# PolarisRisingWar/rgb-experiment

Hardware: AMD Instinct MI355X
Metric: aggregated edges/sec (full-graph GCN d=128, reference epoch = train fwd+bwd+Adam + 2 eval fwd) (higher is better)
Workload: dtype f32

## Files before the change

include/rgbx_hip.h:

```cpp
#ifndef RGBX_HIP_H
#define RGBX_HIP_H

#include <stddef.h>
#include <stdint.h>

#ifdef __cplusplus
extern "C" {
#endif

#define RGBX_VERSION 501

#define RGBX_OK 0
#define RGBX_E_ARG (-1)
#define RGBX_E_RANGE (-2)
#define RGBX_E_ALIGN (-3)
#define RGBX_E_WS (-4)
#define RGBX_E_SHAPE (-5)

typedef void* rgbx_stream_t;

enum {
  RGBX_LOOPS_KEEP = 0,
  RGBX_LOOPS_ADD_REMAINING = 1,
  RGBX_LOOPS_REMOVE_ADD = 2
// ... 77 lines not shown
  float* std;      int64_t ld_std;
  float* max;      int64_t ld_max;
  int32_t* argmax; int64_t ld_argmax;
  float* min;      int64_t ld_min;
  int32_t* argmin; int64_t ld_argmin;
} rgbx_multi_out_t;
int rgbx_spmm_csr_multi_supported(int64_t d);
int rgbx_spmm_csr_multi_partial_words(int64_t n_chunks, int64_t d, int which, int64_t* words);
int rgbx_spmm_csr_multi_f32(const int32_t* rowptr, const int32_t* col, const float* x, int64_t ldx,
                            const rgbx_multi_out_t* out, int64_t N, int64_t d, const rgbx_row_split_t* split,
                            rgbx_stream_t stream);

typedef struct rgbx_multi_grad {
  const float* a;        int64_t ld_a;
  const float* b;        int64_t ld_b;
  const float* x;        int64_t ld_x;
  const float* gmax;     int64_t ld_gmax;
  const int32_t* argmax; int64_t ld_argmax;
  const float* gmin;     int64_t ld_gmin;
  const int32_t* argmin; int64_t ld_argmin;
} rgbx_multi_grad_t;
int rgbx_multi_bwd_f32(const int32_t* rowptr_t, const int32_t* col_t, const int32_t* t2f, const rgbx_multi_grad_t* terms,
                       float* gx, int64_t ldgx, int64_t N, int64_t d, const rgbx_row_split_t* split, rgbx_stream_t stream);

typedef struct rgbx_spmm_epilogue {
  const struct rgbx_ce_epilogue* ce;
  int64_t n_classes;
  double* out_colsums;
  void* stats_ws;
  size_t stats_ws_bytes;
} rgbx_spmm_epilogue_t;

int rgbx_spmm_csr_epilogue_supported(int64_t d);
int rgbx_spmm_csr_epilogue_f32(const int32_t* rowptr, const int32_t* col, const float* w, const float* rs,
                               const float* x, int64_t ldx, const float* y, int64_t ldy, const float* bias,
                               float* out, int64_t ldo, int64_t N, int64_t d, float a, float b,
                               const rgbx_row_split_t* split, const rgbx_spmm_epilogue_t* epi,
                               rgbx_stream_t stream);

int rgbx_spmm_csr_short_rows_supported(int64_t d);
int rgbx_spmm_csr_short_rows_f32(const int32_t* rowptr, const int32_t* col, const float* w, const float* x, int64_t ldx,
                                 const float* bias, float* out, int64_t ldo, int64_t N, int64_t d, rgbx_stream_t stream);

typedef struct rgbx_ce_epilogue {
  const int64_t* y;
  const uint8_t* mask;
  const float* grad_scale;
  double* stats;
  double* scratch;
  int32_t mask_groups;
  const int32_t* rows;
  int64_t n_rows;
  int32_t skip_unselected;
} rgbx_ce_epilogue_t;

int rgbx_spmm_linear_supported(int64_t K, int64_t Nout, int has_root);
int rgbx_ce_rows_grad_scratch_doubles(int64_t N, int64_t* count);
int rgbx_spmm_linear_stats_workspace_bytes(int64_t N, int64_t Nout, size_t* bytes);
int rgbx_spmm_linear_f32(const int32_t* rowptr, const int32_t* col, const float* w, const float* rs,
                         const float* x, int64_t ldx, const float* wt, const float* x_root, int64_t ldr,
                         const float* wt_root, const float* bias, float* out, int64_t ldo, float* z_out,
                         int64_t ldz, const float* pre_scale, const float* pre_shift, const float* pre_rowsum,
                         double* out_colsums, void* stats_ws, size_t stats_ws_bytes,
                         const rgbx_ce_epilogue_t* ce, int64_t N, int64_t K, int64_t Nout,
                         const rgbx_row_split_t* split, rgbx_stream_t stream);

typedef struct rgbx_fused_layer {
  const int32_t* rowptr;
  const int32_t* col;
  const float* w;
  const float* rs;
  const float* x;
  int64_t ldx;
  int64_t x_blk_cols, x_blk_stride;
  const float* wt;
  const float* x_root;
  int64_t ldr;
  int64_t xr_blk_cols, xr_blk_stride;
  const float* wt_root;
  const float* bias;
  float* out;
  int64_t ldo;
  float* out_blk;
  int64_t ob_cols, ob_stride;
  float* z_out;
  int64_t ldz;
  const float* pre_scale;
  const float* pre_shift;
  const float* pre_rowsum;
  double* out_colsums;
  void* stats_ws;
  size_t stats_ws_bytes;
  const rgbx_ce_epilogue_t* ce;
  int64_t N, K, Nout;
  const rgbx_row_split_t* split;
  const float* w_pos;
  float* z_pos_out;
  const uint8_t* col_sel;
} rgbx_fused_layer_t;

int rgbx_fused_layer_f32(const rgbx_fused_layer_t* layer, rgbx_stream_t stream);

int rgbx_blocked_to_rows_f32(const float* src, int64_t blk_cols, int64_t blk_stride, float* dst, int64_t ldd,
                             int64_t n, int64_t d, const float* bias, rgbx_stream_t stream);

int rgbx_appnp_f32(const int32_t* rowptr, const int32_t* col, const float* w, const float* h,
                   int64_t ldh, float* out, float* tmp, int64_t ldo, int64_t N, int64_t d, int K,
                   float alpha, const rgbx_row_split_t* split, rgbx_stream_t stream);


int rgbx_dagnn_gate_fwd_f32(const float* h0, int64_t ld0, const float* hops, int64_t hop_stride, int64_t ldh,
                            const float* s, const float* b, float* out, int64_t ldo, int64_t N, int64_t d, int K,
                            rgbx_stream_t stream);

int rgbx_dagnn_gate_bwd_workspace_bytes(int64_t d, size_t* bytes);
int rgbx_dagnn_gate_bwd_f32(const float* h0, int64_t ld0, const float* hops, int64_t hop_stride, int64_t ldh,
                            const float* s, const float* b, const float* gout, int64_t ldg, float* d0,
                            int64_t ldd0, float* dk, int64_t d_stride, int64_t ldd, float* g_s, float* g_b,
                            void* ws, size_t ws_bytes, int64_t N, int64_t d, int K, rgbx_stream_t stream);


int rgbx_gru_step_supported(int64_t C);
int rgbx_gru_step_f32(const int32_t* rowptr, const int32_t* col, const float* x, int64_t ldx, const float* wt,
                      const float* wt_root, const float* bias, float* out, int64_t ldo, float* z_out, int64_t ldz,
                      float* pre_out, int64_t ldp, int64_t N, int64_t C, const rgbx_row_split_t* split,
                      rgbx_stream_t stream);

int rgbx_gru_gate_fwd_f32(const float* pre, int64_t ldp, const float* x, int64_t ldx, float* out, int64_t ldo,
                          int64_t N, int64_t C, rgbx_stream_t stream);

int rgbx_gru_gate_bwd_f32(const float* pre, int64_t ldp, const float* x, int64_t ldx, const float* gout, int64_t ldg,
                          float* dpre, int64_t lddp, float* dx, int64_t lddx, int64_t N, int64_t C,
                          rgbx_stream_t stream);


int rgbx_gat_scores_f32(const float* hfeat, int64_t ldh, const float* att_src,
                        const float* att_dst, float* a_src, float* a_dst, int64_t n, int H, int C,
                        rgbx_stream_t stream);

int rgbx_gat_scores_bwd_scratch_floats(int64_t n, int H, int C, int64_t* count);

int rgbx_gat_scores_bwd_f32(const float* hfeat, int64_t ldh, const float* g_a_src, const float* g_a_dst,
                            int64_t n_dst, const float* att_src, const float* att_dst, float* g_hfeat,
                            int64_t ldgh, float* g_att_src, float* g_att_dst, float* scratch,
                            int64_t scratch_floats, int64_t n, int H, int C, rgbx_stream_t stream);

int rgbx_gat_aggregate_fwd_f32(const int32_t* rowptr, const int32_t* col, const float* hfeat,
                               int64_t ldh, const float* a_src, const float* att_src,
                               float* a_dst, const float* att_dst, const float* out_scale, const float* bias,
                               float* out, int64_t ldo, float* m, float* rden, float* out_pos, float* a_pos,
                               int64_t N, int H, int C, float slope, const rgbx_row_split_t* split,
// ... 105 lines not shown
                                 const float* nodeq, const float* gout, int64_t ldg, float* g_k, int64_t ldgk,
                                 float* g_v, int64_t ldgv, int64_t N, int H, int C, float scale, const uint32_t* seed,
                                 float p_drop, const rgbx_row_split_t* split, rgbx_stream_t stream);



int rgbx_resgated_supported(int C);

int rgbx_resgated_fwd_f32(const int32_t* rowptr, const int32_t* col, const float* k, int64_t ldk, const float* q,
                          int64_t ldq, const float* v, int64_t ldv, float* out, int64_t ldo, int64_t N, int C,
                          const rgbx_row_split_t* split, rgbx_stream_t stream);

int rgbx_resgated_bwd_dst_f32(const int32_t* rowptr, const int32_t* col, const float* k, int64_t ldk, const float* q,
                              int64_t ldq, const float* v, int64_t ldv, const float* gout, int64_t ldg, float* g_k,
                              int64_t ldgk, int64_t N, int C, const rgbx_row_split_t* split, rgbx_stream_t stream);

int rgbx_resgated_bwd_src_f32(const int32_t* rowptr_t, const int32_t* col_t, const float* k, int64_t ldk, const float* q,
                              int64_t ldq, const float* v, int64_t ldv, const float* gout, int64_t ldg, float* g_q,
                              int64_t ldgq, float* g_v, int64_t ldgv, int64_t N, int C, const rgbx_row_split_t* split,
                              rgbx_stream_t stream);



int rgbx_softmax_aggr_supported(int C);

int rgbx_softmax_aggr_fwd_f32(const int32_t* rowptr, const int32_t* col, const float* m, int64_t ldm, const float* t,
                              int t_stride, float* out, int64_t ldo, float* lse, int64_t ldl, int64_t N, int C,
                              const rgbx_row_split_t* split, rgbx_stream_t stream);

int rgbx_softmax_aggr_gt_partial_floats(int64_t N, int C, const rgbx_row_split_t* split, int64_t* count);

int rgbx_softmax_aggr_bwd_f32(const int32_t* rowptr_t, const int32_t* col_t, const float* m, int64_t ldm, const float* t,
                              int t_stride, const float* out, int64_t ldo, const float* lse, int64_t ldl,
                              const float* gout, int64_t ldg, float* g_m, int64_t ldgm, float* g_t, float* gt_partial,
                              int64_t n_gt_partial, int64_t N, int C, const rgbx_row_split_t* split,
                              rgbx_stream_t stream);


int rgbx_gemm_tn_workspace_bytes(int64_t K, int64_t M, int64_t N, size_t* bytes);

int rgbx_gemm_tn_f32(const float* A, int64_t lda, const float* B, int64_t ldb, float* C, int64_t ldc,
                     float* a_colsum, int64_t K, int64_t M, int64_t N, float alpha, void* workspace,
                     size_t workspace_bytes, rgbx_stream_t stream);

int rgbx_gemm_tn_bn_bwd_f32(const float* G, int64_t ldg, const float* X, int64_t ldx, const float* mean,
                            const float* rstd, const float* ca, const float* cb, const float* ck, const float* B,
                            int64_t ldb, float* C, int64_t ldc, float* a_colsum, int64_t K, int64_t M, int64_t N,
                            float alpha, void* workspace, size_t workspace_bytes, rgbx_stream_t stream);

int rgbx_gemm_tn_rows_f32(const float* A, int64_t lda, const float* B, int64_t ldb, const int32_t* rows,
                          int64_t n_rows, float* C, int64_t ldc, float* a_colsum, int64_t K, int64_t M, int64_t N,
                          float alpha, void* workspace, size_t workspace_bytes, rgbx_stream_t stream);


int rgbx_bn_scratch_doubles(int64_t N, int64_t d, int64_t* count);

int rgbx_bn_stats_f32(const float* x, int64_t ldx, int64_t N, int64_t d, double* sums, double* scratch,
                      int64_t scratch_doubles, rgbx_stream_t stream);

int rgbx_bn_finalize_f32(const double* packed, const float* weight, const float* bias, float eps, float momentum,
                         float* running_mean, float* running_var, float* mean, float* rstd, float* scale,
                         float* shift, int64_t d, rgbx_stream_t stream);

int rgbx_fold_bn_linear_f32(const float* W, int64_t ldw, const float* Wr, int64_t ldwr, const float* bias,
                            const float* bias2, const float* gamma, const float* beta, const float* running_mean,
                            const float* running_var, float eps, float* wt, float* wrt, float* b_out, int64_t Nout,
                            int64_t K, rgbx_stream_t stream);

int rgbx_bn_bwd_finalize_f32(const double* glob, const double* local, const double* count, const float* weight,
                             const float* rstd, float* ca, float* cb, float* ck, float* g_weight, float* g_bias,
                             int64_t d, rgbx_stream_t stream);

int rgbx_affine_cols_f32(const float* x, int64_t ldx, const float* scale, const float* shift, float* y,
                         int64_t ldy, int64_t N, int64_t d, rgbx_stream_t stream);

int rgbx_bn_bwd_reduce_f32(const float* gy, int64_t ldg, const float* x, int64_t ldx, const float* mean,
                           const float* rstd, int64_t N, int64_t d, double* sums, double* scratch,
                           int64_t scratch_doubles, rgbx_stream_t stream);

int rgbx_bn_bwd_apply_f32(const float* gy, int64_t ldg, const float* x, int64_t ldx, const float* mean,
                          const float* rstd, const float* ca, const float* cb, const float* ck, float* gx,
                          int64_t ldgx, int64_t N, int64_t d, rgbx_stream_t stream);


int rgbx_masked_nll_scratch_doubles(int64_t N, int want_accuracy, int64_t* count);

int rgbx_masked_nll_fwd_f32(const float* logp, int64_t ld, const int64_t* y, const uint8_t* mask,
                            int64_t N, int64_t C, double* stats, double* scratch,
                            int64_t scratch_doubles, int want_accuracy, rgbx_stream_t stream);

int rgbx_masked_nll_bwd_f32(const int64_t* y, const uint8_t* mask, int64_t N, int64_t C,
                            const float* scale, float* grad, int64_t ldg, rgbx_stream_t stream);

int rgbx_masked_ce_fwd_f32(const float* logits, int64_t ld, const int64_t* y, const uint8_t* mask, int64_t N,
                           int64_t C, double* stats, double* scratch, int64_t scratch_doubles,
                           rgbx_stream_t stream);

int rgbx_masked_ce_fwd_blocked_f32(const float* logits, int64_t blk_cols, int64_t blk_stride, const float* bias,
                                   const int64_t* y, const uint8_t* mask, int64_t N, int64_t C, double* stats,
                                   double* scratch, int64_t scratch_doubles, rgbx_stream_t stream);

int rgbx_masked_ce_bwd_f32(const float* logits, int64_t ld, const int64_t* y, const uint8_t* mask, int64_t N,
                           int64_t C, const float* scale, float* grad, int64_t ldg, rgbx_stream_t stream);


int rgbx_coalesce_workspace_bytes(int64_t E, int64_t N, int mirror, size_t* bytes);
// ... 54 lines not shown
```

rgb_experiment_amd/_lib.py:

```python
import ctypes
import os

import torch

_HERE = os.path.dirname(os.path.abspath(__file__))
LIB_PATH = os.path.join(_HERE, "csrc", "librgbx_hip.so")

_P = ctypes.c_void_p
_I64 = ctypes.c_int64
_I = ctypes.c_int
_F = ctypes.c_float

class RowSplit(ctypes.Structure):
    _fields_ = [("threshold", ctypes.c_int32), ("n_chunks", ctypes.c_int32), ("n_long", ctypes.c_int32),
                ("chunk_begin", ctypes.c_void_p), ("chunk_end", ctypes.c_void_p), ("chunk_row", ctypes.c_void_p),
                ("long_row", ctypes.c_void_p),
                ("long_chunk_ptr", ctypes.c_void_p), ("partial", ctypes.c_void_p)]


class MultiOut(ctypes.Structure):
    _fields_ = [(f, t) for name in ("sum", "mean", "var", "std", "max", "argmax", "min", "argmin")
                for f, t in ((name, ctypes.c_void_p), ("ld_" + name, ctypes.c_int64))]


class MultiGrad(ctypes.Structure):
    _fields_ = [(f, t) for name in ("a", "b", "x", "gmax", "argmax", "gmin", "argmin")
                for f, t in ((name, ctypes.c_void_p), ("ld_" + name, ctypes.c_int64))]


class CeEpilogue(ctypes.Structure):
    _fields_ = [("y", ctypes.c_void_p), ("mask", ctypes.c_void_p), ("grad_scale", ctypes.c_void_p),
                ("stats", ctypes.c_void_p), ("scratch", ctypes.c_void_p), ("mask_groups", ctypes.c_int32),
                ("rows", ctypes.c_void_p), ("n_rows", ctypes.c_int64), ("skip_unselected", ctypes.c_int32)]


class SpmmEpilogue(ctypes.Structure):
    _fields_ = [("ce", ctypes.c_void_p), ("n_classes", ctypes.c_int64), ("out_colsums", ctypes.c_void_p),
                ("stats_ws", ctypes.c_void_p), ("stats_ws_bytes", ctypes.c_size_t)]


class FusedLayer(ctypes.Structure):
    _fields_ = [("rowptr", _P), ("col", _P), ("w", _P), ("rs", _P), ("x", _P), ("ldx", _I64),
                ("x_blk_cols", _I64), ("x_blk_stride", _I64), ("wt", _P), ("x_root", _P), ("ldr", _I64),
                ("xr_blk_cols", _I64), ("xr_blk_stride", _I64), ("wt_root", _P), ("bias", _P), ("out", _P),
                ("ldo", _I64), ("out_blk", _P), ("ob_cols", _I64), ("ob_stride", _I64), ("z_out", _P), ("ldz", _I64),
                ("pre_scale", _P), ("pre_shift", _P), ("pre_rowsum", _P), ("out_colsums", _P), ("stats_ws", _P),
                ("stats_ws_bytes", ctypes.c_size_t), ("ce", _P), ("N", _I64), ("K", _I64), ("Nout", _I64),
                ("split", _P), ("w_pos", _P), ("z_pos_out", _P), ("col_sel", _P)]


SIGNATURES = {
    "rgbx_csr_workspace_bytes": [_I64, _I64, ctypes.POINTER(ctypes.c_size_t)],
    "rgbx_csr_build": [_P, _P, _I64, _I64, _I, _P, _P, _P, _P, ctypes.c_size_t, _P],
    "rgbx_deg_inv_sqrt_f32": [_P, _I64, _P, _P],
    "rgbx_gcn_norm_f32": [_P, _P, _I64, _P, _P, _P],
    "rgbx_inv_degree_f32": [_P, _I64, _P, _P],
    "rgbx_loop_weights_f32": [_P, _P, _P, _I64, _I64, _I, _F, _P, _P, _P],
    "rgbx_edge_slot_weights_f32": [_P, _I64, _P, _I64, _P, _P, _P],
    "rgbx_weighted_deg_inv_sqrt_f32": [_P, _P, _I64, _P, _P],
    "rgbx_gcn_norm_weighted_f32": [_P, _P, _P, _I64, _P, _P, _P],
    "rgbx_edge_dot_supported": [_I64],
    "rgbx_edge_dot_f32": [_P, _P, _P, _I64, _P, _I64, _P, _I64, _I64, _P, _P],
    "rgbx_gcn_norm_bwd_f32": [_P, _P, _P, _P, _P, _P, _P, _P, _P, _P, _I64, _I64, _P, _P, _P],
    "rgbx_spmm_csr_f32": [_P, _P, _P, _P, _P, _I64, _P, _I64, _P, _P, _I64, _I64, _I64, _F, _F, _P, _P],
    "rgbx_spmm_csr_extremum_supported": [_I64],
    "rgbx_spmm_csr_extremum_f32": [_P, _P, _P, _I64, _P, _I64, _P, _I64, _I64, _I, _P, _P],
    "rgbx_extremum_bwd_f32": [_P, _P, _P, _P, _I64, _P, _P, _I64, _I64, _I64, _P, _P],
    "rgbx_spmm_csr_multi_supported": [_I64],
    "rgbx_spmm_csr_multi_partial_words": [_I64, _I64, _I, ctypes.POINTER(ctypes.c_int64)],
    "rgbx_spmm_csr_multi_f32": [_P, _P, _P, _I64, _P, _I64, _I64, _P, _P],
    "rgbx_multi_bwd_f32": [_P, _P, _P, _P, _P, _I64, _I64, _I64, _P, _P],
    "rgbx_spmm_csr_epilogue_supported": [_I64],
    "rgbx_spmm_csr_epilogue_f32": [_P, _P, _P, _P, _P, _I64, _P, _I64, _P, _P, _I64, _I64, _I64, _F, _F, _P, _P, _P],
    "rgbx_spmm_csr_short_rows_supported": [_I64],
    "rgbx_spmm_csr_short_rows_f32": [_P, _P, _P, _P, _I64, _P, _P, _I64, _I64, _I64, _P],
    "rgbx_spmm_linear_supported": [_I64, _I64, _I],
    "rgbx_ce_rows_grad_scratch_doubles": [_I64, ctypes.POINTER(ctypes.c_int64)],
    "rgbx_spmm_linear_stats_workspace_bytes": [_I64, _I64, ctypes.POINTER(ctypes.c_size_t)],
    "rgbx_spmm_linear_f32": [_P, _P, _P, _P, _P, _I64, _P, _P, _I64, _P, _P, _P, _I64, _P, _I64, _P, _P, _P, _P, _P,
                             ctypes.c_size_t, _P, _I64, _I64, _I64, _P, _P],
    "rgbx_fused_layer_f32": [_P, _P],
    "rgbx_blocked_to_rows_f32": [_P, _I64, _I64, _P, _I64, _I64, _I64, _P, _P],
    "rgbx_appnp_f32": [_P, _P, _P, _P, _I64, _P, _P, _I64, _I64, _I64, _I, _F, _P, _P],
    "rgbx_dagnn_gate_fwd_f32": [_P, _I64, _P, _I64, _I64, _P, _P, _P, _I64, _I64, _I64, _I, _P],
    "rgbx_dagnn_gate_bwd_workspace_bytes": [_I64, ctypes.POINTER(ctypes.c_size_t)],
    "rgbx_dagnn_gate_bwd_f32": [_P, _I64, _P, _I64, _I64, _P, _P, _P, _I64, _P, _I64, _P, _I64, _I64, _P, _P, _P,
                                ctypes.c_size_t, _I64, _I64, _I, _P],
    "rgbx_gru_step_supported": [_I64],
    "rgbx_gru_step_f32": [_P, _P, _P, _I64, _P, _P, _P, _P, _I64, _P, _I64, _P, _I64, _I64, _I64, _P, _P],
    "rgbx_gru_gate_fwd_f32": [_P, _I64, _P, _I64, _P, _I64, _I64, _I64, _P],
    "rgbx_gru_gate_bwd_f32": [_P, _I64, _P, _I64, _P, _I64, _P, _I64, _P, _I64, _I64, _I64, _P],
    "rgbx_gat_scores_f32": [_P, _I64, _P, _P, _P, _P, _I64, _I, _I, _P],
    "rgbx_gat_scores_bwd_scratch_floats": [_I64, _I, _I, ctypes.POINTER(ctypes.c_int64)],
    "rgbx_gat_scores_bwd_f32": [_P, _I64, _P, _P, _I64, _P, _P, _P, _I64, _P, _P, _P, _I64, _I64, _I, _I, _P],
    "rgbx_gat_aggregate_fwd_f32": [_P, _P, _P, _I64, _P, _P, _P, _P, _P, _P, _P, _I64, _P, _P, _P, _P, _I64, _I, _I, _F, _P,
                                   _P],
    "rgbx_gat_edge_softmax_f32": [_P, _P, _P, _P, _F, _P, _P, _P, _P, _P, _I64, _P, _P],
    "rgbx_gat_bwd_dst_f32": [_P, _P, _P, _I64, _P, _P, _P, _P, _P, _I64, _P, _I64, _P, _P, _I64, _I, _I,
                             _F, _P],
    "rgbx_gat_bwd_prep_f32": [_P, _P, _P, _P, _I64, _P, _P, _I64, _P, _P, _P, _F, _P, _I64, _I, _I, _P],
    "rgbx_gat_bwd_src_f32": [_P, _P, _P, _I64, _P, _P, _P, _I64, _P, _I64, _P, _P, _P, _P, _I64, _I, _I, _F, _P, _P],
    "rgbx_supergat_supported": [_I, _I],
    "rgbx_supergat_loss_records": [_I64, _P, ctypes.POINTER(ctypes.c_int64)],
    "rgbx_supergat_aggregate_fwd_f32": [_P, _P, _P, _I64, _P, _P, _P, _P, _I64, _P, _P, _I64, _I, _I, _F, _P, _F, _F, _P,
                                        _I64, _P, _P, _P],
    "rgbx_supergat_bwd_dst_f32": [_P, _P, _P, _I64, _P, _P, _P, _P, _P, _I64, _P, _P, _I64, _P, _P, _I64, _P, _I64, _I, _I,
                                  _F, _P, _F, _F, _P, _P, _P],
    "rgbx_supergat_bwd_src_f32": [_P, _P, _P, _P, _I64, _P, _P, _P, _I64, _P, _I64, _P, _I64, _I, _I, _F, _P, _F, _F, _P,
                                  _P, _P],
    "rgbx_supergat_sample_negatives": [_P, _I64, _I64, _P, _I64, _I, _P, _P, _P],
    "rgbx_supergat_neg_loss_fwd_f32": [_P, _I64, _P, _P, _I64, _I, _I, _P, _I64, _P, _P],
    "rgbx_supergat_neg_loss_bwd_f32": [_P, _I64, _P, _P, _I64, _I, _I, _P, _P, _I64, _P],
    "rgbx_supergat_draws_u8": [_P, _I64, _I, _F, _F, _P, _P, _P],
    "rgbx_gatv2_supported": [_I, _I],
    "rgbx_gatv2_fwd_f32": [_P, _P, _P, _I64, _P, _I64, _P, _P, _P, _I64, _P, _P, _I64, _I, _I, _F, _P, _F, _P, _P],
    "rgbx_gatv2_att_partial_floats": [_I64, _I, _I, _P, ctypes.POINTER(ctypes.c_int64)],
    "rgbx_gatv2_bwd_dst_f32": [_P, _P, _P, _I64, _P, _I64, _P, _P, _P, _P, _I64, _P, _P, _I64, _P, _P, _I64, _P, _P, _I64,
                               _I64, _I, _I, _F, _P, _F, _P, _P],
    "rgbx_gatv2_bwd_src_f32": [_P, _P, _P, _P, _I64, _P, _I64, _P, _P, _P, _I64, _P, _I64, _I64, _I, _I, _F, _P, _F, _P,
                               _P],
    "rgbx_gatv2_draws_u8": [_P, _I64, _I, _F, _P, _P],
    "rgbx_transformer_supported": [_I, _I],
    "rgbx_transformer_fwd_f32": [_P, _P, _P, _I64, _P, _I64, _P, _I64, _P, _I64, _P, _P, _I64, _I, _I, _F, _P, _F, _P,
                                 _P],
    "rgbx_transformer_bwd_dst_f32": [_P, _P, _P, _I64, _P, _I64, _P, _I64, _P, _P, _P, _I64, _P, _I64, _P, _P, _I64,
                                     _I64, _I, _I, _F, _P, _F, _P, _P],
    "rgbx_transformer_bwd_src_f32": [_P, _P, _P, _P, _I64, _P, _I64, _P, _I64, _P, _P, _I64, _P, _I64, _P, _I64, _I64,
                                     _I, _I, _F, _P, _F, _P, _P],
    "rgbx_resgated_supported": [_I],
    "rgbx_resgated_fwd_f32": [_P, _P, _P, _I64, _P, _I64, _P, _I64, _P, _I64, _I64, _I, _P, _P],
    "rgbx_resgated_bwd_dst_f32": [_P, _P, _P, _I64, _P, _I64, _P, _I64, _P, _I64, _P, _I64, _I64, _I, _P, _P],
    "rgbx_resgated_bwd_src_f32": [_P, _P, _P, _I64, _P, _I64, _P, _I64, _P, _I64, _P, _I64, _P, _I64, _I64, _I, _P,
                                  _P],
    "rgbx_softmax_aggr_supported": [_I],
    "rgbx_softmax_aggr_fwd_f32": [_P, _P, _P, _I64, _P, _I, _P, _I64, _P, _I64, _I64, _I, _P, _P],
    "rgbx_softmax_aggr_gt_partial_floats": [_I64, _I, _P, ctypes.POINTER(ctypes.c_int64)],
    "rgbx_softmax_aggr_bwd_f32": [_P, _P, _P, _I64, _P, _I, _P, _I64, _P, _I64, _P, _I64, _P, _I64, _P, _P, _I64, _I64,
                                  _I, _P, _P],
    "rgbx_gemm_tn_workspace_bytes": [_I64, _I64, _I64, ctypes.POINTER(ctypes.c_size_t)],
    "rgbx_gemm_tn_f32": [_P, _I64, _P, _I64, _P, _I64, _P, _I64, _I64, _I64, _F, _P, ctypes.c_size_t, _P],
    "rgbx_gemm_tn_bn_bwd_f32": [_P, _I64, _P, _I64, _P, _P, _P, _P, _P, _P, _I64, _P, _I64, _P, _I64, _I64, _I64, _F, _P,
                                ctypes.c_size_t, _P],
    "rgbx_gemm_tn_rows_f32": [_P, _I64, _P, _I64, _P, _I64, _P, _I64, _P, _I64, _I64, _I64, _F, _P, ctypes.c_size_t, _P],
    "rgbx_bn_scratch_doubles": [_I64, _I64, ctypes.POINTER(ctypes.c_int64)],
    "rgbx_bn_stats_f32": [_P, _I64, _I64, _I64, _P, _P, _I64, _P],
    "rgbx_bn_finalize_f32": [_P, _P, _P, _F, _F, _P, _P, _P, _P, _P, _P, _I64, _P],
    "rgbx_fold_bn_linear_f32": [_P, _I64, _P, _I64, _P, _P, _P, _P, _P, _P, _F, _P, _P, _P, _I64, _I64, _P],
    "rgbx_bn_bwd_finalize_f32": [_P, _P, _P, _P, _P, _P, _P, _P, _P, _P, _I64, _P],
    "rgbx_affine_cols_f32": [_P, _I64, _P, _P, _P, _I64, _I64, _I64, _P],
    "rgbx_bn_bwd_reduce_f32": [_P, _I64, _P, _I64, _P, _P, _I64, _I64, _P, _P, _I64, _P],
    "rgbx_bn_bwd_apply_f32": [_P, _I64, _P, _I64, _P, _P, _P, _P, _P, _P, _I64, _I64, _I64, _P],
    "rgbx_masked_nll_scratch_doubles": [_I64, _I, ctypes.POINTER(ctypes.c_int64)],
    "rgbx_masked_nll_fwd_f32": [_P, _I64, _P, _P, _I64, _I64, _P, _P, _I64, _I, _P],
    "rgbx_masked_ce_fwd_f32": [_P, _I64, _P, _P, _I64, _I64, _P, _P, _I64, _P],
    "rgbx_masked_ce_fwd_blocked_f32": [_P, _I64, _I64, _P, _P, _P, _I64, _I64, _P, _P, _I64, _P],
    "rgbx_masked_ce_bwd_f32": [_P, _I64, _P, _P, _I64, _I64, _P, _P, _I64, _P],
    "rgbx_masked_nll_bwd_f32": [_P, _P, _I64, _I64, _P, _P, _I64, _P],
    "rgbx_coalesce_workspace_bytes": [_I64, _I64, _I, ctypes.POINTER(ctypes.c_size_t)],
    "rgbx_coalesce_keys_i64": [_P, _P, _I64, _I64, _I, _P, _P, _P, ctypes.c_size_t, _P],
    "rgbx_split_edge_keys_i64": [_P, _P, _I64, _I64, _P, _P, _P],
    "rgbx_gather_rows_f32": [_P, _I64, _P, _I64, _I64, _P, _I64, _P],
    "rgbx_scatter_add_rows_f32": [_P, _I64, _P, _I64, _I64, _P, _I64, _P],
    "rgbx_paced_copy_f32": [_P, _P, _I64, _I, _I, _P],
    "rgbx_py_random_shuffle_i64": [_I64, _I64, _P],
    "rgbx_faconv_supported": [_I64],
    "rgbx_faconv_scores_f32": [_P, _I64, _P, _P, _P, _I64, _I64, _P],
    "rgbx_faconv_fwd_f32": [_P, _P, _P, _P, _I64, _P, _P, _I64, _F, _P, _I64, _I64, _I64, _P, _F, _P, _P],
    "rgbx_faconv_bwd_dst_f32": [_P, _P, _P, _P, _I64, _P, _P, _I64, _P, _I64, _I64, _P, _F, _P, _P],
    "rgbx_faconv_bwd_src_f32": [_P, _P, _P, _P, _P, _I64, _P, _P, _I64, _P, _P, _P, _P, _I64, _I64, _I64, _P, _F, _P,
                                _P],
    "rgbx_faconv_edge_coef_f32": [_P, _P, _P, _P, _P, _I, _I64, _P, _F, _P, _P, _P],
    "rgbx_faconv_edge_dot_f32": [_P, _P, _P, _P, _I64, _P, _I64, _P, _I64, _I64, _I64, _P],
    "rgbx_faconv_draws_u8": [_P, _I64, _F, _P, _P],
}
EXPORTS = ["rgbx_version", "rgbx_last_error_string"] + list(SIGNATURES)

_lib = None


def bind(path, strict=True):
    lib = ctypes.CDLL(path)
    lib.rgbx_version.restype = _I
    lib.rgbx_version.argtypes = []
    lib.rgbx_last_error_string.restype = ctypes.c_char_p
    lib.rgbx_last_error_string.argtypes = []
    for name, argtypes in SIGNATURES.items():
        if not strict and not hasattr(lib, name):
            continue
        fn = getattr(lib, name)
        fn.restype = _I
        fn.argtypes = argtypes
    return lib


def load():
    global _lib
# ... 46 lines not shown
```

rgb_experiment_amd/csrc/gemm.hip:

```cpp
#include "rgbx_common.h"

namespace rgbx {
namespace {

constexpr int BM = 128, BN = 128, KT = 32;
enum { A_PLAIN = 0, A_BN = 1, A_ROWS = 2 };

struct TnExtra {
  const float* X;
  int64_t ldx;
  const float *mean, *rstd, *ca, *cb, *ck;
  const int32_t* rows;
  int64_t n_rows;
};
using f32x16 = __attribute__((ext_vector_type(16))) float;

template <int W>
__device__ __forceinline__ void stage_tile(float* __restrict__ lds, const float* __restrict__ src,
                                           int64_t ld, int64_t k0, int64_t k_end, int c0, int ncols) {
  const int tid = threadIdx.x;
#pragma unroll 4
  for (int p = 0; p < KT * W / 256; ++p) {
    const int idx = p * 256 + tid;
    const int r = idx / W, c = idx % W;
    const int64_t k = k0 + r;
    lds[r * W + c] = (k < k_end && c0 + c < ncols) ? src[k * ld + c0 + c] : 0.f;
  }
}

template <int W>
__device__ __forceinline__ void fetch_tile(float4 (&regs)[KT * (W / 4) / 256], const float* __restrict__ src, int64_t ld,
                                           int64_t k0, int64_t k_end, int c0, int ncols) {
#pragma unroll
  for (int p = 0; p < KT * (W / 4) / 256; ++p) {
    const int idx = p * 256 + threadIdx.x;
    const int r = idx / (W / 4), c = (idx % (W / 4)) * 4;
    const int64_t k = k0 + r;
    regs[p] = make_float4(0.f, 0.f, 0.f, 0.f);
    if (k < k_end && c0 + c < ncols) regs[p] = *reinterpret_cast<const float4*>(src + k * ld + c0 + c);
  }
}

template <int W>
__device__ __forceinline__ void put_tile(float* __restrict__ lds, const float4 (&regs)[KT * (W / 4) / 256]) {
#pragma unroll
  for (int p = 0; p < KT * (W / 4) / 256; ++p) {
    const int idx = p * 256 + threadIdx.x;
    const int r = idx / (W / 4), c = (idx % (W / 4)) * 4;
    *reinterpret_cast<float4*>(lds + r * W + c) = regs[p];
  }
}

template <int W>
__device__ __forceinline__ void put_tile_bn(float* __restrict__ lds, const float4 (&rg)[KT * (W / 4) / 256],
                                            const float4 (&rx)[KT * (W / 4) / 256], const float* __restrict__ lc,
                                            int64_t k0, int64_t k_end, int c0, int ncols) {
#pragma unroll
  for (int p = 0; p < KT * (W / 4) / 256; ++p) {
    const int idx = p * 256 + threadIdx.x;
// ... 88 lines not shown
      for (int i = 0; i < MI; ++i) {
        acc[i][0] = __builtin_amdgcn_mfma_f32_32x32x2f32(a[i], b0, acc[i][0], 0, 0, 0);
        acc[i][1] = __builtin_amdgcn_mfma_f32_32x32x2f32(a[i], b1, acc[i][1], 0, 0, 0);
      }
    }
  };
  if constexpr (MODE == A_BN) {
    float* lc = lds + KT * (MT + 128);
    for (int i = threadIdx.x; i < 5 * MT; i += 256) {
      const float* src = i < MT ? ex.mean : i < 2 * MT ? ex.rstd : i < 3 * MT ? ex.ca : i < 4 * MT ? ex.cb : ex.ck;
      const int c = m0 + i % MT;
      lc[i] = c < M ? src[c] : 0.f;
    }
    float4 ra[KT * (MT / 4) / 256], rx[KT * (MT / 4) / 256], rb[KT * 32 / 256];
    fetch_tile<MT>(ra, A, lda, k_begin, k_end, m0, M);
    fetch_tile<MT>(rx, ex.X, ex.ldx, k_begin, k_end, m0, M);
    fetch_tile<128>(rb, B, ldb, k_begin, k_end, n0, N);
    for (int64_t k0 = k_begin; k0 < k_end; k0 += KT) {
      __syncthreads();
      put_tile_bn<MT>(la, ra, rx, lc, k0, k_end, m0, M);
      put_tile<128>(lb, rb);
      __syncthreads();
      if (k0 + KT < k_end) {
        fetch_tile<MT>(ra, A, lda, k0 + KT, k_end, m0, M);
        fetch_tile<MT>(rx, ex.X, ex.ldx, k0 + KT, k_end, m0, M);
        fetch_tile<128>(rb, B, ldb, k0 + KT, k_end, n0, N);
      }
      consume();
    }
  } else if constexpr (MODE == A_ROWS) {
    const int64_t j_begin = lower_bound_rows(ex.rows, ex.n_rows, k_begin);
    const int64_t j_end = lower_bound_rows(ex.rows, ex.n_rows, k_end);
    float4 ra[KT * (MT / 4) / 256], rb[KT * 32 / 256];
    int32_t ia[KT * (MT / 4) / 256], ib[KT * 32 / 256];
    fetch_row_ids<MT>(ia, ex.rows, j_begin, j_end);
    fetch_row_ids<128>(ib, ex.rows, j_begin, j_end);
    fetch_tile_rows<MT>(ra, A, lda, ia, m0, M);
    fetch_tile_rows<128>(rb, B, ldb, ib, n0, N);
    fetch_row_ids<MT>(ia, ex.rows, j_begin + KT, j_end);
    fetch_row_ids<128>(ib, ex.rows, j_begin + KT, j_end);
    for (int64_t j0 = j_begin; j0 < j_end; j0 += KT) {
      __syncthreads();
      put_tile<MT>(la, ra);
      put_tile<128>(lb, rb);
      __syncthreads();
      if (j0 + KT < j_end) {
        fetch_tile_rows<MT>(ra, A, lda, ia, m0, M);
        fetch_tile_rows<128>(rb, B, ldb, ib, n0, N);
        fetch_row_ids<MT>(ia, ex.rows, j0 + 2 * KT, j_end);
        fetch_row_ids<128>(ib, ex.rows, j0 + 2 * KT, j_end);
      }
      consume();
    }
  } else if constexpr (VEC4) {
    float4 ra[KT * (MT / 4) / 256], rb[KT * 32 / 256];
    fetch_tile<MT>(ra, A, lda, k_begin, k_end, m0, M);
    fetch_tile<128>(rb, B, ldb, k_begin, k_end, n0, N);
    for (int64_t k0 = k_begin; k0 < k_end; k0 += KT) {
      __syncthreads();
      put_tile<MT>(la, ra);
      put_tile<128>(lb, rb);
      __syncthreads();
      if (k0 + KT < k_end) {
        fetch_tile<MT>(ra, A, lda, k0 + KT, k_end, m0, M);
        fetch_tile<128>(rb, B, ldb, k0 + KT, k_end, n0, N);
      }
      consume();
    }
  } else {
    for (int64_t k0 = k_begin; k0 < k_end; k0 += KT) {
      __syncthreads();
      stage_tile<MT>(la, A, lda, k0, k_end, m0, M);
      stage_tile<128>(lb, B, ldb, k0, k_end, n0, N);
      __syncthreads();
      consume();
    }
  }

  if (sums && m0 + (int)threadIdx.x < M) colpart[(int64_t)split * M + m0 + threadIdx.x] = csum;
  float* out = part + (int64_t)split * M * N;
#pragma unroll
  for (int i = 0; i < MI; ++i)
#pragma unroll
    for (int j = 0; j < 2; ++j)
#pragma unroll
      for (int r = 0; r < 16; ++r) {
        const int m = m0 + wm + i * 32 + (r & 3) + 8 * (r >> 2) + 4 * kr;
        const int n = n0 + wn + j * 32 + cc;
        if (m < M && n < N) out[(int64_t)m * N + n] = acc[i][j][r];
      }
}

__global__ void __launch_bounds__(256)
gemm_tn_reduce_kernel(const float* __restrict__ part, int S, int64_t MN, float* __restrict__ C, int N,
                      int64_t ldc, float alpha) {
  __shared__ float sh[8][32];
  const int j = threadIdx.x & 31, q = threadIdx.x >> 5;
  for (int64_t base = (int64_t)blockIdx.x * 32; base < MN; base += (int64_t)gridDim.x * 32) {
    const int64_t i = base + j;
    float s = 0.f;
    if (i < MN)
      for (int p = q; p < S; p += 8) s += part[(int64_t)p * MN + i];
    __syncthreads();
    sh[q][j] = s;
    __syncthreads();
    if (q == 0 && i < MN) {
      float t = 0.f;
#pragma unroll
      for (int k = 0; k < 8; ++k) t += sh[k][j];
      C[(i / N) * ldc + (i % N)] = alpha * t;
    }
  }
}

int tile_rows(int M) { return M <= 64 ? 64 : BM; }

int choose_splits(int64_t K, int M, int N) {
  const int64_t tiles = cdiv(M, tile_rows(M)) * cdiv(N, BN);
  int64_t s = cdiv(tile_rows(M) == 64 ? 1024 : 768, tiles);
  const int64_t max_s = cdiv(K, 16 * KT);
  if (s > max_s) s = max_s;
  if (s < 1) s = 1;
  return (int)s;
}

}
}

using namespace rgbx;

extern "C" int rgbx_gemm_tn_workspace_bytes(int64_t K, int64_t M, int64_t N, size_t* bytes) {
  if (!bytes || K < 0 || M < 0 || N < 0) return fail(RGBX_E_ARG, "gemm_tn_workspace_bytes: bad argument");
  if (M >= INT32_MAX || N >= INT32_MAX) return fail(RGBX_E_RANGE, "gemm_tn: M or N exceeds int32");
  *bytes = (size_t)choose_splits(K, (int)M, (int)N) * ((size_t)M * (size_t)N + (size_t)M) * sizeof(float);
  return RGBX_OK;
}

namespace rgbx {
namespace {

int run_gemm_tn(const char* name, int mode, const float* A, int64_t lda, const float* B, int64_t ldb, float* C,
                int64_t ldc, float* a_colsum, int64_t K, int64_t M, int64_t N, float alpha, void* workspace,
                size_t workspace_bytes, rgbx_stream_t stream, const TnExtra& ex) {
  if (K < 0 || M < 0 || N < 0) return fail(RGBX_E_ARG, "%s: negative size", name);
  if (M == 0 || N == 0) return RGBX_OK;
  if (!C || (K > 0 && (!A || !B))) return fail(RGBX_E_ARG, "%s: null pointer", name);
  if (M >= INT32_MAX || N >= INT32_MAX) return fail(RGBX_E_RANGE, "%s: M or N exceeds int32", name);
  if (lda < M || ldb < N || ldc < N) return fail(RGBX_E_ARG, "%s: leading dimension too small", name);
  bool v4 = aligned16(A) && aligned16(B) && lda % 4 == 0 && ldb % 4 == 0;
  if (mode == A_BN) {
    if (K > 0 && (!ex.X || !ex.mean || !ex.rstd || !ex.ca || !ex.cb || !ex.ck))
      return fail(RGBX_E_ARG, "%s: null pointer", name);
    if (ex.ldx < M) return fail(RGBX_E_ARG, "%s: leading dimension too small", name);
    v4 = v4 && aligned16(ex.X) && ex.ldx % 4 == 0;
  }
  if (mode == A_ROWS) {
    if (ex.n_rows < 0 || ex.n_rows > K || (ex.n_rows > 0 && !ex.rows)) return fail(RGBX_E_ARG, "%s: bad row list", name);
    if (K >= INT32_MAX) return fail(RGBX_E_RANGE, "%s: K exceeds int32", name);
  }
  if (mode != A_PLAIN && !v4)
    return fail(RGBX_E_ALIGN, "%s: operands must be 16-byte aligned with leading dimensions that are multiples of 4", name);
  size_t need = 0;
  if (int rc = rgbx_gemm_tn_workspace_bytes(K, M, N, &need)) return rc;
  if (!workspace || workspace_bytes < need)
    return fail(RGBX_E_WS, "%s: workspace %zu < %zu bytes", name, workspace_bytes, need);
  hipStream_t s = (hipStream_t)stream;
  const int S = choose_splits(K, (int)M, (int)N);
  const int64_t slab = cdiv(cdiv(K > 0 ? K : 1, S), KT) * KT;
  float* part = static_cast<float*>(workspace);
  float* colpart = a_colsum ? part + (size_t)S * M * N : nullptr;
  const int mt = tile_rows((int)M);
  dim3 grid(S, (unsigned)cdiv(M, mt), (unsigned)cdiv(N, BN));
#define RGBX_GEMM_TN(V4, MT, MODE) \
  gemm_tn_partial_kernel<V4, MT, MODE><<<grid, 256, 0, s>>>(A, lda, B, ldb, part, colpart, K, (int)M, (int)N, slab, ex)
  if (mode == A_BN) { if (mt == 64) RGBX_GEMM_TN(true, 64, A_BN); else RGBX_GEMM_TN(true, 128, A_BN); }
  else if (mode == A_ROWS) { if (mt == 64) RGBX_GEMM_TN(true, 64, A_ROWS); else RGBX_GEMM_TN(true, 128, A_ROWS); }
  else if (v4) { if (mt == 64) RGBX_GEMM_TN(true, 64, A_PLAIN); else RGBX_GEMM_TN(true, 128, A_PLAIN); }
  else { if (mt == 64) RGBX_GEMM_TN(false, 64, A_PLAIN); else RGBX_GEMM_TN(false, 128, A_PLAIN); }
#undef RGBX_GEMM_TN
  RGBX_CHECK_LAUNCH("gemm_tn_partial_kernel");
  const int64_t MN = M * N;
  int64_t rb = cdiv(MN, 32);
  if (rb > kMaxGrid) rb = kMaxGrid;
  gemm_tn_reduce_kernel<<<(int)rb, 256, 0, s>>>(part, S, MN, C, (int)N, ldc, alpha);
  RGBX_CHECK_LAUNCH("gemm_tn_reduce_kernel");
  if (a_colsum) {
    gemm_tn_reduce_kernel<<<(int)cdiv(M, 32), 256, 0, s>>>(colpart, S, M, a_colsum, (int)M, M, 1.0f);
    RGBX_CHECK_LAUNCH("gemm_tn_reduce_kernel");
  }
  return RGBX_OK;
}

}
}

extern "C" int rgbx_gemm_tn_f32(const float* A, int64_t lda, const float* B, int64_t ldb, float* C,
                                int64_t ldc, float* a_colsum, int64_t K, int64_t M, int64_t N, float alpha,
                                void* workspace, size_t workspace_bytes, rgbx_stream_t stream) {
  return run_gemm_tn("gemm_tn", A_PLAIN, A, lda, B, ldb, C, ldc, a_colsum, K, M, N, alpha, workspace, workspace_bytes,
                     stream, TnExtra{});
}

extern "C" int rgbx_gemm_tn_bn_bwd_f32(const float* G, int64_t ldg, const float* X, int64_t ldx, const float* mean,
                                       const float* rstd, const float* ca, const float* cb, const float* ck,
                                       const float* B, int64_t ldb, float* C, int64_t ldc, float* a_colsum, int64_t K,
                                       int64_t M, int64_t N, float alpha, void* workspace, size_t workspace_bytes,
                                       rgbx_stream_t stream) {
  TnExtra ex{};
  ex.X = X, ex.ldx = ldx, ex.mean = mean, ex.rstd = rstd, ex.ca = ca, ex.cb = cb, ex.ck = ck;
  return run_gemm_tn("gemm_tn_bn_bwd", A_BN, G, ldg, B, ldb, C, ldc, a_colsum, K, M, N, alpha, workspace,
                     workspace_bytes, stream, ex);
}

extern "C" int rgbx_gemm_tn_rows_f32(const float* A, int64_t lda, const float* B, int64_t ldb, const int32_t* rows,
                                     int64_t n_rows, float* C, int64_t ldc, float* a_colsum, int64_t K, int64_t M,
                                     int64_t N, float alpha, void* workspace, size_t workspace_bytes,
                                     rgbx_stream_t stream) {
  TnExtra ex{};
  ex.rows = rows, ex.n_rows = n_rows;
  return run_gemm_tn("gemm_tn_rows", A_ROWS, A, lda, B, ldb, C, ldc, a_colsum, K, M, N, alpha, workspace,
                     workspace_bytes, stream, ex);
}
```

rgb_experiment_amd/csrc/graph_prep.hip:

```cpp
#include "rgbx_common.h"

#include <rocprim/rocprim.hpp>

namespace rgbx {

char* err_buf() {
  static thread_local char buf[256] = "";
  return buf;
}

namespace {

__global__ void __launch_bounds__(256)
fill_keys_kernel(const int64_t* __restrict__ agg_row, const int64_t* __restrict__ other_row,
                 int64_t E, int64_t M, int N, int loops_mode, int* __restrict__ keys,
                 int* __restrict__ ids) {
  for (int64_t e = (int64_t)blockIdx.x * blockDim.x + threadIdx.x; e < M;
       e += (int64_t)gridDim.x * blockDim.x) {
    int key;
    if (e < E) {
      const int64_t t = agg_row[e];
      key = (loops_mode != RGBX_LOOPS_KEEP && other_row[e] == t) ? N : (int)t;
    } else {
      key = (int)(e - E);
// ... 33 lines not shown
  }
}

__global__ void __launch_bounds__(256)
inv_degree_kernel(const int* __restrict__ rowptr, int N, float* __restrict__ inv) {
  for (int i = blockIdx.x * blockDim.x + threadIdx.x; i < N; i += gridDim.x * blockDim.x) {
    const int cnt = rowptr[i + 1] - rowptr[i];
    inv[i] = 1.0f / (float)(cnt > 1 ? cnt : 1);
  }
}

__global__ void __launch_bounds__(256)
gcn_norm_kernel(const int* __restrict__ rowptr, const int* __restrict__ col, int N,
                const float* __restrict__ dis, float* __restrict__ w) {
  const int lane = threadIdx.x & 63;
  const int wpb = blockDim.x >> 6;
  for (int row = blockIdx.x * wpb + (threadIdx.x >> 6); row < N; row += gridDim.x * wpb) {
    const int s = rowptr[row], e = rowptr[row + 1];
    const float di = dis[row];
    for (int p = s + lane; p < e; p += 64) w[p] = dis[col[p]] * di;
  }
}


__global__ void __launch_bounds__(256) fill_i32_kernel(int* __restrict__ v, int64_t n, int value) {
  for (int64_t i = (int64_t)blockIdx.x * blockDim.x + threadIdx.x; i < n; i += (int64_t)gridDim.x * blockDim.x)
    v[i] = value;
}

__global__ void __launch_bounds__(256)
loop_source_kernel(const int64_t* __restrict__ src, const int64_t* __restrict__ dst, int64_t E,
                   int* __restrict__ loop_src) {
  for (int64_t e = (int64_t)blockIdx.x * blockDim.x + threadIdx.x; e < E; e += (int64_t)gridDim.x * blockDim.x) {
    const int64_t t = dst[e];
    if (src[e] == t) atomicMax(loop_src + t, (int)e);
  }
}

__global__ void __launch_bounds__(256)
loop_weight_kernel(const int* __restrict__ loop_src, const float* __restrict__ ew, int N, float fill,
                   float* __restrict__ loop_w) {
  for (int i = blockIdx.x * blockDim.x + threadIdx.x; i < N; i += gridDim.x * blockDim.x) {
    const int e = loop_src[i];
    loop_w[i] = e >= 0 ? ew[e] : fill;
  }
}

__global__ void __launch_bounds__(256)
slot_weight_kernel(const int* __restrict__ perm, int64_t nnz, const float* __restrict__ ew, int64_t E,
                   const float* __restrict__ loop_w, float* __restrict__ ew_slot) {
  for (int64_t p = (int64_t)blockIdx.x * blockDim.x + threadIdx.x; p < nnz; p += (int64_t)gridDim.x * blockDim.x) {
    const int id = perm[p];
    ew_slot[p] = id < E ? ew[id] : loop_w[id - E];
  }
}

__device__ __forceinline__ float wave_sum_fixed(float v) {
#pragma unroll
  for (int off = 32; off >= 1; off >>= 1) v += __shfl_xor(v, off);
  return v;
}

__global__ void __launch_bounds__(256)
weighted_deg_inv_sqrt_kernel(const int* __restrict__ rowptr, const float* __restrict__ ew_slot, int N,
                             float* __restrict__ dis) {
  const int lane = threadIdx.x & 63;
  const int wpb = blockDim.x >> 6;
  for (int row = blockIdx.x * wpb + (threadIdx.x >> 6); row < N; row += gridDim.x * wpb) {
    const int s = rowptr[row], e = rowptr[row + 1];
    float acc = 0.f;
    for (int p = s + lane; p < e; p += 64) acc += ew_slot[p];
    const float deg = wave_sum_fixed(acc);
    if (lane == 0) dis[row] = deg == 0.f ? 0.f : 1.0f / sqrtf(deg);
  }
}

__global__ void __launch_bounds__(256)
gcn_norm_weighted_kernel(const int* __restrict__ rowptr, const int* __restrict__ col,
                         const float* __restrict__ ew_slot, int N, const float* __restrict__ dis,
                         float* __restrict__ w) {
  const int lane = threadIdx.x & 63;
  const int wpb = blockDim.x >> 6;
  for (int row = blockIdx.x * wpb + (threadIdx.x >> 6); row < N; row += gridDim.x * wpb) {
    const int s = rowptr[row], e = rowptr[row + 1];
    const float di = dis[row];
    for (int p = s + lane; p < e; p += 64) w[p] = dis[col[p]] * ew_slot[p] * di;
  }
}

__global__ void __launch_bounds__(256)
gcn_norm_bwd_deg_kernel(const int* __restrict__ rowptr, const int* __restrict__ col,
                        const int* __restrict__ rowptr_t, const int* __restrict__ col_t,
                        const int* __restrict__ t2f, const float* __restrict__ g,
                        const float* __restrict__ ew_slot, const float* __restrict__ dis, int N,
                        float* __restrict__ ddeg) {
  const int lane = threadIdx.x & 63;
  const int wpb = blockDim.x >> 6;
  for (int row = blockIdx.x * wpb + (threadIdx.x >> 6); row < N; row += gridDim.x * wpb) {
    float acc = 0.f;
    for (int p = rowptr[row] + lane; p < rowptr[row + 1]; p += 64) acc = fmaf(g[p] * ew_slot[p], dis[col[p]], acc);
    float acc_t = 0.f;
    for (int q = rowptr_t[row] + lane; q < rowptr_t[row + 1]; q += 64) {
      const int p = t2f[q];
      acc_t = fmaf(g[p] * ew_slot[p], dis[col_t[q]], acc_t);
    }
    const float ddis = wave_sum_fixed(acc) + wave_sum_fixed(acc_t);
// ... 141 lines not shown
  RGBX_CHECK_LAUNCH("loop_weight_kernel");
  return RGBX_OK;
}

extern "C" int rgbx_edge_slot_weights_f32(const int32_t* perm, int64_t nnz, const float* ew, int64_t E,
                                          const float* loop_w, float* ew_slot, rgbx_stream_t stream) {
  if (nnz < 0 || E < 0 || (nnz > 0 && (!perm || !ew_slot)) || (E > 0 && !ew))
    return fail(RGBX_E_ARG, "edge_slot_weights: null pointer or negative size");
  if (nnz > E && !loop_w) return fail(RGBX_E_ARG, "edge_slot_weights: nnz > E needs loop weights");
  if (nnz == 0) return RGBX_OK;
  slot_weight_kernel<<<grid_for(nnz), 256, 0, (hipStream_t)stream>>>(perm, nnz, ew, E, loop_w, ew_slot);
  RGBX_CHECK_LAUNCH("slot_weight_kernel");
  return RGBX_OK;
}

extern "C" int rgbx_weighted_deg_inv_sqrt_f32(const int32_t* rowptr, const float* ew_slot, int64_t N, float* dis,
                                              rgbx_stream_t stream) {
  if (N < 0 || !rowptr || !ew_slot || (N > 0 && !dis)) return fail(RGBX_E_ARG, "weighted_deg_inv_sqrt: bad argument");
  if (N >= INT32_MAX) return fail(RGBX_E_RANGE, "weighted_deg_inv_sqrt: N exceeds int32");
  if (N == 0) return RGBX_OK;
  weighted_deg_inv_sqrt_kernel<<<grid_for(N, 4), 256, 0, (hipStream_t)stream>>>(rowptr, ew_slot, (int)N, dis);
  RGBX_CHECK_LAUNCH("weighted_deg_inv_sqrt_kernel");
  return RGBX_OK;
}

extern "C" int rgbx_gcn_norm_weighted_f32(const int32_t* rowptr, const int32_t* col, const float* ew_slot,
                                          int64_t N, const float* dis, float* w, rgbx_stream_t stream) {
  if (N < 0 || !rowptr || !col || !ew_slot || !dis || !w) return fail(RGBX_E_ARG, "gcn_norm_weighted: bad argument");
  if (N >= INT32_MAX) return fail(RGBX_E_RANGE, "gcn_norm_weighted: N exceeds int32");
  if (N == 0) return RGBX_OK;
  gcn_norm_weighted_kernel<<<grid_for(N, 4), 256, 0, (hipStream_t)stream>>>(rowptr, col, ew_slot, (int)N, dis, w);
  RGBX_CHECK_LAUNCH("gcn_norm_weighted_kernel");
  return RGBX_OK;
}

extern "C" int rgbx_gcn_norm_bwd_f32(const int32_t* rowptr, const int32_t* col, const int32_t* perm,
                                     const int32_t* rowptr_t, const int32_t* col_t, const int32_t* t2f,
                                     const int32_t* loop_src, const float* g, const float* ew_slot,
                                     const float* dis, int64_t N, int64_t E, float* ddeg, float* dew,
                                     rgbx_stream_t stream) {
  if (N < 0 || E < 0) return fail(RGBX_E_ARG, "gcn_norm_bwd: negative size");
  if (!rowptr || !col || !perm || !rowptr_t || !col_t || !t2f || !g || !ew_slot || !dis || !ddeg || (E > 0 && !dew))
    return fail(RGBX_E_ARG, "gcn_norm_bwd: null pointer");
  if (N >= INT32_MAX || E >= INT32_MAX) return fail(RGBX_E_RANGE, "gcn_norm_bwd: N or E exceeds int32");
  hipStream_t s = (hipStream_t)stream;
  if (E > 0) RGBX_HIP(hipMemsetAsync(dew, 0, sizeof(float) * (size_t)E, s));
  if (N == 0) return RGBX_OK;
  gcn_norm_bwd_deg_kernel<<<grid_for(N, 4), 256, 0, s>>>(rowptr, col, rowptr_t, col_t, t2f, g, ew_slot, dis, (int)N, ddeg);
  RGBX_CHECK_LAUNCH("gcn_norm_bwd_deg_kernel");
  gcn_norm_bwd_edge_kernel<<<grid_for(N, 4), 256, 0, s>>>(rowptr, col, perm, loop_src, g, dis, ddeg, (int)N, E, dew);
  RGBX_CHECK_LAUNCH("gcn_norm_bwd_edge_kernel");
  return RGBX_OK;
}
```

rgb_experiment_amd/csrc/spmm.hip:

```cpp
#include "rgbx_common.h"
#include "spmm_internal.h"

namespace rgbx {
namespace {

struct SpmmArgs {
  const int* rowptr;
  const int* col;
  const float* w;
  const float* rs;
  const float* x;
  const float* y;
  const float* bias;
  float* out;
  int64_t ldx, ldy, ldo;
  int N, d;
  float a, b;
  int skip_longer;
};

template <int G, int VEC, bool HAS_W>
__device__ __forceinline__ void accumulate_slots(const SpmmArgs& A, int start, int end, const float* xc,
                                                 bool active, int lane, int g, float (&acc)[VEC]) {
  constexpr int NG = kWave / G;
  constexpr int U = 4;
  for (int base = start; base < end; base += kWave) {
    const int n = min(kWave, end - base);
    int mycol = 0;
    float myw = 0.f;
    if (lane < n) {
      mycol = A.col[base + lane];
      if constexpr (HAS_W) myw = A.w[base + lane];
    }
    for (int k = 0; k < n; k += NG * U) {
      float v[U][VEC];
      float ww[U];
#pragma unroll
      for (int u = 0; u < U; ++u) {
        const int idx = k + u * NG + g;
        const int src = __shfl(mycol, idx & 63);
        if constexpr (HAS_W) ww[u] = __shfl(myw, idx & 63);
        const bool ok = active && idx < n;
#pragma unroll
        for (int i = 0; i < VEC; ++i) v[u][i] = 0.f;
        if (ok) load_vec<VEC>(v[u], xc + (int64_t)src * A.ldx);
        if constexpr (HAS_W) { if (!ok) ww[u] = 0.f; }
      }
#pragma unroll
      for (int u = 0; u < U; ++u) {
#pragma unroll
        for (int i = 0; i < VEC; ++i) {
          if constexpr (HAS_W) acc[i] = fmaf(ww[u], v[u][i], acc[i]);
          else acc[i] += v[u][i];
        }
      }
    }
  }
#pragma unroll
  for (int off = 32; off >= G; off >>= 1) {
#pragma unroll
    for (int i = 0; i < VEC; ++i) acc[i] += __shfl_xor(acc[i], off);
  }
}

template <int VEC>
__device__ __forceinline__ void spmm_epilogue(const SpmmArgs& A, int row, int c, const float (&acc)[VEC]) {
  const float scale = A.rs ? A.a * A.rs[row] : A.a;
  float r[VEC];
#pragma unroll
  for (int i = 0; i < VEC; ++i) r[i] = scale * acc[i];
  if (A.y) {
    float yv[VEC];
    load_vec<VEC>(yv, A.y + (int64_t)row * A.ldy + c);
#pragma unroll
    for (int i = 0; i < VEC; ++i) r[i] = fmaf(A.b, yv[i], r[i]);
  }
  if (A.bias) {
    float bv[VEC];
    load_vec<VEC>(bv, A.bias + c);
#pragma unroll
    for (int i = 0; i < VEC; ++i) r[i] += bv[i];
  }
  if constexpr (VEC == 4) {
    using f4v = __attribute__((ext_vector_type(4))) float;
    f4v t = {r[0], r[1], r[2], r[3]};
    __builtin_nontemporal_store(t, reinterpret_cast<f4v*>(A.out + (int64_t)row * A.ldo + c));
  } else {
    store_vec<VEC>(A.out + (int64_t)row * A.ldo + c, r);
  }
}

template <int G, int VEC, bool HAS_W>
__global__ void __launch_bounds__(256) spmm_csr_kernel(const SpmmArgs A) {
  const int lane = threadIdx.x & 63;
  const int g = lane / G;
  const int t = lane % G;
  const int wpb = blockDim.x >> 6;
  const int wave0 = blockIdx.x * wpb + (threadIdx.x >> 6);
  const int wstride = gridDim.x * wpb;

  for (int row = wave0; row < A.N; row += wstride) {
    const int start = __builtin_amdgcn_readfirstlane(A.rowptr[row]);
    const int end = __builtin_amdgcn_readfirstlane(A.rowptr[row + 1]);
    if (A.skip_longer > 0 && end - start > A.skip_longer) continue;
    for (int cbase = 0; cbase < A.d; cbase += G * VEC) {
      const int c = cbase + t * VEC;
      const bool active = c < A.d;
      float acc[VEC];
#pragma unroll
      for (int i = 0; i < VEC; ++i) acc[i] = 0.f;
      accumulate_slots<G, VEC, HAS_W>(A, start, end, A.x + c, active, lane, g, acc);
      if (g == 0 && active) spmm_epilogue<VEC>(A, row, c, acc);
    }
  }
}

template <int G, int VEC, bool HAS_W>
__global__ void __launch_bounds__(256)
spmm_chunk_kernel(const SpmmArgs A, int n_chunks, const int* __restrict__ chunk_begin,
                  const int* __restrict__ chunk_end, float* __restrict__ partial) {
  const int lane = threadIdx.x & 63;
  const int g = lane / G;
  const int t = lane % G;
  const int wpb = blockDim.x >> 6;
  for (int ch = blockIdx.x * wpb + (threadIdx.x >> 6); ch < n_chunks; ch += gridDim.x * wpb) {
    const int start = __builtin_amdgcn_readfirstlane(chunk_begin[ch]);
    const int end = __builtin_amdgcn_readfirstlane(chunk_end[ch]);
    for (int cbase = 0; cbase < A.d; cbase += G * VEC) {
      const int c = cbase + t * VEC;
      const bool active = c < A.d;
      float acc[VEC];
#pragma unroll
      for (int i = 0; i < VEC; ++i) acc[i] = 0.f;
      accumulate_slots<G, VEC, HAS_W>(A, start, end, A.x + c, active, lane, g, acc);
      if (g == 0 && active) store_vec<VEC>(partial + (int64_t)ch * A.d + c, acc);
    }
  }
}

template <int VEC>
__global__ void __launch_bounds__(256)
spmm_combine_kernel(const SpmmArgs A, int n_long, const int* __restrict__ long_row,
                    const int* __restrict__ long_chunk_ptr, const float* __restrict__ partial) {
  const int lane = threadIdx.x & 63;
  const int wpb = blockDim.x >> 6;
  for (int r = blockIdx.x * wpb + (threadIdx.x >> 6); r < n_long; r += gridDim.x * wpb) {
    const int row = long_row[r];
    const int c0 = long_chunk_ptr[r], c1 = long_chunk_ptr[r + 1];
    for (int c = lane * VEC; c < A.d; c += kWave * VEC) {
      float acc[VEC];
#pragma unroll
      for (int i = 0; i < VEC; ++i) acc[i] = 0.f;
      for (int ch = c0; ch < c1; ++ch) {
        float p[VEC];
        load_vec<VEC>(p, partial + (int64_t)ch * A.d + c);
#pragma unroll
        for (int i = 0; i < VEC; ++i) acc[i] += p[i];
      }
      spmm_epilogue<VEC>(A, row, c, acc);
    }
  }
}

template <int VEC>
__global__ void __launch_bounds__(256)
spmm_combine_compact_kernel(const float* __restrict__ rs, int d, int n_long, const int* __restrict__ long_row,
                            const int* __restrict__ long_chunk_ptr, const float* __restrict__ partial,
                            float* __restrict__ zlong) {
  const int lane = threadIdx.x & 63;
  const int wpb = blockDim.x >> 6;
  for (int r = blockIdx.x * wpb + (threadIdx.x >> 6); r < n_long; r += gridDim.x * wpb) {
    const float scale = rs ? rs[long_row[r]] : 1.0f;
    const int c0 = long_chunk_ptr[r], c1 = long_chunk_ptr[r + 1];
    for (int c = lane * VEC; c < d; c += kWave * VEC) {
      float acc[VEC];
#pragma unroll
      for (int i = 0; i < VEC; ++i) acc[i] = 0.f;
      for (int ch = c0; ch < c1; ++ch) {
        float p[VEC];
        load_vec<VEC>(p, partial + (int64_t)ch * d + c);
#pragma unroll
        for (int i = 0; i < VEC; ++i) acc[i] += p[i];
      }
#pragma unroll
      for (int i = 0; i < VEC; ++i) acc[i] *= scale;
      store_vec<VEC>(zlong + (int64_t)r * d + c, acc);
    }
  }
}

template <int G>
int launch_long_compact(const SpmmArgs& A, const rgbx_row_split_t* sp, float* zlong, hipStream_t s) {
  int64_t cb = cdiv(sp->n_chunks, 4);
  if (cb > kMaxGrid) cb = kMaxGrid;
  if (A.w)
    spmm_chunk_kernel<G, 4, true><<<(int)cb, 256, 0, s>>>(A, sp->n_chunks, sp->chunk_begin, sp->chunk_end, sp->partial);
  else
    spmm_chunk_kernel<G, 4, false><<<(int)cb, 256, 0, s>>>(A, sp->n_chunks, sp->chunk_begin, sp->chunk_end, sp->partial);
  RGBX_CHECK_LAUNCH("spmm_chunk_kernel");
  int64_t lb = cdiv(sp->n_long, 4);
  if (lb > kMaxGrid) lb = kMaxGrid;
  spmm_combine_compact_kernel<4><<<(int)lb, 256, 0, s>>>(A.rs, A.d, sp->n_long, sp->long_row, sp->long_chunk_ptr,
                                                         sp->partial, zlong);
  RGBX_CHECK_LAUNCH("spmm_combine_compact_kernel");
  return RGBX_OK;
}

template <int G, int VEC>
int launch(const SpmmArgs& A, const rgbx_row_split_t* sp, hipStream_t s) {
  constexpr int kWavesPerBlock = 4;
  const int64_t blocks = cdiv(A.N, kWavesPerBlock);
  if (A.w)
    spmm_csr_kernel<G, VEC, true><<<(int)blocks, 256, 0, s>>>(A);
  else
    spmm_csr_kernel<G, VEC, false><<<(int)blocks, 256, 0, s>>>(A);
  RGBX_CHECK_LAUNCH("spmm_csr_kernel");
  if (sp) {
    int64_t cb = cdiv(sp->n_chunks, kWavesPerBlock);
    if (cb > kMaxGrid) cb = kMaxGrid;
    if (A.w)
      spmm_chunk_kernel<G, VEC, true><<<(int)cb, 256, 0, s>>>(A, sp->n_chunks, sp->chunk_begin, sp->chunk_end,
                                                             sp->partial);
    else
      spmm_chunk_kernel<G, VEC, false><<<(int)cb, 256, 0, s>>>(A, sp->n_chunks, sp->chunk_begin, sp->chunk_end,
                                                              sp->partial);
    RGBX_CHECK_LAUNCH("spmm_chunk_kernel");
    int64_t lb = cdiv(sp->n_long, kWavesPerBlock);
    if (lb > kMaxGrid) lb = kMaxGrid;
    spmm_combine_kernel<VEC><<<(int)lb, 256, 0, s>>>(A, sp->n_long, sp->long_row, sp->long_chunk_ptr, sp->partial);
    RGBX_CHECK_LAUNCH("spmm_combine_kernel");
  }
  return RGBX_OK;
}

struct EpiArgs {
  float* stats_part;
  const int64_t* ce_y;
  const uint8_t* ce_mask;
  const float* ce_scale;
  double* ce_part;
  int ce_groups;
  int C;
  const int* long_row;
  const float* zlong;
  int threshold, n_long;
};

template <int G, bool HAS_W, bool CE>
// ... 185 lines not shown
}

template <int G>
int launch_epilogue(const SpmmArgs& A, const EpiArgs& E, hipStream_t s) {
  const int tiles = (int)cdiv(A.N, kTileRows);
  if (E.ce_part) {
    if (A.w) spmm_tile_epilogue_kernel<G, true, true><<<tiles, 256, 0, s>>>(A, E);
    else spmm_tile_epilogue_kernel<G, false, true><<<tiles, 256, 0, s>>>(A, E);
  } else {
    if (A.w) spmm_tile_epilogue_kernel<G, true, false><<<tiles, 256, 0, s>>>(A, E);
    else spmm_tile_epilogue_kernel<G, false, false><<<tiles, 256, 0, s>>>(A, E);
  }
  RGBX_CHECK_LAUNCH("spmm_tile_epilogue_kernel");
  return RGBX_OK;
}

template <int VEC>
int dispatch_groups(const SpmmArgs& A, const rgbx_row_split_t* sp, hipStream_t s) {
  const int lanes = (A.d + VEC - 1) / VEC;
  if (lanes <= 1) return launch<1, VEC>(A, sp, s);
  if (lanes <= 2) return launch<2, VEC>(A, sp, s);
  if (lanes <= 4) return launch<4, VEC>(A, sp, s);
  if (lanes <= 8) return launch<8, VEC>(A, sp, s);
  if (lanes <= 16) return launch<16, VEC>(A, sp, s);
  if (lanes <= 32) return launch<32, VEC>(A, sp, s);
  return launch<64, VEC>(A, sp, s);
}

int spmm_dispatch(SpmmArgs A, const rgbx_row_split_t* split, hipStream_t s) {
  const rgbx_row_split_t* sp = nullptr;
  if (split && split->threshold > 0 && split->n_chunks > 0) {
    if (split->n_long <= 0 || !split->chunk_begin || !split->chunk_end || !split->long_row ||
        !split->long_chunk_ptr || !split->partial)
      return fail(RGBX_E_ARG, "spmm: incomplete row-split plan");
    sp = split;
    A.skip_longer = split->threshold;
  }
  auto vec_ok = [&](int v) {
    const uintptr_t mask = (uintptr_t)v * 4 - 1;
    auto okp = [&](const void* p, int64_t ld) {
      return !p || (((reinterpret_cast<uintptr_t>(p) & mask) == 0) && (ld % v == 0));
    };
    return A.d % v == 0 && okp(A.x, A.ldx) && okp(A.y, A.ldy) && okp(A.out, A.ldo) && okp(A.bias, v) &&
           (!sp || okp(sp->partial, v));
  };
  if (vec_ok(4)) return dispatch_groups<4>(A, sp, s);
  if (vec_ok(2)) return dispatch_groups<2>(A, sp, s);
  return dispatch_groups<1>(A, sp, s);
}

}

int spmm_long_rows_compact(const int* rowptr, const int* col, const float* w, const float* rs, const float* x,
                           int64_t ldx, int d, const rgbx_row_split_t* split, float* zlong, hipStream_t s) {
  if (!split || split->n_long <= 0 || split->n_chunks <= 0 || !split->chunk_begin || !split->chunk_end ||
      !split->long_row || !split->long_chunk_ptr || !split->partial || !zlong)
    return fail(RGBX_E_ARG, "spmm_long_rows: incomplete row-split plan");
  if (d % 4 || !aligned16(x) || ldx % 4 || !aligned16(split->partial) || !aligned16(zlong))
    return fail(RGBX_E_ALIGN, "spmm_long_rows: needs d %% 4 == 0 and 16-byte aligned x / partial / zlong");
  SpmmArgs A{rowptr, col, w, rs, x, nullptr, nullptr, zlong, ldx, 0, d, 0, d, 1.0f, 0.0f, 0};
  const int lanes = d / 4;
  if (lanes <= 1) return launch_long_compact<1>(A, split, zlong, s);
  if (lanes <= 2) return launch_long_compact<2>(A, split, zlong, s);
  if (lanes <= 4) return launch_long_compact<4>(A, split, zlong, s);
  if (lanes <= 8) return launch_long_compact<8>(A, split, zlong, s);
  if (lanes <= 16) return launch_long_compact<16>(A, split, zlong, s);
  if (lanes <= 32) return launch_long_compact<32>(A, split, zlong, s);
  return launch_long_compact<64>(A, split, zlong, s);
}

}

using namespace rgbx;

extern "C" int rgbx_spmm_csr_f32(const int32_t* rowptr, const int32_t* col, const float* w,
                                 const float* rs, const float* x, int64_t ldx, const float* y,
                                 int64_t ldy, const float* bias, float* out, int64_t ldo, int64_t N,
                                 int64_t d, float a, float b, const rgbx_row_split_t* split,
                                 rgbx_stream_t stream) {
  if (N < 0 || d < 0) return fail(RGBX_E_ARG, "spmm: negative size");
  if (N == 0 || d == 0) return RGBX_OK;
  if (!rowptr || !col || !x || !out) return fail(RGBX_E_ARG, "spmm: null pointer");
  if (N >= INT32_MAX || d >= INT32_MAX) return fail(RGBX_E_RANGE, "spmm: N or d exceeds int32");
  if (ldx < d || ldo < d || (y && ldy < d)) return fail(RGBX_E_ARG, "spmm: leading dimension < d");
  if (out == x) return fail(RGBX_E_ARG, "spmm: out must not alias x");
  SpmmArgs A{rowptr, col, w, rs, x, y, bias, out, ldx, ldy, ldo, (int)N, (int)d, a, b, 0};
  return spmm_dispatch(A, split, (hipStream_t)stream);
}

extern "C" int rgbx_appnp_f32(const int32_t* rowptr, const int32_t* col, const float* w,
                              const float* h, int64_t ldh, float* out, float* tmp, int64_t ldo,
                              int64_t N, int64_t d, int K, float alpha, const rgbx_row_split_t* split,
                              rgbx_stream_t stream) {
  if (N < 0 || d < 0 || K < 0) return fail(RGBX_E_ARG, "appnp: negative size");
  if (N == 0 || d == 0) return RGBX_OK;
  if (!rowptr || !col || !h || !out || (K > 1 && !tmp)) return fail(RGBX_E_ARG, "appnp: null pointer");
  if (N >= INT32_MAX || d >= INT32_MAX) return fail(RGBX_E_RANGE, "appnp: N or d exceeds int32");
  if (ldh < d || ldo < d) return fail(RGBX_E_ARG, "appnp: leading dimension < d");
  if (out == h || tmp == h || (K > 1 && out == tmp)) return fail(RGBX_E_ARG, "appnp: buffers alias");
  hipStream_t s = (hipStream_t)stream;
  if (K == 0) {
    RGBX_HIP(hipMemcpy2DAsync(out, ldo * sizeof(float), h, ldh * sizeof(float), d * sizeof(float),
                              N, hipMemcpyDeviceToDevice, s));
    return RGBX_OK;
  }
  const float* src = h;
  int64_t lds = ldh;
  for (int k = 0; k < K; ++k) {
    float* dst = ((K - 1 - k) % 2 == 0) ? out : tmp;
    SpmmArgs A{rowptr, col, w, nullptr, src, h, nullptr, dst, lds, ldh, ldo, (int)N, (int)d, 1.0f - alpha, alpha, 0};
    if (int rc = spmm_dispatch(A, split, s)) return rc;
    src = dst;
    lds = ldo;
// ... 80 lines not shown
```

rgb_experiment_amd/csrc/spmm_internal.h:

```cpp
#pragma once
#include "rgbx_common.h"

namespace rgbx {

int spmm_long_rows_compact(const int* rowptr, const int* col, const float* w, const float* rs, const float* x,
                           int64_t ldx, int d, const rgbx_row_split_t* split, float* zlong, hipStream_t s);

constexpr int kTileRows = 32;
constexpr int kCeGather = 64;
constexpr int kStatsGather = 1024;
int reduce_ce_tiles(double* scratch, int tiles, double* stats, int W, hipStream_t s);
int reduce_tile_stats(const float* part, int tiles, int width2, double* part2, double* sums, int64_t n_rows, hipStream_t s);

}
```

rgb_experiment_amd/csrc/spmm_linear.hip:

```cpp
#include "rgbx_common.h"
#include "spmm_internal.h"

namespace rgbx {
namespace {

using f32x16 = __attribute__((ext_vector_type(16))) float;

using f4v = __attribute__((ext_vector_type(4))) float;
__device__ __forceinline__ void nt_store4(float* p, const float (&v)[4]) {
  f4v t = {v[0], v[1], v[2], v[3]};
  __builtin_nontemporal_store(t, reinterpret_cast<f4v*>(p));
}
__device__ __forceinline__ void nt_store1(float* p, float v) { __builtin_nontemporal_store(v, p); }

struct FusedArgs {
  const int* rowptr;
  const int* col;
  const float* w;
  const float* rs;
  const float* x;
  const float* wt;
  const float* xr;
  const float* wtr;
  const float* bias;
  float* out;
  float* z_out;
  int64_t ldx, ldo, ldz, ldr;
  const int* long_row;
  const float* zlong;
  int threshold, n_long;
  int N, K, Nout;
  const float* pre_scale;
  const float* pre_shift;
  const float* pre_rowsum;
  float* stats_part;
  const int64_t* ce_y;
  const uint8_t* ce_mask;
  const float* ce_scale;
  double* ce_part;
  int ce_groups;
  int64_t x_bc, x_bs, xr_bc, xr_bs;
  float* out_blk;
  int64_t ob_c, ob_s;
  const float* w2;
  float* zpos_out;
  const float* zlong_pos;
  const int* ce_rows;
  int ce_n_rows;
  int ce_skip;
  float* ce_term;
  uint8_t* ce_hit;
  const uint8_t* col_sel;
};

__device__ __forceinline__ const float* blocked_at(const float* base, int64_t bc, int64_t bs, int64_t ld, int row,
                                                   int c) {
  return bc ? base + (int64_t)(c / (int)bc) * bs + (int64_t)row * bc + (c % (int)bc) : base + (int64_t)row * ld + c;
}

constexpr int TM = kTileRows;
constexpr int NT_ROOT = 2;

constexpr int KB = 16;

__device__ __forceinline__ void load_b_batch(float (&b)[KB], const float* __restrict__ wt, int Nout, int n0,
                                             int s0, int kr, int cc) {
#pragma unroll
  for (int i = 0; i < KB; ++i) b[i] = wt[(int64_t)(2 * (s0 + i) + kr) * Nout + n0 + cc];
}

__device__ __forceinline__ void mfma_batch(f32x16& acc, const float (&b)[KB], const float* __restrict__ zt, int ldz,
                                           int s0, int kr, int cc) {
#pragma unroll
  for (int i = 0; i < KB; ++i) {
    const float a = zt[cc * ldz + 2 * (s0 + i) + kr];
    acc = __builtin_amdgcn_mfma_f32_32x32x2f32(a, b[i], acc, 0, 0, 0);
  }
}

template <int KC>
__device__ __forceinline__ void tile_times_wt(f32x16& acc, const float* __restrict__ zt, int ldz,
                                              const float* __restrict__ wt, int K, int Nout, int n0, int kr,
                                              int cc, const float (*first)[KB] = nullptr) {
  if constexpr (KC > 0) {
    static_assert(KC % (2 * KB) == 0, "KC must be a multiple of 2 * KB");
    int s0 = 0;
    if (first) {
      mfma_batch(acc, *first, zt, ldz, 0, kr, cc);
      s0 = KB;
    }
#pragma unroll 1
    for (; s0 < KC / 2; s0 += KB) {
      float b[KB];
      load_b_batch(b, wt, Nout, n0, s0, kr, cc);
      mfma_batch(acc, b, zt, ldz, s0, kr, cc);
    }
  } else {
    for (int ks = 0; ks < K; ks += 4) {
      const float b0 = wt[(int64_t)(ks + kr) * Nout + n0 + cc];
      const float b1 = wt[(int64_t)(ks + 2 + kr) * Nout + n0 + cc];
      const float a0 = zt[cc * ldz + ks + kr], a1 = zt[cc * ldz + ks + 2 + kr];
      acc = __builtin_amdgcn_mfma_f32_32x32x2f32(a0, b0, acc, 0, 0, 0);
      acc = __builtin_amdgcn_mfma_f32_32x32x2f32(a1, b1, acc, 0, 0, 0);
    }
  }
// ... 83 lines not shown
    for (int k = 0; k < 32; ++k) t += sh[k][j];
    sums[c] = t;
  }
}


__device__ __forceinline__ int ce_select(const FusedArgs& A, int row, int* t) {
  int bits = A.ce_mask ? (int)A.ce_mask[row] : 1;
  bits = A.ce_groups == 2 ? (bits & 3) : (bits ? 1 : 0);
  *t = -1;
  if (bits) {
    const int64_t ti = A.ce_y[row];
    if (ti >= 0 && ti < A.Nout) *t = (int)ti;
  }
  return *t >= 0 ? bits : 0;
}

template <bool CE>
__device__ __forceinline__ int tile_row(const FusedArgs& A, int row_base, int r) {
  if constexpr (CE) {
    if (A.ce_rows) {
      const int i = row_base + r;
      const int row = i < A.ce_n_rows ? A.ce_rows[i] : A.N;
      return (unsigned)row < (unsigned)A.N ? row : A.N;
    }
  }
  return row_base + r;
}

__device__ __forceinline__ void zero_rows(float* __restrict__ base, int64_t ld, int q, int lo, int hi, int lane) {
  const int per = kWave / q, sub = lane / q;
  const float zero[4] = {0.f, 0.f, 0.f, 0.f};
  if (sub < per)
    for (int r = lo + sub; r < hi; r += per) nt_store4(base + (int64_t)r * ld + (lane - sub * q) * 4, zero);
}

__device__ __forceinline__ void ce_fill_gaps(const FusedArgs& A, int i, int row, int lane) {
  if (i >= A.ce_n_rows || row >= A.N) return;
  int lo = 0;
  if (i > 0) {
    const int prev = A.ce_rows[i - 1];
    lo = (unsigned)prev < (unsigned)A.N ? prev + 1 : A.N;
  }
  if (lo < row) {
    zero_rows(A.out, A.ldo, A.Nout >> 2, lo, row, lane);
    if (A.z_out) zero_rows(A.z_out, A.ldz, A.K >> 2, lo, row, lane);
  }
  if (i == A.ce_n_rows - 1 && row + 1 < A.N) {
    zero_rows(A.out, A.ldo, A.Nout >> 2, row + 1, A.N, lane);
    if (A.z_out) zero_rows(A.z_out, A.ldz, A.K >> 2, row + 1, A.N, lane);
  }
}

__device__ __forceinline__ void ce_epilogue(const FusedArgs& A, const f32x16& acc, float* __restrict__ ot, int row_base,
                                            int wave, int lane, int tile = -1) {
  if (tile < 0) tile = blockIdx.x;
  const int kr = lane >> 5, cc = lane & 31;
  const int ldq = A.Nout + 4;
  const int n0 = wave * 32;
  __syncthreads();
  if (n0 < A.Nout) {
    const float bb = A.bias ? A.bias[n0 + cc] : 0.f;
#pragma unroll
    for (int r = 0; r < 16; ++r) ot[((r & 3) + 8 * (r >> 2) + 4 * kr) * ldq + n0 + cc] = acc[r] + bb;
  }
  __syncthreads();
  double nll = 0.0, nll2 = 0.0;
  int cnt = 0, hit = 0, cnt2 = 0, hit2 = 0;
  const int W = 3 * A.ce_groups;
  const float sc = A.ce_scale ? A.ce_scale[0] : 0.f;
  const bool c0 = lane < A.Nout, c1 = lane + 64 < A.Nout;
  for (int rr = 0; rr < TM / 4; ++rr) {
    const int rl = wave * (TM / 4) + rr;
    const int row = tile_row<true>(A, row_base, rl);
    if (row >= A.N) break;
    int t;
    const int bits = ce_select(A, row, &t);
    if (t < 0 && !A.ce_scale) continue;
    const float v0 = c0 ? ot[rl * ldq + lane] : -INFINITY;
    const float v1 = c1 ? ot[rl * ldq + lane + 64] : -INFINITY;
    float best = v0;
    int arg = c0 ? lane : INT32_MAX;
    if (v1 > best) { best = v1; arg = lane + 64; }
#pragma unroll
    for (int off = 32; off > 0; off >>= 1) {
      const float ob = __shfl_xor(best, off);
      const int oa = __shfl_xor(arg, off);
      if (ob > best || (ob == best && oa < arg)) { best = ob; arg = oa; }
    }
    float se = (c0 ? expf(v0 - best) : 0.f) + (c1 ? expf(v1 - best) : 0.f);
#pragma unroll
    for (int off = 32; off > 0; off >>= 1) se += __shfl_xor(se, off);
    const float lse = best + logf(se);
    if (t >= 0 && A.ce_term) {
      if (lane == 0) {
        A.ce_term[row] = lse - ot[rl * ldq + t];
        A.ce_hit[row] = arg == t ? 1 : 0;
      }
    } else if (t >= 0) {
      const double term = (double)(lse - ot[rl * ldq + t]);
      const int h = arg == t ? 1 : 0;
      if (bits & 1) {
        nll += term;
        cnt += 1;
        hit += h;
      }
      if (bits & 2) {
        nll2 += term;
        cnt2 += 1;
        hit2 += h;
      }
    }
    if (A.ce_scale) {
      float* orow = A.out + (int64_t)row * A.ldo;
      if (c0) nt_store1(&orow[lane], t >= 0 ? sc * (expf(v0 - lse) - (lane == t ? 1.f : 0.f)) : 0.f);
      if (c1) nt_store1(&orow[lane + 64], t >= 0 ? sc * (expf(v1 - lse) - (lane + 64 == t ? 1.f : 0.f)) : 0.f);
    }
  }
  if (A.ce_term) return;
  __shared__ double cew[4][6];
  if (lane == 0) {
    cew[wave][0] = nll;
    cew[wave][1] = (double)cnt;
    cew[wave][2] = (double)hit;
    cew[wave][3] = nll2;
    cew[wave][4] = (double)cnt2;
    cew[wave][5] = (double)hit2;
  }
  __syncthreads();
  if ((int)threadIdx.x < W) {
    const int k = threadIdx.x;
    A.ce_part[(int64_t)tile * W + k] = (cew[0][k] + cew[1][k]) + (cew[2][k] + cew[3][k]);
  }
}


__device__ __forceinline__ double block_tree_sum(double v, double* sh) {
  sh[threadIdx.x] = v;
  __syncthreads();
  for (int off = 128; off > 0; off >>= 1) {
    if ((int)threadIdx.x < off) sh[threadIdx.x] += sh[threadIdx.x + off];
    __syncthreads();
  }
  const double r = sh[0];
  __syncthreads();
  return r;
}

__global__ void __launch_bounds__(256)
ce_tiles_gather_kernel(const double* __restrict__ part, int n_tiles, double* __restrict__ part2, int W) {
  __shared__ double sh[256];
  const int per = (n_tiles + gridDim.x - 1) / gridDim.x;
  const int b0 = blockIdx.x * per, b1 = min(n_tiles, b0 + per);
  for (int k = 0; k < W; ++k) {
    double v = 0.0;
    for (int b = b0 + threadIdx.x; b < b1; b += 256) v += part[(int64_t)b * W + k];
    v = block_tree_sum(v, sh);
    if (threadIdx.x == 0) part2[blockIdx.x * W + k] = v;
  }
}

__global__ void __launch_bounds__(256)
ce_tiles_finish_kernel(const double* __restrict__ part2, int n, double* __restrict__ stats, int W) {
  __shared__ double sh[256];
  for (int k = 0; k < W; ++k) {
    const double v = block_tree_sum((int)threadIdx.x < n ? part2[threadIdx.x * W + k] : 0.0, sh);
    if (threadIdx.x == 0) stats[k] = v;
  }
}

__global__ void __launch_bounds__(256) ce_row_records_kernel(const FusedArgs A, int tiles) {
  const int tid = blockIdx.x * 256 + threadIdx.x;
  const int b = tid >> 2, w = tid & 3;
  double v[3] = {0.0, 0.0, 0.0};
  if (b < tiles) {
    double nll = 0.0;
    int cnt = 0, hit = 0;
    for (int rr = 0; rr < TM / 4; ++rr) {
      const int row = b * TM + w * (TM / 4) + rr;
      if (row >= A.N) break;
      int t;
      if (ce_select(A, row, &t)) {
        nll += (double)A.ce_term[row];
        cnt += 1;
        hit += A.ce_hit[row];
      }
    }
    v[0] = nll, v[1] = (double)cnt, v[2] = (double)hit;
  }
#pragma unroll
  for (int k = 0; k < 3; ++k) {
    const double pair = v[k] + __shfl_xor(v[k], 1);
    const double rec = pair + __shfl_xor(pair, 2);
    if (w == 0 && b < tiles) A.ce_part[(int64_t)b * 3 + k] = rec;
  }
}

template <int G, bool HAS_W, int KC, int NT, bool CE = false, bool DENSE = false, bool BLK = false, bool POS = false,
          bool SEL = false>
__global__ void __launch_bounds__(256, POS ? 7 : (NT == 2 ? 5 : 8)) spmm_linear_kernel(const FusedArgs A) {
  constexpr int NG = kWave / G;
  constexpr int U = 4;
  extern __shared__ float zt[];
  const int K = KC ? KC : A.K;
  const int ldz = K + 4;
  const int lane = threadIdx.x & 63, wave = threadIdx.x >> 6;
  const int g = lane / G, t = lane % G;
  const int c = t * 4;
  const bool active = c < K;
  const int row_base = blockIdx.x * TM;

  __shared__ int next_row;
  if constexpr (DENSE) {
    const int k4 = K >> 2;
    for (int idx = threadIdx.x; idx < TM * k4; idx += 256) {
      const int r = idx / k4, c4 = (idx - r * k4) * 4;
      const int row = row_base + r;
      float v[4] = {0.f, 0.f, 0.f, 0.f};
      if (row < A.N) {
        load_vec<4>(v, blocked_at(A.x, BLK ? A.x_bc : 0, A.x_bs, A.ldx, row, c4));
        if (A.pre_scale) {
          float ps[4], pt[4];
          load_vec<4>(ps, A.pre_scale + c4);
          load_vec<4>(pt, A.pre_shift + c4);
          const float rsum = A.pre_rowsum[row];
#pragma unroll
          for (int i = 0; i < 4; ++i) v[i] = fmaf(v[i], ps[i], pt[i] * rsum);
        }
        if (A.z_out) store_vec<4>(A.z_out + (int64_t)row * A.ldz + c4, v);
      }
      store_vec<4>(&zt[r * ldz + c4], v);
    }
  }
  if (!DENSE && threadIdx.x == 0) next_row = 0;
  if constexpr (!DENSE) __syncthreads();
  while (!DENSE) {
    int lr = 0;
    if (lane == 0) lr = atomicAdd(&next_row, 1);
    lr = __builtin_amdgcn_readfirstlane(lr);
    if (lr >= TM) break;
    const int row = tile_row<CE>(A, row_base, lr);
    if constexpr (CE && !POS && !DENSE) {
      if (A.ce_term) ce_fill_gaps(A, row_base + lr, row, lane);
    }
    float acc[4] = {0.f, 0.f, 0.f, 0.f};
    float accp[4] = {0.f, 0.f, 0.f, 0.f};
    bool skip = false;
    if constexpr (CE && !POS) {
      if (A.ce_skip && row < A.N) {
        int t;
        skip = ce_select(A, row, &t) == 0;
      }
    }
    if (row < A.N && !skip) {
      const int start = __builtin_amdgcn_readfirstlane(A.rowptr[row]);
      const int end = __builtin_amdgcn_readfirstlane(A.rowptr[row + 1]);
      if (A.threshold > 0 && end - start > A.threshold) {
        int lo = 0, hi = A.n_long - 1;
        while (lo < hi) {
          const int mid = (lo + hi) >> 1;
          if (A.long_row[mid] < row) lo = mid + 1;
          else hi = mid;
        }
        if (g == 0 && active) {
          load_vec<4>(acc, A.zlong + (int64_t)lo * K + c);
          if constexpr (POS) load_vec<4>(accp, A.zlong_pos + (int64_t)lo * K + c);
        }
      } else {
        const float* xc = A.x + c;
        for (int base = start; base < end; base += kWave) {
          const int n = min(kWave, end - base);
          int mycol = 0;
          float myw = 0.f, mywp = 0.f;
          if (lane < n) {
            mycol = A.col[base + lane];
            if constexpr (HAS_W) myw = A.w[base + lane];
            if constexpr (POS) mywp = A.w2[base + lane];
            if constexpr (SEL) { if (!A.col_sel[mycol]) mycol = -1; }
          }
          for (int k = 0; k < n; k += NG * U) {
            float v[U][4];
            float ww[U];
            float wp[POS ? U : 1];
#pragma unroll
            for (int u = 0; u < U; ++u) {
              const int idx = k + u * NG + g;
              const int src = __shfl(mycol, idx & 63);
              if constexpr (HAS_W) ww[u] = __shfl(myw, idx & 63);
              if constexpr (POS) wp[u] = __shfl(mywp, idx & 63);
              const bool ok = active && idx < n && (!SEL || src >= 0);
#pragma unroll
              for (int i = 0; i < 4; ++i) v[u][i] = 0.f;
              if (ok) load_vec<4>(v[u], xc + (int64_t)src * A.ldx);
              if constexpr (HAS_W) { if (!ok) ww[u] = 0.f; }
              if constexpr (POS) { if (!ok) wp[u] = 0.f; }
            }
#pragma unroll
            for (int u = 0; u < U; ++u) {
#pragma unroll
              for (int i = 0; i < 4; ++i) {
                if constexpr (HAS_W) acc[i] = fmaf(ww[u], v[u][i], acc[i]);
                else acc[i] += v[u][i];
                if constexpr (POS) accp[i] = fmaf(wp[u], v[u][i], accp[i]);
              }
            }
          }
        }
#pragma unroll
        for (int off = 32; off >= G; off >>= 1) {
#pragma unroll
          for (int i = 0; i < 4; ++i) acc[i] += __shfl_xor(acc[i], off);
          if constexpr (POS) {
#pragma unroll
            for (int i = 0; i < 4; ++i) accp[i] += __shfl_xor(accp[i], off);
          }
        }
        if (A.rs) {
          const float s = A.rs[row];
#pragma unroll
          for (int i = 0; i < 4; ++i) acc[i] *= s;
        }
      }
    }
    if (g == 0 && active) {
      if (A.pre_scale && row < A.N && !skip) {
        float ps[4], pt[4];
        load_vec<4>(ps, A.pre_scale + c);
        load_vec<4>(pt, A.pre_shift + c);
        const float rsum = A.pre_rowsum[row];
#pragma unroll
        for (int i = 0; i < 4; ++i) acc[i] = fmaf(acc[i], ps[i], pt[i] * rsum);
      }
      store_vec<4>(&zt[lr * ldz + c], acc);
      if (A.z_out && row < A.N) nt_store4(A.z_out + (int64_t)row * A.ldz + c, acc);
      if constexpr (POS) {
        if (row < A.N) store_vec<4>(A.zpos_out + (int64_t)row * A.ldz + c, accp);
      }
    }
  }
  const int kr = lane >> 5, cc = lane & 31;
  float bpre[KB];
  const bool pre = KC > 0 && NT > 0 && wave < 4 && wave * 32 < A.Nout;
  if constexpr (KC > 0) {
    if (pre) load_b_batch(bpre, A.wt, A.Nout, wave * 32, 0, kr, cc);
  }
  constexpr bool kRootRegs = KC > 0 && KC <= 128 && NT > 0;
  constexpr int kRootVecs = kRootRegs ? (TM * (KC / 4)) / 256 : 1;
  float rootv[kRootVecs][4];
  if constexpr (kRootRegs) {
    if (A.xr) {
#pragma unroll
      for (int j = 0; j < kRootVecs; ++j) {
        const int idx = threadIdx.x + j * 256;
        const int r = idx / (KC / 4), c4 = (idx - r * (KC / 4)) * 4;
        const int row = tile_row<CE>(A, row_base, r);
#pragma unroll
        for (int i = 0; i < 4; ++i) rootv[j][i] = 0.f;
        if (row < A.N) {
          load_vec<4>(rootv[j], blocked_at(A.xr, BLK ? A.xr_bc : 0, A.xr_bs, A.ldr, row, c4));
          if (A.pre_scale) {
            float ps[4], pt[4];
            load_vec<4>(ps, A.pre_scale + c4);
            load_vec<4>(pt, A.pre_shift + c4);
#pragma unroll
            for (int i = 0; i < 4; ++i) rootv[j][i] = fmaf(rootv[j][i], ps[i], pt[i]);
          }
        }
      }
    }
  }
  __syncthreads();

  if (NT == 0) {
    if (wave >= 4) return;
    for (int n0 = wave * 32; n0 < A.Nout; n0 += 4 * 32) {
      f32x16 acc;
#pragma unroll
      for (int r = 0; r < 16; ++r) acc[r] = 0.f;
      tile_times_wt<KC>(acc, zt, ldz, A.wt, K, A.Nout, n0, kr, cc);
      store_tile<BLK>(acc, A.bias, A.out, A.ldo, row_base, A.N, n0, kr, cc, A.stats_part, A.Nout, A.out_blk, A.ob_c, A.ob_s);
    }
    return;
  }
  constexpr int NTT = NT > 0 ? NT : 1;
  f32x16 acc[NTT];
#pragma unroll
  for (int tt = 0; tt < NTT; ++tt) {
#pragma unroll
    for (int r = 0; r < 16; ++r) acc[tt][r] = 0.f;
    const int n0 = wave * 32 + tt * 128;
    if (wave < 4 && n0 < A.Nout)
      tile_times_wt<KC>(acc[tt], zt, ldz, A.wt, K, A.Nout, n0, kr, cc, pre && tt == 0 ? &bpre : nullptr);
  }
  if (!A.xr) {
    if constexpr (CE) {
      ce_epilogue(A, acc[0], zt, row_base, wave, lane);
      return;
    }
    if (wave >= 4) return;
#pragma unroll
    for (int tt = 0; tt < NTT; ++tt) {
      const int n0 = wave * 32 + tt * 128;
      if (n0 < A.Nout) store_tile<BLK>(acc[tt], A.bias, A.out, A.ldo, row_base, A.N, n0, kr, cc, A.stats_part, A.Nout, A.out_blk,
                                  A.ob_c, A.ob_s);
    }
    return;
  }
  __syncthreads();
  if constexpr (kRootRegs) {
#pragma unroll
    for (int j = 0; j < kRootVecs; ++j) {
      const int idx = threadIdx.x + j * 256;
      const int r = idx / (KC / 4), c4 = (idx - r * (KC / 4)) * 4;
      store_vec<4>(&zt[r * ldz + c4], rootv[j]);
    }
  } else {
    const int k4 = K >> 2;
    for (int idx = threadIdx.x; idx < TM * k4; idx += 256) {
      const int r = idx / k4, c4 = (idx - r * k4) * 4;
      const int row = tile_row<CE>(A, row_base, r);
      float v[4] = {0.f, 0.f, 0.f, 0.f};
      if (row < A.N) {
        load_vec<4>(v, blocked_at(A.xr, BLK ? A.xr_bc : 0, A.xr_bs, A.ldr, row, c4));
        if (A.pre_scale) {
          float ps[4], pt[4];
          load_vec<4>(ps, A.pre_scale + c4);
          load_vec<4>(pt, A.pre_shift + c4);
#pragma unroll
          for (int i = 0; i < 4; ++i) v[i] = fmaf(v[i], ps[i], pt[i]);
        }
      }
      store_vec<4>(&zt[r * ldz + c4], v);
    }
  }
  __syncthreads();
  if constexpr (CE) {
    if (wave * 32 < A.Nout) tile_times_wt<KC>(acc[0], zt, ldz, A.wtr, K, A.Nout, wave * 32, kr, cc);
    ce_epilogue(A, acc[0], zt, row_base, wave, lane);
    return;
  }
  if (wave >= 4) return;
#pragma unroll
  for (int tt = 0; tt < NTT; ++tt) {
    const int n0 = wave * 32 + tt * 128;
    if (n0 < A.Nout) {
      tile_times_wt<KC>(acc[tt], zt, ldz, A.wtr, K, A.Nout, n0, kr, cc);
      store_tile<BLK>(acc[tt], A.bias, A.out, A.ldo, row_base, A.N, n0, kr, cc, A.stats_part, A.Nout, A.out_blk,
                                  A.ob_c, A.ob_s);
    }
  }
}

__device__ __forceinline__ void park4(float* __restrict__ row, int c4, const float (&v)[4]) {
  float* p = row + (c4 & ~7) + ((c4 & 4) >> 1);
  const bool swap = (c4 & 32) != 0;
  const float2 even = make_float2(v[0], v[2]), odd = make_float2(v[1], v[3]);
  *reinterpret_cast<float2*>(swap ? p + 4 : p) = swap ? odd : even;
  *reinterpret_cast<float2*>(swap ? p : p + 4) = swap ? even : odd;
}

template <int KC>
__device__ __forceinline__ void stream_tile_mfma(f32x16& acc, const float* __restrict__ zt, const float (&breg)[KC / 2],
                                                 int kr, int cc) {
  constexpr int ldz = KC + 4;
#pragma unroll
  for (int j = 0; j < KC / 8; ++j) {
    const float4 a = *reinterpret_cast<const float4*>(&zt[cc * ldz + 8 * j + 4 * kr]);
    acc = __builtin_amdgcn_mfma_f32_32x32x2f32(a.x, breg[4 * j], acc, 0, 0, 0);
    acc = __builtin_amdgcn_mfma_f32_32x32x2f32(a.y, breg[4 * j + 1], acc, 0, 0, 0);
    acc = __builtin_amdgcn_mfma_f32_32x32x2f32(a.z, breg[4 * j + 2], acc, 0, 0, 0);
    acc = __builtin_amdgcn_mfma_f32_32x32x2f32(a.w, breg[4 * j + 3], acc, 0, 0, 0);
  }
}

template <int KC, int NT, bool CE, bool ROOT>
__global__ void __launch_bounds__(256, ROOT || NT > 1 ? 2 : (CE || KC > 64 ? 3 : 4)) dense_stream_kernel(const FusedArgs A, int tiles) {
  extern __shared__ float zt[];
  constexpr int ldz = KC + 4, k4 = KC / 4, S = KC / 2;
  constexpr bool PIPE = !CE && NT == 1;
  constexpr int VPT = (TM * k4) / 256;
  static_assert((TM * k4) % 256 == 0, "tile loads are spread evenly over the workgroup");
  const int lane = threadIdx.x & 63, wave = threadIdx.x >> 6;
  const int kr = lane >> 5, cc = lane & 31;
  float breg[NT][S];
  float rreg[ROOT ? NT : 1][ROOT ? S : 1];
#pragma unroll
  for (int tt = 0; tt < NT; ++tt) {
    const int n0 = wave * 32 + tt * 128;
    if (n0 < A.Nout) {
#pragma unroll
      for (int i = 0; i < S; ++i) {
// ... 147 lines not shown
    }
    __syncthreads();
  }
}

template <int KC>
bool launch_dense_stream(const FusedArgs& A, hipStream_t s) {
  const int tiles = (int)cdiv(A.N, TM);
  const bool root = A.xr != nullptr;
  const int nt = A.Nout <= 128 ? 1 : 2;
  if (A.Nout > 256 || (root && nt == 2)) return false;
  if (A.ce_part) return false;
  const int per_cu = (root || nt > 1) ? 2 : (KC > 64 ? 3 : 4);
  const int slots = 256 * per_cu;
  const int grid = tiles <= slots ? tiles : (int)cdiv(tiles, cdiv(tiles, slots));
  const size_t lds2 = 2 * (size_t)TM * (KC + 4) * sizeof(float);
  if (nt == 1) {
    if (root) {
      static const hipError_t allow = hipFuncSetAttribute(
          reinterpret_cast<const void*>(&dense_stream_kernel<KC, 1, false, true>),
          hipFuncAttributeMaxDynamicSharedMemorySize, (int)(2 * lds2));
      if (allow != hipSuccess) return false;
      dense_stream_kernel<KC, 1, false, true><<<grid, 256, 2 * lds2, s>>>(A, tiles);
    }
    else dense_stream_kernel<KC, 1, false, false><<<grid, 256, lds2, s>>>(A, tiles);
  } else {
    dense_stream_kernel<KC, 2, false, false><<<grid, 256, lds2, s>>>(A, tiles);
  }
  return true;
}

template <int G, int KC, bool DENSE = false>
int launch(const FusedArgs& A, hipStream_t s) {
  const int64_t blocks = A.ce_rows ? cdiv(A.ce_n_rows, TM) : cdiv(A.N, TM);
  if (blocks == 0) return RGBX_OK;
  const size_t lds = (size_t)TM * ((A.ce_part && A.Nout > A.K ? A.Nout : A.K) + 4) * sizeof(float);
  const int nt = A.Nout <= 128 ? 1 : (A.Nout <= 128 * NT_ROOT ? NT_ROOT : 0);
  const bool blk = DENSE || A.out_blk || A.xr_bc;
#define RGBX_FUSED(HW, NTV)                                                                      \
  do {                                                                                           \
    if (blk) spmm_linear_kernel<G, HW, KC, NTV, false, DENSE, true><<<(int)blocks, 256, lds, s>>>(A); \
    else spmm_linear_kernel<G, HW, KC, NTV, false, DENSE, DENSE><<<(int)blocks, 256, lds, s>>>(A);   \
  } while (0)
  if constexpr (!DENSE && KC > 0) {
    if (A.w2) {
      if (A.ce_part) spmm_linear_kernel<G, true, KC, 1, true, false, false, true><<<(int)blocks, 256, lds, s>>>(A);
      else spmm_linear_kernel<G, true, KC, 1, false, false, false, true><<<(int)blocks, 256, lds, s>>>(A);
      RGBX_CHECK_LAUNCH("spmm_linear_kernel (second aggregate)");
      return RGBX_OK;
    }
  }
  if constexpr (!DENSE && KC > 0) {
    if (A.col_sel && !blk && nt == 1) {
      if (A.w) spmm_linear_kernel<G, true, KC, 1, false, false, false, false, true><<<(int)blocks, 256, lds, s>>>(A);
      else spmm_linear_kernel<G, false, KC, 1, false, false, false, false, true><<<(int)blocks, 256, lds, s>>>(A);
      RGBX_CHECK_LAUNCH("spmm_linear_kernel (column selection)");
      return RGBX_OK;
    }
  }
  if (A.ce_part) {
    if (A.w && !DENSE) spmm_linear_kernel<G, !DENSE, KC, 1, true, DENSE, DENSE><<<(int)blocks, 256, lds, s>>>(A);
    else if (blk) spmm_linear_kernel<G, false, KC, 1, true, DENSE, true><<<(int)blocks, 256, lds, s>>>(A);
    else spmm_linear_kernel<G, false, KC, 1, true, DENSE, DENSE><<<(int)blocks, 256, lds, s>>>(A);
    RGBX_CHECK_LAUNCH("spmm_linear_kernel (cross-entropy epilogue)");
    return RGBX_OK;
  }
  if (A.w && !DENSE) {
    if (nt == 0) RGBX_FUSED(!DENSE, 0);
    else if (nt == 1) RGBX_FUSED(!DENSE, 1);
    else RGBX_FUSED(!DENSE, 2);
  } else {
    if (nt == 0) RGBX_FUSED(false, 0);
    else if (nt == 1) RGBX_FUSED(false, 1);
    else RGBX_FUSED(false, 2);
  }
#undef RGBX_FUSED
  RGBX_CHECK_LAUNCH("spmm_linear_kernel");
  return RGBX_OK;
}

}

int reduce_ce_tiles(double* scratch, int tiles, double* stats, int W, hipStream_t s) {
  double* part2 = scratch + (size_t)tiles * W;
  ce_tiles_gather_kernel<<<kCeGather, 256, 0, s>>>(scratch, tiles, part2, W);
  RGBX_CHECK_LAUNCH("ce_tiles_gather_kernel");
  ce_tiles_finish_kernel<<<1, 256, 0, s>>>(part2, kCeGather, stats, W);
  RGBX_CHECK_LAUNCH("ce_tiles_finish_kernel");
  return RGBX_OK;
}

int reduce_tile_stats(const float* part, int tiles, int width2, double* part2, double* sums, int64_t n_rows, hipStream_t s) {
  const int G = tiles < kStatsGather ? tiles : kStatsGather;
  tile_stats_gather_kernel<<<G, 256, 0, s>>>(part, tiles, width2, part2, (int)n_rows);
  RGBX_CHECK_LAUNCH("tile_stats_gather_kernel");
  tile_stats_finish_kernel<<<(int)cdiv(width2, 8), 256, 0, s>>>(part2, G, width2, sums);
  RGBX_CHECK_LAUNCH("tile_stats_finish_kernel");
  return RGBX_OK;
}

}

using namespace rgbx;

extern "C" int rgbx_spmm_linear_supported(int64_t K, int64_t Nout, int has_root) {
  return K >= 4 && K % 4 == 0 && K <= 256 && Nout >= 32 && Nout % 32 == 0 && (!has_root || Nout <= 128 * NT_ROOT);
}

extern "C" int rgbx_spmm_linear_f32(const int32_t* rowptr, const int32_t* col, const float* w, const float* rs,
                                    const float* x, int64_t ldx, const float* wt, const float* x_root, int64_t ldr,
                                    const float* wt_root, const float* bias, float* out, int64_t ldo, float* z_out,
                                    int64_t ldz, const float* pre_scale, const float* pre_shift,
                                    const float* pre_rowsum, double* out_colsums, void* stats_ws,
                                    size_t stats_ws_bytes, const rgbx_ce_epilogue_t* ce, int64_t N, int64_t K,
                                    int64_t Nout, const rgbx_row_split_t* split, rgbx_stream_t stream) {
  if (!rowptr) return fail(RGBX_E_ARG, "spmm_linear: null pointer");
  rgbx_fused_layer_t L{};
  L.rowptr = rowptr; L.col = col; L.w = w; L.rs = rs; L.x = x; L.ldx = ldx; L.wt = wt;
  L.x_root = x_root; L.ldr = ldr; L.wt_root = wt_root; L.bias = bias; L.out = out; L.ldo = ldo;
  L.z_out = z_out; L.ldz = ldz; L.pre_scale = pre_scale; L.pre_shift = pre_shift; L.pre_rowsum = pre_rowsum;
  L.out_colsums = out_colsums; L.stats_ws = stats_ws; L.stats_ws_bytes = stats_ws_bytes; L.ce = ce;
  L.N = N; L.K = K; L.Nout = Nout; L.split = split;
  return rgbx_fused_layer_f32(&L, stream);
}

extern "C" int rgbx_fused_layer_f32(const rgbx_fused_layer_t* Lp, rgbx_stream_t stream) {
  if (!Lp) return fail(RGBX_E_ARG, "fused_layer: null pointer");
  const rgbx_fused_layer_t& L = *Lp;
  const int64_t N = L.N, K = L.K, Nout = L.Nout;
  const rgbx_ce_epilogue_t* ce = L.ce;
  const bool dense = L.rowptr == nullptr;
  if (N < 0 || K <= 0 || Nout <= 0) return fail(RGBX_E_ARG, "spmm_linear: bad size");
  if (N == 0) return RGBX_OK;
  const bool stats_only = ce && !ce->grad_scale;
  if ((!dense && !L.col) || !L.x || !L.wt || (!L.out && !L.out_blk && !stats_only))
    return fail(RGBX_E_ARG, "spmm_linear: null pointer");
  if (ce) {
    if (!ce->y || !ce->stats || !ce->scratch) return fail(RGBX_E_ARG, "spmm_linear: incomplete cross-entropy epilogue");
    if (Nout > 128) return fail(RGBX_E_SHAPE, "spmm_linear: the cross-entropy epilogue needs Nout <= 128 (got %lld)", (long long)Nout);
    if (L.out_colsums) return fail(RGBX_E_ARG, "spmm_linear: out_colsums and the cross-entropy epilogue exclude each other");
    if (L.out_blk) return fail(RGBX_E_ARG, "spmm_linear: a blocked output and the cross-entropy epilogue exclude each other");
    if (ce->grad_scale && !L.out) return fail(RGBX_E_ARG, "spmm_linear: the loss gradient needs `out`");
    if (ce->mask_groups < 0 || ce->mask_groups > 2)
      return fail(RGBX_E_ARG, "spmm_linear: mask_groups must be 0, 1 or 2 (got %d)", (int)ce->mask_groups);
    if (ce->mask_groups == 2 && ce->grad_scale && (ce->rows || ce->n_rows))
      return fail(RGBX_E_ARG, "spmm_linear: a row list with the loss gradient excludes two statistics sets (mask_groups == 2)");
    if (ce->mask_groups == 2 && (ce->grad_scale || !ce->mask))
      return fail(RGBX_E_ARG, "spmm_linear: two statistics sets (mask_groups == 2) need a mask and no loss gradient");
    if (ce->rows || ce->n_rows) {
      if (!ce->rows || ce->n_rows < 0 || ce->n_rows > N)
        return fail(RGBX_E_ARG, "spmm_linear: row list of %lld rows for N = %lld", (long long)ce->n_rows, (long long)N);
      if (dense || L.w_pos)
        return fail(RGBX_E_ARG, "spmm_linear: a row list needs an aggregating launch (rowptr set) without w_pos");
      if (!ce->grad_scale && L.z_out)
        return fail(RGBX_E_ARG, "spmm_linear: a row list with z_out needs the loss gradient (grad_scale): the "
                                "statistics-only form leaves unlisted rows unwritten");
      if (ce->grad_scale && (!aligned16(L.out) || L.ldo % 4))
        return fail(RGBX_E_ALIGN, "spmm_linear: a row list with the loss gradient needs `out` 16-byte aligned with "
                                  "ldo %% 4 == 0");
    }
  }
  if (L.col_sel && (dense || ce || L.w_pos || L.out_blk || (L.x_root && L.xr_blk_cols > 0)))
    return fail(RGBX_E_ARG, "fused_layer: col_sel needs an aggregating launch without ce, w_pos or blocked layouts");
  if ((L.w_pos != nullptr) != (L.z_pos_out != nullptr))
    return fail(RGBX_E_ARG, "fused_layer: w_pos and z_pos_out go together");
  if (L.w_pos) {
    if (dense || !L.w || L.rs || L.pre_scale || L.out_blk || L.z_out == nullptr)
      return fail(RGBX_E_ARG, "fused_layer: w_pos needs an aggregating launch with w and z_out, without rs / pre_* / out_blk");
    if ((K != 64 && K != 128 && K != 256) || Nout > 128)
      return fail(RGBX_E_SHAPE, "fused_layer: w_pos needs K in {64, 128, 256} and Nout <= 128 (got K=%lld, Nout=%lld)",
                  (long long)K, (long long)Nout);
    if (!aligned16(L.z_pos_out)) return fail(RGBX_E_ALIGN, "fused_layer: z_pos_out must be 16-byte aligned");
  }
  if (N >= INT32_MAX) return fail(RGBX_E_RANGE, "spmm_linear: N exceeds int32");
  if ((L.x_root != nullptr) != (L.wt_root != nullptr))
    return fail(RGBX_E_ARG, "spmm_linear: x_root and wt_root go together");
  if ((L.pre_scale != nullptr) != (L.pre_shift != nullptr) || (L.pre_scale != nullptr) != (L.pre_rowsum != nullptr))
    return fail(RGBX_E_ARG, "spmm_linear: pre_scale, pre_shift and pre_rowsum go together");
  if (L.pre_scale && (!aligned16(L.pre_scale) || !aligned16(L.pre_shift)))
    return fail(RGBX_E_ALIGN, "spmm_linear: pre_scale / pre_shift must be 16-byte aligned");
  if (!rgbx_spmm_linear_supported(K, Nout, L.x_root != nullptr))
    return fail(RGBX_E_SHAPE,
                "spmm_linear: needs K %% 4 == 0, K <= 256, Nout %% 32 == 0, Nout <= 256 with a root term (got K=%lld, "
                "Nout=%lld)", (long long)K, (long long)Nout);
  const bool x_blk = dense && L.x_blk_cols > 0, xr_blk = L.x_root && L.xr_blk_cols > 0;
  if (!dense && L.x_blk_cols) return fail(RGBX_E_ARG, "fused_layer: a blocked x needs DENSE mode (rowptr == NULL)");
  if (!dense && xr_blk && ((ce && L.w) || L.w_pos))
    return fail(RGBX_E_ARG, "fused_layer: blocked root rows (xr_blk_cols) cannot be combined with per-slot weights plus "
                            "the cross-entropy epilogue, or with w_pos, on an aggregating launch");
  if ((x_blk && (L.x_blk_cols % 4 || L.x_blk_stride % 4 || K % L.x_blk_cols)) ||
      (xr_blk && (L.xr_blk_cols % 4 || L.xr_blk_stride % 4 || K % L.xr_blk_cols)) ||
      (L.out_blk && (L.ob_cols <= 0 || Nout % L.ob_cols)))
    return fail(RGBX_E_ARG, "fused_layer: block widths must divide the matrix width (inputs: multiples of 4)");
  if ((!x_blk && L.ldx < K) || (L.out && L.ldo < Nout) || (L.z_out && L.ldz < K) || (L.x_root && !xr_blk && L.ldr < K))
    return fail(RGBX_E_ARG, "spmm_linear: leading dimension too small");
  if (!aligned16(L.x) || (!x_blk && L.ldx % 4) || (L.z_out && (!aligned16(L.z_out) || L.ldz % 4)) ||
      (L.x_root && (!aligned16(L.x_root) || (!xr_blk && L.ldr % 4))))
    return fail(RGBX_E_ALIGN, "spmm_linear: x / x_root / z_out must be 16-byte aligned with ld %% 4 == 0");
  float* stats_part = nullptr;
  double* stats_part2 = nullptr;
  if (L.out_colsums) {
    size_t need = 0;
    rgbx_spmm_linear_stats_workspace_bytes(N, Nout, &need);
    if (!L.stats_ws || L.stats_ws_bytes < need)
      return fail(RGBX_E_WS, "spmm_linear: statistics workspace %zu < %zu bytes", L.stats_ws_bytes, need);
    if (reinterpret_cast<uintptr_t>(L.stats_ws) % 8) return fail(RGBX_E_ALIGN, "spmm_linear: stats_ws must be 8-byte aligned");
    stats_part2 = static_cast<double*>(L.stats_ws);
    stats_part = reinterpret_cast<float*>(stats_part2 + (size_t)kStatsGather * 2 * Nout);
  }
  hipStream_t s = (hipStream_t)stream;
  const int* long_row = nullptr;
  const float* zlong = nullptr;
  const float* zlong_pos = nullptr;
  int threshold = 0, n_long = 0;
  const rgbx_row_split_t* split = dense ? nullptr : L.split;
  if (split && split->threshold > 0 && split->n_chunks > 0) {
    float* zl = split->partial ? split->partial + (size_t)split->n_chunks * K : nullptr;
    if (int rc = spmm_long_rows_compact(L.rowptr, L.col, L.w, L.rs, L.x, L.ldx, (int)K, split, zl, s)) return rc;
    if (L.w_pos) {
      float* zlp = zl ? zl + (size_t)split->n_long * K : nullptr;
      if (int rc = spmm_long_rows_compact(L.rowptr, L.col, L.w_pos, L.rs, L.x, L.ldx, (int)K, split, zlp, s)) return rc;
      zlong_pos = zlp;
    }
    long_row = split->long_row;
    zlong = zl;
    threshold = split->threshold;
    n_long = split->n_long;
  }
  FusedArgs A{L.rowptr, L.col, L.w, L.rs, L.x, L.wt, L.x_root, L.wt_root, L.bias, L.out, L.z_out,
              L.ldx, L.ldo, L.ldz, L.ldr, long_row, zlong, threshold, n_long, (int)N, (int)K, (int)Nout,
              L.pre_scale, L.pre_shift, L.pre_rowsum, stats_part,
              ce ? ce->y : nullptr, ce ? ce->mask : nullptr, ce ? ce->grad_scale : nullptr, ce ? ce->scratch : nullptr,
              ce && ce->mask_groups == 2 ? 2 : 1,
              x_blk ? L.x_blk_cols : 0, L.x_blk_stride, xr_blk ? L.xr_blk_cols : 0, L.xr_blk_stride,
              L.out_blk, L.ob_cols, L.ob_stride, L.w_pos, L.z_pos_out, zlong_pos};
  A.col_sel = L.col_sel;
  if (ce) {
    A.ce_rows = ce->rows;
    A.ce_n_rows = (int)ce->n_rows;
    A.ce_skip = ce->skip_unselected ? 1 : 0;
    if (ce->rows && ce->grad_scale) {
      if (ce->n_rows == 0) {
        A.ce_rows = nullptr;
        A.ce_skip = 1;
      } else {
        double* behind = ce->scratch + (size_t)(cdiv(N, TM) + kCeGather) * 3;
        A.ce_term = reinterpret_cast<float*>(behind);
        A.ce_hit = reinterpret_cast<uint8_t*>(behind + cdiv(N, 2));
        A.ce_skip = 0;
      }
    }
  }
  const int64_t tiles = A.ce_rows && !A.ce_term ? cdiv(A.ce_n_rows, TM) : cdiv(N, TM);
  const int lanes = (int)(K / 4);
  int rc;
  if (dense) {
    if (K == 128 && launch_dense_stream<128>(A, s)) { RGBX_CHECK_LAUNCH("dense_stream_kernel"); rc = RGBX_OK; }
    else if (K == 64 && launch_dense_stream<64>(A, s)) { RGBX_CHECK_LAUNCH("dense_stream_kernel"); rc = RGBX_OK; }
    else if (K == 128) rc = launch<32, 128, true>(A, s);
    else if (K == 64) rc = launch<16, 64, true>(A, s);
    else if (K == 256) rc = launch<64, 256, true>(A, s);
    else rc = launch<32, 0, true>(A, s);
  }
  else if (K == 128) rc = launch<32, 128>(A, s);
  else if (K == 64) rc = launch<16, 64>(A, s);
  else if (K == 256) rc = launch<64, 256>(A, s);
  else if (lanes <= 1) rc = launch<1, 0>(A, s);
  else if (lanes <= 2) rc = launch<2, 0>(A, s);
  else if (lanes <= 4) rc = launch<4, 0>(A, s);
  else if (lanes <= 8) rc = launch<8, 0>(A, s);
  else if (lanes <= 16) rc = launch<16, 0>(A, s);
  else if (lanes <= 32) rc = launch<32, 0>(A, s);
  else rc = launch<64, 0>(A, s);
  if (rc) return rc;
  if (A.ce_term) {
    ce_row_records_kernel<<<(int)cdiv(tiles * 4, 256), 256, 0, s>>>(A, (int)tiles);
    RGBX_CHECK_LAUNCH("ce_row_records_kernel");
  }
  if (ce) {
    if (int rc2 = reduce_ce_tiles(ce->scratch, (int)tiles, ce->stats, ce->mask_groups == 2 ? 6 : 3, s)) return rc2;
  }
  if (!L.out_colsums) return RGBX_OK;
  return reduce_tile_stats(stats_part, (int)cdiv(N, TM), (int)(2 * Nout), stats_part2, L.out_colsums, N, s);
}

extern "C" int rgbx_ce_rows_grad_scratch_doubles(int64_t N, int64_t* count) {
  if (!count || N < 0) return fail(RGBX_E_ARG, "ce_rows_grad_scratch_doubles: bad argument");
  *count = (cdiv(N, TM) + kCeGather) * 3 + cdiv(N, 2) + cdiv(N, 8);
  return RGBX_OK;
}

extern "C" int rgbx_spmm_linear_stats_workspace_bytes(int64_t N, int64_t Nout, size_t* bytes) {
  if (!bytes || N < 0 || Nout <= 0) return fail(RGBX_E_ARG, "spmm_linear_stats_workspace_bytes: bad argument");
  *bytes = (size_t)kStatsGather * 2 * (size_t)Nout * sizeof(double) + (size_t)cdiv(N, TM) * 2 * (size_t)Nout * sizeof(float);
  return RGBX_OK;
}
```

rgb_experiment_amd/ops.py:

```python
import ctypes

import torch

from . import _lib

_EVENT_SINK = None


def set_event_sink(sink):
    global _EVENT_SINK
    _EVENT_SINK = sink


class Kind(str):
    variant = None


class _Timed:
    def __init__(self, kind, variant=None):
        if variant is not None and _EVENT_SINK is not None:
            kind = Kind(kind)
            kind.variant = variant
        self.kind = kind

# ... 650 lines not shown
    _WEIGHTS_EPOCH[0] += 1


def weights_epoch():
    return _WEIGHTS_EPOCH[0]


from torch.optim.optimizer import register_optimizer_step_post_hook as _register_step_post_hook

_register_step_post_hook(note_weights_changed)


class _MadeOn:
    __slots__ = ("value", "stream", "event")

    def __init__(self, value):
        self.value, self.stream, self.event = value, None, None
        if value.is_cuda and not torch.cuda.is_current_stream_capturing():
            self.stream = torch.cuda.current_stream(value.device)
            self.event = torch.cuda.Event()
            self.event.record(self.stream)

    def get(self):
        if self.event is not None:
            cur = torch.cuda.current_stream(self.value.device)
            if cur != self.stream and not torch.cuda.is_current_stream_capturing():
                cur.wait_event(self.event)
                self.value.record_stream(cur)
        return self.value


def weight_t(weight):
    w = weight.detach()
    if not isinstance(weight, torch.nn.Parameter) or (w.is_cuda and torch.cuda.is_current_stream_capturing()):
        return w.t().contiguous()
    tag = (weight._version, _WEIGHTS_EPOCH[0], w.data_ptr(), tuple(w.shape))
    cached = getattr(weight, "_rgbx_wt", None)
    if cached is None or cached[0] != tag:
        cached = (tag, _MadeOn(w.t().contiguous()))
        weight._rgbx_wt = cached
    return cached[1].get()


def _blocked(t, what):
    if (t.dtype != torch.float32 or t.dim() != 3 or (t.size(2) > 1 and t.stride(2) != 1)
            or (t.size(1) > 1 and t.stride(1) != t.size(2))):
        raise RuntimeError(f"{what}: expected a float32 [blocks, rows, cols] tensor with contiguous blocks, got "
                           f"{t.dtype} {tuple(t.shape)} strides {t.stride()}")
    return t.data_ptr(), t.size(2), t.stride(0)


def fused_layer(x, wt, csr=None, w=None, rs=None, bias=None, x_root=None, wt_root=None, pre=None, want_out=True,
                out_blocked=None, want_z=False, want_colsums=False, ce=None, kind="linear", out=None, z=None, w_pos=None,
                select_rows=False, col_sel=None):
    _lib.require_device(x, wt, bias, x_root, wt_root, out_blocked, col_sel)
    lib = _lib.load()
    L = _lib.FusedLayer()
    dense = csr is None
    if x.dim() == 3:
        if not dense:
            raise RuntimeError("fused_layer: a blocked x needs DENSE mode (no csr)")
        L.x, L.x_blk_cols, L.x_blk_stride = _blocked(x, "x")
        n_rows, K = x.size(1), x.size(0) * x.size(2)
    else:
        x = x if x.stride(-1) == 1 else x.contiguous()
        L.x, L.ldx = x.data_ptr(), x.stride(0) if x.size(0) > 1 else x.size(1)
        n_rows, K = x.size(0), x.size(1)
    N = n_rows if dense else csr.N
    wt = wt.contiguous()
    n_out = wt.size(1)
    if wt.size(0) != K:
        raise RuntimeError(f"fused_layer: wt is {tuple(wt.shape)}, the input width is {K}")
    keep = [x, wt]
    L.wt = wt.data_ptr()
    if not dense:
        L.rowptr, L.col, L.w, L.rs = _lib.ptr(csr.rowptr), _lib.ptr(csr.col), _lib.ptr(w), _lib.ptr(rs)
        if col_sel is not None:
            if col_sel.dtype != torch.uint8 or col_sel.numel() < x.size(0):
                raise RuntimeError(f"fused_layer: col_sel must be uint8 with an entry per input row, got {col_sel.dtype} "
                                   f"{tuple(col_sel.shape)} for {x.size(0)} rows")
            col_sel = col_sel.contiguous()
            keep.append(col_sel)
            L.col_sel = col_sel.data_ptr()
        split, _scratch = csr.split_arg(K, x.device, hub_rows=2 if w_pos is not None else 1)
        keep.append(_scratch)
        if split is not None:
            keep.append(split)
            L.split = ctypes.addressof(split)
    if wt_root is not None:
        wtr = wt_root.contiguous()
        keep.append(wtr)
        L.wt_root = wtr.data_ptr()
        if x_root.dim() == 3:
            L.x_root, L.xr_blk_cols, L.xr_blk_stride = _blocked(x_root, "x_root")
        else:
            xr = x_root if x_root.stride(-1) == 1 else x_root.contiguous()
            keep.append(xr)
            L.x_root, L.ldr = xr.data_ptr(), xr.stride(0) if xr.size(0) > 1 else xr.size(1)
    if bias is not None:
        b = bias.contiguous()
        keep.append(b)
        L.bias = b.data_ptr()
    if pre is not None:
        ps, pt, pr = (t.contiguous() for t in pre)
        keep += [ps, pt, pr]
        L.pre_scale, L.pre_shift, L.pre_rowsum = ps.data_ptr(), pt.data_ptr(), pr.data_ptr()
    ce_stats = None
    groups = 1
    if ce is not None:
        y, mask, grad_scale = ce
        if isinstance(mask, (tuple, list)):
            if grad_scale is not None:
                raise RuntimeError("fused_layer: two masks are for statistics only (no loss gradient)")
            mask, groups = group_masks(*mask), 2
        _lib.require_device(y, mask, grad_scale)
        if y.dtype != torch.int64:
            raise RuntimeError(f"labels must be int64, got {y.dtype}")
        if mask is not None and mask.dtype not in (torch.bool, torch.uint8):
            raise RuntimeError(f"mask must be bool, got {mask.dtype}")
        y = y.contiguous()
        mask = None if mask is None else mask.contiguous()
        ce_stats = torch.empty(3 * groups, dtype=torch.float64, device=x.device)
        scratch_doubles = 3 * groups * ((N + 31) // 32 + 64)
        rows = None
        if select_rows and not dense and w_pos is None and mask is not None:
            if grad_scale is not None:
                if CE_GRAD_ROW_LIST and (out is None or (out.data_ptr() % 16 == 0 and (N == 1 or out.stride(0) % 4 == 0))):
                    rows = selected_rows(y, mask, n_out)
                    if rows is not None and rows.numel() == 0:
                        rows = None
            elif not want_z and z is None:
                rows = selected_rows(y, mask, n_out)
        if rows is not None and grad_scale is not None:
            count = ctypes.c_int64(0)
            _lib.check(lib.rgbx_ce_rows_grad_scratch_doubles(N, ctypes.byref(count)), "rgbx_ce_rows_grad_scratch_doubles")
            scratch_doubles = count.value
        ce_scratch = torch.empty(scratch_doubles, dtype=torch.float64, device=x.device)
        ce_arg = _lib.CeEpilogue(_lib.ptr(y), _lib.ptr(mask), _lib.ptr(grad_scale), _lib.ptr(ce_stats),
                                 _lib.ptr(ce_scratch), groups)
        if rows is not None:
            ce_arg.rows, ce_arg.n_rows = rows.data_ptr(), rows.numel()
            keep.append(rows)
        elif select_rows and not dense and w_pos is None and grad_scale is not None:
            ce_arg.skip_unselected = 1
        keep += [y, mask, ce_scratch, ce_arg]
        L.ce = ctypes.addressof(ce_arg)
        want_out = grad_scale is not None
    if out is not None:
        if tuple(out.shape) != (N, n_out) or out.stride(1) != 1 or out.dtype != torch.float32:
            raise RuntimeError(f"fused_layer: out is {tuple(out.shape)}, expected a float32 [{N}, {n_out}] with contiguous rows")
    elif want_out:
        out = torch.empty((N, n_out), dtype=torch.float32, device=x.device)
    if out is not None:
        L.out, L.ldo = out.data_ptr(), out.stride(0) if N > 1 else n_out
    else:
        L.ldo = n_out
    if out_blocked is not None:
        L.out_blk, L.ob_cols, L.ob_stride = _blocked(out_blocked, "out_blocked")
        if out_blocked.size(1) != N or out_blocked.size(0) * out_blocked.size(2) != n_out:
            raise RuntimeError(f"fused_layer: out_blocked is {tuple(out_blocked.shape)} for a [{N}, {n_out}] output")
    if z is not None:
        if tuple(z.shape) != (N, K) or z.stride(1) != 1 or z.dtype != torch.float32:
            raise RuntimeError(f"fused_layer: z is {tuple(z.shape)}, expected a float32 [{N}, {K}] with contiguous rows")
    elif want_z or w_pos is not None:
        z = torch.empty((N, K), dtype=torch.float32, device=x.device)
    L.ldz = K
    if z is not None:
        L.z_out, L.ldz = z.data_ptr(), z.stride(0) if N > 1 else K
    z_pos = None
    if w_pos is not None:
        _lib.require_device(w_pos)
        z_pos = torch.empty_strided((N, K), (L.ldz, 1), dtype=torch.float32, device=x.device)
        keep.append(w_pos)
        L.w_pos, L.z_pos_out = w_pos.data_ptr(), z_pos.data_ptr()
    colsums = None
    if want_colsums:
        nbytes = ctypes.c_size_t(0)
        _lib.check(lib.rgbx_spmm_linear_stats_workspace_bytes(N, n_out, ctypes.byref(nbytes)),
                   "rgbx_spmm_linear_stats_workspace_bytes")
        ws = torch.empty(max(nbytes.value, 8), dtype=torch.uint8, device=x.device)
        colsums = torch.empty((2, n_out), dtype=torch.float64, device=x.device)
        keep.append(ws)
        L.out_colsums, L.stats_ws, L.stats_ws_bytes = colsums.data_ptr(), ws.data_ptr(), nbytes.value
    L.N, L.K, L.Nout = N, K, n_out
    variant = None
    if _EVENT_SINK is not None:
        variant = "+".join([name for name, on in (
            ("dense", dense), ("pre", pre is not None), ("root", wt_root is not None), ("z", z is not None),
            ("zpos", w_pos is not None), ("stats", want_colsums), ("ce_stats", ce is not None and ce[2] is None),
            ("ce_grad", ce is not None and ce[2] is not None), ("noout", out is None and out_blocked is None and ce is None),
            ("blk", out_blocked is not None)) if on]) or "plain"
    with _Timed(kind, variant):
        _lib.check(lib.rgbx_fused_layer_f32(ctypes.byref(L), _lib.stream_ptr()), "rgbx_fused_layer_f32")
    del keep
    if groups == 2:
        ce_stats = ce_stats.view(2, 3)
    return out, (z if w_pos is None else (z, z_pos)), (ce_stats if ce is not None else colsums)


def blocked_to_rows(src, out=None, bias=None):
    _lib.require_device(src, bias)
    ptr, bc, bs = _blocked(src, "src")
    n, d = src.size(1), src.size(0) * src.size(2)
    if out is None:
        out = torch.empty((n, d), dtype=torch.float32, device=src.device)
    b = None if bias is None else bias.detach().contiguous()
    _lib.check(_lib.load().rgbx_blocked_to_rows_f32(ptr, bc, bs, out.data_ptr(), out.stride(0), n, d, _lib.ptr(b),
                                                    _lib.stream_ptr()), "rgbx_blocked_to_rows_f32")
    return out


def spmm_linear_raw(csr, w, rs, x, wt, bias=None, want_z=False, x_root=None, wt_root=None, kind="linear", pre=None,
                    want_colsums=False, ce=None, select_rows=False):
    out, z, extra = fused_layer(x, wt, csr=csr, w=w, rs=rs, bias=bias, x_root=x_root if wt_root is not None else None,
                                wt_root=wt_root, pre=pre, want_z=want_z, want_colsums=want_colsums, ce=ce, kind=kind,
                                select_rows=select_rows)
    if ce is not None or want_colsums:
        return out, z, extra
    return out, z


class _AggregateLinear(torch.autograd.Function):

    @staticmethod
    def forward(ctx, z, weight, bias, root_weight, x_root, want_colsums):
        out, _, cs = fused_layer(z, weight_t(weight), bias=None if bias is None else bias.detach(),
                                 x_root=x_root if root_weight is not None else None,
                                 wt_root=None if root_weight is None else weight_t(root_weight),
                                 want_colsums=want_colsums, kind="cached_aggregate_linear_fwd")
        ctx.save_for_backward(z, x_root if root_weight is not None else None)
        ctx.has_bias = bias is not None
        if want_colsums:
            ctx.mark_non_differentiable(cs)
            return out, cs
        return out

    @staticmethod
    def backward(ctx, gy, _g_cs=None):
        z, x_root = ctx.saved_tensors
        gy = gy.contiguous()
        gw = gb = gwr = None
        want_b = ctx.has_bias and ctx.needs_input_grad[2]
        if ctx.needs_input_grad[1]:
            if want_b:
                gw, gb = gemm_tn(gy, z, colsum=True)
            else:
                gw = gemm_tn(gy, z)
        elif want_b:
            gb = gy.sum(0)
        if x_root is not None and ctx.needs_input_grad[3]:
            gwr = gemm_tn(gy, x_root)
        return None, gw, gb, gwr, None, None


def aggregate_linear_ok(in_channels, out_channels, root=False):
    return bool(_lib.load().rgbx_spmm_linear_supported(in_channels, out_channels, int(root)))


def aggregate_linear(z, weight, bias=None, root_weight=None, x_root=None, want_colsums=False):
    return _tag_colsums(_AggregateLinear.apply(z, weight, bias, root_weight, x_root, want_colsums), want_colsums)


def fold_bn_linear(weight, bias=None, bias2=None, root_weight=None, bn=None):
    _lib.require_device(weight, bias, bias2, root_weight)
    W = weight.detach()
    W = W if W.stride(-1) == 1 else W.contiguous()
    n_out, K = W.shape
    Wr = None
    if root_weight is not None:
        Wr = root_weight.detach()
        Wr = Wr if Wr.stride(-1) == 1 else Wr.contiguous()
    wt = torch.empty((K, n_out), dtype=torch.float32, device=W.device)
    wrt = torch.empty_like(wt) if Wr is not None else None
    has_b = bias is not None or bias2 is not None or bn is not None
    b_out = torch.empty(n_out, dtype=torch.float32, device=W.device) if has_b else None
    c = lambda t: None if t is None else t.detach().contiguous()
    b1, b2 = c(bias), c(bias2)
    g = be = rm = rv = None
    eps = 0.0
    if bn is not None:
        g, be, rm, rv, eps = c(bn.weight), c(bn.bias), c(bn.running_mean), c(bn.running_var), bn.eps
    _lib.check(_lib.load().rgbx_fold_bn_linear_f32(
        _lib.ptr(W), W.stride(0), _lib.ptr(Wr), 0 if Wr is None else Wr.stride(0), _lib.ptr(b1), _lib.ptr(b2),
        _lib.ptr(g), _lib.ptr(be), _lib.ptr(rm), _lib.ptr(rv), float(eps), _lib.ptr(wt), _lib.ptr(wrt), _lib.ptr(b_out),
        n_out, K, _lib.stream_ptr()), "rgbx_fold_bn_linear_f32")
    return wt, b_out, wrt


FUSE_DENSE_BACKWARD = True
CE_GRAD_ROW_LIST = True

BN_HANDOVER = "_rgbx_bn_handover"


class BNHandover:
    __slots__ = ("bn", "mean", "rstd", "n", "reduce")

    def __init__(self, bn):
        self.bn, self.mean, self.rstd, self.n, self.reduce = bn, None, None, None, None

    def fill(self, mean, rstd, n, reduce):
        self.mean, self.rstd, self.n, self.reduce = mean, rstd, n, reduce


def _take_handover(x, bn):
    rec = getattr(x, BN_HANDOVER, None)
    if rec is None or rec.bn is not bn or rec.mean is not None or not x.requires_grad or not FUSE_DENSE_BACKWARD:
        return None
    return rec


class _PropagateLinear(torch.autograd.Function):

    @staticmethod
    def forward(ctx, x, graph, kind, weight, bias, need_z=True, root_weight=None, x_root=None, want_colsums=False,
                bn_weight=None, bn_bias=None, handover=None):
        x = x.contiguous()
        xr = x if x_root is None else x_root.contiguous()
        w = graph.w if kind == "gcn" else None
        rs = graph.inv_deg if kind == "mean" else None
        if kind not in ("gcn", "mean", "sum"):
            raise ValueError(kind)
        res = spmm_linear_raw(graph.fwd, w, rs, x, weight_t(weight), None if bias is None else bias.detach(),
                              need_z, xr if root_weight is not None else None,
                              None if root_weight is None else weight_t(root_weight),
                              kind=f"{getattr(graph, 'event_prefix', '')}{kind}_linear_fwd", want_colsums=want_colsums)
        out, z = res[0], res[1]
        ctx.save_for_backward(z, weight, root_weight, xr if root_weight is not None else None,
                              bn_weight if handover is not None else None, out if handover is not None else None)
        ctx.graph, ctx.kind, ctx.has_bias, ctx.handover = graph, kind, bias is not None, handover
        if want_colsums:
            ctx.mark_non_differentiable(res[2])
            return out, res[2]
        return out

    @staticmethod
    def backward(ctx, gy, _g_colsums=None):
        z, weight, root_weight, x, bn_weight, y = ctx.saved_tensors
        g, kind = ctx.graph, ctx.kind
        gy = gy.contiguous()
        gx = gw = gb = gwr = g_bnw = g_bnb = None
        want_b = ctx.has_bias and ctx.needs_input_grad[4]
        rec, bn_a = ctx.handover, None
        if rec is not None and rec.mean is not None:
            from .nn import batchnorm as B
            ca, cb, ck, g_bnw, g_bnb = B.train_backward_coefficients(gy, y, bn_weight, rec.mean, rec.rstd, rec.n,
                                                                     rec.reduce)
            if (ctx.needs_input_grad[0] or (root_weight is not None and ctx.needs_input_grad[6])
                    or not ctx.needs_input_grad[3]):
                gy = B.bwd_apply(gy, y, rec.mean, rec.rstd, ca, cb, ck)
            else:
                bn_a = (y, rec.mean, rec.rstd, ca, cb, ck)
        if bn_a is not None:
            gw, gb = gemm_tn_bn_bwd(gy, *bn_a, z, colsum=want_b)
        elif ctx.needs_input_grad[3]:
            if want_b:
                gw, gb = gemm_tn(gy, z, colsum=True)
            else:
                gw = gemm_tn(gy, z)
        elif want_b:
            gb = gy.sum(0)
        if root_weight is not None and ctx.needs_input_grad[6]:
            gwr = gemm_tn(gy, x)
        if ctx.needs_input_grad[0]:
            gx = _propagate_linear_input_grad(g, kind, gy, weight, root_weight)
        return gx, None, None, gw, gb, None, gwr, None, None, g_bnw, g_bnb, None


def _propagate_linear_input_grad(g, kind, gy, weight, root_weight, ce_sel=None):
    csr = g.bwd
    wt = {"gcn": lambda: g.w_t, "mean": lambda: g.w_mean_t, "sum": lambda: None}[kind]()
    prefix = getattr(g, "event_prefix", "")
    n_out, n_in = weight.shape
    if n_out <= n_in and _lib.load().rgbx_spmm_linear_supported(n_out, n_in, int(root_weight is not None)):
        gx, _, _ = fused_layer(gy, weight.detach().contiguous(), csr=csr, w=wt,
                               x_root=gy if root_weight is not None else None,
                               wt_root=None if root_weight is None else root_weight.detach().contiguous(),
                               col_sel=None if ce_sel is None else selected_cols(*ce_sel), kind=f"{prefix}{kind}_linear_bwd")
        return gx
    gz = gy @ weight
    gr = gy @ root_weight if root_weight is not None else None
    if gr is None:
        return spmm_raw(csr, wt, None, gz, kind=f"{prefix}{kind}_bwd")
    return spmm_raw(csr, wt, None, gz, y=gr, a=1.0, b=1.0, out=gr, kind=f"{prefix}{kind}_bwd")


class _BNPropagateLinear(torch.autograd.Function):

    @staticmethod
    def forward(ctx, x, bn_weight, bn_bias, graph, kind, weight, bias, root_weight, eps, reduce, running, need_z,
                colsums=None, want_colsums=False, handover=None):
        from .nn import batchnorm as B
        x = x.contiguous()
        mean, rstd, scale, shift, n = B.train_statistics(x, bn_weight, bn_bias, eps, reduce, running, colsums)
        if handover is not None:
            handover.fill(mean, rstd, n, reduce)
        ctx.handed_over = handover is not None
        w, rs = (graph.w, None) if kind == "gcn" else (None, graph.inv_deg)
        res = spmm_linear_raw(graph.fwd, w, rs, x, weight_t(weight), None if bias is None else bias.detach(), need_z,
                              x if root_weight is not None else None,
                              None if root_weight is None else weight_t(root_weight), kind=f"{kind}_linear_fwd",
                              pre=(scale, shift, graph.rowsum(kind)), want_colsums=want_colsums)
        out, z = res[0], res[1]
        ctx.save_for_backward(x, bn_weight, mean, rstd, n, z, weight, root_weight, scale, shift)
        ctx.graph, ctx.kind, ctx.has_bias, ctx.reduce = graph, kind, bias is not None, reduce
        if want_colsums:
            ctx.mark_non_differentiable(res[2])
            return out, res[2]
        return out

    @staticmethod
    def backward(ctx, gy, _g_colsums=None):
        from .nn import batchnorm as B
        x, bn_weight, mean, rstd, n, z, weight, root_weight, scale, shift = ctx.saved_tensors
        g, kind = ctx.graph, ctx.kind
        gy = gy.contiguous()
        gw = gb = gwr = None
        if ctx.needs_input_grad[5]:
            gw, gcol = gemm_tn(gy, z, colsum=True)
            gb = gcol if ctx.has_bias and ctx.needs_input_grad[6] else None
        else:
            gcol = gy.sum(0)
            gb = gcol if ctx.has_bias and ctx.needs_input_grad[6] else None
        if root_weight is not None and ctx.needs_input_grad[7]:
            gwr = gemm_tn(gy, x) * scale + gcol[:, None] * shift
        g_h = _propagate_linear_input_grad(g, kind, gy, weight, root_weight)
# ... 32 lines not shown
        hit = (_MadeOn(g), mask_a, mask_b)
        _GROUP_MASKS[key] = hit
        while len(_GROUP_MASKS) > 16:
            _GROUP_MASKS.pop(next(iter(_GROUP_MASKS)))
    return hit[0].get()


def ce_selection(y, mask, C):
    sel = (y >= 0) & (y < C)
    if mask is not None:
        sel = sel & mask.bool()
    return sel


def _sel_key(y, mask, C):
    return (y.data_ptr(), y._version, y.numel(),
            None if mask is None else (mask.data_ptr(), mask._version, mask.numel()), int(C))


_SEL_ROWS = {}


def selected_rows(y, mask, C):
    key = _sel_key(y, mask, C)
    hit = _SEL_ROWS.get(key)
    if hit is None:
        if torch.cuda.is_current_stream_capturing():
            return None
        rows = ce_selection(y, mask, C).nonzero().reshape(-1).to(torch.int32).contiguous()
        hit = (_MadeOn(rows), y, mask)
        _SEL_ROWS[key] = hit
        while len(_SEL_ROWS) > 16:
            _SEL_ROWS.pop(next(iter(_SEL_ROWS)))
    return hit[0].get()


_SEL_COLS = {}


def selected_cols(y, mask, C):
    key = _sel_key(y, mask, C)
    hit = _SEL_COLS.get(key)
    if hit is None:
        if torch.cuda.is_current_stream_capturing():
            return None
        hit = (_MadeOn(ce_selection(y, mask, C).to(torch.uint8).contiguous()), y, mask)
        _SEL_COLS[key] = hit
        while len(_SEL_COLS) > 16:
            _SEL_COLS.pop(next(iter(_SEL_COLS)))
    return hit[0].get()



def ce_from_logits(logits, y, mask):
    if isinstance(mask, (tuple, list)):
        return None, torch.stack([masked_ce_accuracy(logits, y, m) for m in mask])
    if torch.is_grad_enabled() and logits.requires_grad:
        return masked_ce_loss(logits, y, mask, with_stats=True)
    stats = masked_ce_accuracy(logits, y, mask)
    return (stats[0] / stats[1]).float(), stats


def fused_ce_ok(graph, in_channels, out_channels, root, x, y):
    return (not _is_dist(graph) and out_channels <= 128 and y is not None and y.is_cuda and y.dtype == torch.int64
            and fused_linear_ok(graph, in_channels, out_channels, root=root, x=x))


class _PropagateLinearCE(torch.autograd.Function):

    @staticmethod
    def forward(ctx, x, graph, kind, weight, bias, root_weight, y, mask, want_grad, bn_weight, bn_bias, bn_args):
        from .nn import batchnorm as B
        x = x.contiguous()
        pre = None
        if bn_weight is not None:
            eps, reduce, running, colsums, handover = bn_args
            mean, rstd, scale, shift, n = B.train_statistics(x, bn_weight, bn_bias, eps, reduce, running, colsums)
            pre = (scale, shift, graph.rowsum(kind))
            if handover is not None:
                handover.fill(mean, rstd, n, reduce)
        ctx.handed_over = bn_weight is not None and bn_args[4] is not None
        w, rs = (graph.w, None) if kind == "gcn" else (None, graph.inv_deg)
        grad_scale = mask_scale(y, mask, weight.size(0)) if want_grad else None
        dlogits, z, stats = spmm_linear_raw(
            graph.fwd, w, rs, x, weight_t(weight), None if bias is None else bias.detach(),
            want_grad and weight.requires_grad, x if root_weight is not None else None,
            None if root_weight is None else weight_t(root_weight), kind=f"{kind}_linear_fwd", pre=pre,
            ce=(y, mask, grad_scale), select_rows=True)
        ctx.graph, ctx.kind, ctx.has_bias, ctx.has_bn = graph, kind, bias is not None, bn_weight is not None
        ctx.ce_sel = (y, mask, weight.size(0)) if want_grad else None
        if want_grad:
            if ctx.has_bn:
                ctx.save_for_backward(dlogits, z, weight, root_weight, x, bn_weight, mean, rstd, n, scale, shift)
                ctx.reduce = bn_args[1]
            else:
                ctx.save_for_backward(dlogits, z, weight, root_weight, x if root_weight is not None else None)
        ctx.mark_non_differentiable(stats)
        if stats.dim() == 2:
            return stats.new_zeros(()).float(), stats
        return (stats[0] / stats[1]).float(), stats

    @staticmethod
    def backward(ctx, g, _g_stats):
        from .nn import batchnorm as B
        saved = ctx.saved_tensors
        if ctx.has_bn:
            gy, z, weight, root_weight, x, bn_weight, mean, rstd, n, scale, shift = saved
        else:
            gy, z, weight, root_weight, x = saved
        graph, kind = ctx.graph, ctx.kind
        g = g.reshape(()).float()
        gw = gb = gwr = gx = g_bnw = g_bnb = None
        gcol = None
        if ctx.needs_input_grad[3]:
            rows = selected_rows(*ctx.ce_sel) if FUSE_DENSE_BACKWARD else None
            gw, gcol = gemm_tn_rows(gy, z, rows, colsum=True)
        if ctx.has_bias and ctx.needs_input_grad[4]:
            gb = gcol if gcol is not None else gy.sum(0)
        if root_weight is not None and ctx.needs_input_grad[5]:
            if ctx.has_bn:
                gcol = gcol if gcol is not None else gy.sum(0)
                gwr = gemm_tn(gy, x) * scale + gcol[:, None] * shift
            else:
                gwr = gemm_tn(gy, x)
        need_h = ctx.needs_input_grad[0] or (ctx.has_bn and (ctx.needs_input_grad[9] or ctx.needs_input_grad[10]))
        items = [(k, t) for k, t in (("gw", gw), ("gb", gb), ("gwr", gwr)) if t is not None]
        if need_h:
            items.append(("w", weight.detach()))
            if root_weight is not None:
                items.append(("wr", root_weight.detach()))
        sc = dict(zip((k for k, _ in items), torch._foreach_mul([t for _, t in items], g))) if items else {}
        gw, gb, gwr = sc.get("gw"), sc.get("gb"), sc.get("gwr")
        if need_h:
            g_h = _propagate_linear_input_grad(graph, kind, gy, sc["w"], sc.get("wr"), ce_sel=ctx.ce_sel)
            if ctx.has_bn and not ctx.handed_over:
                gx, g_bnw, g_bnb = B.train_backward(g_h, x, bn_weight, mean, rstd, n, ctx.reduce)
            else:
                gx = g_h
        return gx, None, None, gw, gb, gwr, None, None, None, g_bnw, g_bnb, None


def propagate_linear_ce(x, graph, kind, weight, bias, root_weight, y, mask, bn=None, colsums=None):
    want_grad = not isinstance(mask, (tuple, list)) and torch.is_grad_enabled() and any(
        t is not None and t.requires_grad
        for t in (weight, x, bias, root_weight) + ((bn.weight, bn.bias) if bn is not None else ()))
    if bn is not None:
        bn_args = (bn.eps, bn._reduce, bn.begin_training_step(), colsums, _take_handover(x, bn) if want_grad else None)
        return _PropagateLinearCE.apply(x, graph, kind, weight, bias, root_weight, y, mask, want_grad, bn.weight, bn.bias,
                                        bn_args)
    return _PropagateLinearCE.apply(x, graph, kind, weight, bias, root_weight, y, mask, want_grad, None, None, None)


def bn_propagate_linear(x, bn, graph, kind, weight, bias=None, root_weight=None, colsums=None, want_colsums=False):
    need_z = weight.requires_grad
    return _tag_colsums(_BNPropagateLinear.apply(x, bn.weight, bn.bias, graph, kind, weight, bias, root_weight, bn.eps,
                                                 bn._reduce, bn.begin_training_step(), need_z, colsums, want_colsums,
                                                 _take_handover(x, bn)),
                        want_colsums)


COLSUMS = "_rgbx_colsums"


def _tag_colsums(res, want_colsums):
    if not want_colsums:
        return res
    out, colsums = res
    setattr(out, COLSUMS, colsums)
    return out


def propagate_linear(x, graph, kind, weight, bias=None, root_weight=None, want_colsums=False, next_bn=None):
    if _is_dist(graph):
        return graph.propagate_linear(x, kind, weight, bias, root_weight)
    need_z = torch.is_grad_enabled() and weight.requires_grad
    if next_bn is None or not FUSE_DENSE_BACKWARD or not torch.is_grad_enabled():
        return _tag_colsums(_PropagateLinear.apply(x, graph, kind, weight, bias, need_z, root_weight, None, want_colsums),
                            want_colsums)
    rec = BNHandover(next_bn)
    out = _tag_colsums(_PropagateLinear.apply(x, graph, kind, weight, bias, need_z, root_weight, None, want_colsums,
                                              next_bn.weight, next_bn.bias, rec), want_colsums)
    setattr(out, BN_HANDOVER, rec)
    return out


def appnp_raw(csr, w, h, K, alpha, kind="appnp"):
    _lib.require_device(h)
# ... 1327 lines not shown
        a, b = (_aligned_rows(t) for t in (a, b))
    pa, lda = _lib.mat(a, "a")
    pb, ldb = _lib.mat(b, "b")
    K, M, N = a.size(0), a.size(1), b.size(1)
    lib = _lib.load()
    nbytes = ctypes.c_size_t(0)
    _lib.check(lib.rgbx_gemm_tn_workspace_bytes(K, M, N, ctypes.byref(nbytes)), "rgbx_gemm_tn_workspace_bytes")
    ws = torch.empty(max(nbytes.value, 1), dtype=torch.uint8, device=a.device)
    if out is None:
        out = torch.empty((M, N), dtype=torch.float32, device=a.device)
    elif tuple(out.shape) != (M, N) or not out.is_contiguous() or out.dtype != torch.float32:
        raise RuntimeError(f"gemm_tn: out must be a contiguous float32 [{M}, {N}] tensor")
    sums = None
    if colsum:
        sums = sums_out if sums_out is not None else torch.empty(M, dtype=torch.float32, device=a.device)
        if tuple(sums.shape) != (M,) or not sums.is_contiguous() or sums.dtype != torch.float32:
            raise RuntimeError(f"gemm_tn: sums_out must be a contiguous float32 [{M}] tensor")
    with _Timed("gemm_tn", f"{M}x{N}" if _EVENT_SINK is not None else None):
        _lib.check(lib.rgbx_gemm_tn_f32(pa, lda, pb, ldb, _lib.ptr(out), N, _lib.ptr(sums), K, M, N, float(alpha),
                                        _lib.ptr(ws), ws.numel(), _lib.stream_ptr()), "rgbx_gemm_tn_f32")
    return (out, sums) if colsum else out


def _gemm_tn_v4(*mats):
    return all(t.is_cuda and t.dtype == torch.float32 and t.dim() == 2 and t.stride(1) == 1 and t.size(1) % 4 == 0
               and t.stride(0) % 4 == 0 and t.stride(0) >= t.size(1) and t.data_ptr() % 16 == 0 for t in mats)


def _gemm_tn_buffers(K, M, N, device, colsum):
    nbytes = ctypes.c_size_t(0)
    _lib.check(_lib.load().rgbx_gemm_tn_workspace_bytes(K, M, N, ctypes.byref(nbytes)), "rgbx_gemm_tn_workspace_bytes")
    ws = torch.empty(max(nbytes.value, 1), dtype=torch.uint8, device=device)
    out = torch.empty((M, N), dtype=torch.float32, device=device)
    return ws, out, torch.empty(M, dtype=torch.float32, device=device) if colsum else None


def gemm_tn_bn_bwd(g, x, mean, rstd, ca, cb, ck, b, colsum=False):
    from .nn import batchnorm as B
    _lib.require_device(g, x, b)
    if not _gemm_tn_v4(g, x, b) or g.shape != x.shape:
        res = gemm_tn(B.bwd_apply(g, x, mean, rstd, ca, cb, ck), b, colsum=colsum)
        return res if colsum else (res, None)
    K, M, N = g.size(0), g.size(1), b.size(1)
    consts = [t.contiguous() for t in (mean, rstd, ca, cb, ck)]
    ws, out, sums = _gemm_tn_buffers(K, M, N, g.device, colsum)
    (pg, ldg), (px, ldx), (pb, ldb) = (_lib.mat(t, n) for t, n in ((g, "g"), (x, "x"), (b, "b")))
    with _Timed("gemm_tn", f"{M}x{N}+bn_bwd" if _EVENT_SINK is not None else None):
        _lib.check(_lib.load().rgbx_gemm_tn_bn_bwd_f32(
            pg, ldg, px, ldx, *(_lib.ptr(t) for t in consts), pb, ldb, _lib.ptr(out), N, _lib.ptr(sums), K, M, N, 1.0,
            _lib.ptr(ws), ws.numel(), _lib.stream_ptr()), "rgbx_gemm_tn_bn_bwd_f32")
    return out, sums


def gemm_tn_rows(a, b, rows, colsum=False):
    _lib.require_device(a, b)
    if rows is None or not _gemm_tn_v4(a, b) or a.size(0) != b.size(0) or a.size(0) >= 2**31:
        return gemm_tn(a, b, colsum=colsum)
    K, M, N = a.size(0), a.size(1), b.size(1)
    ws, out, sums = _gemm_tn_buffers(K, M, N, a.device, colsum)
    (pa, lda), (pb, ldb) = _lib.mat(a, "a"), _lib.mat(b, "b")
    with _Timed("gemm_tn", f"{M}x{N}+rows" if _EVENT_SINK is not None else None):
        _lib.check(_lib.load().rgbx_gemm_tn_rows_f32(
            pa, lda, pb, ldb, _lib.ptr(rows), rows.numel(), _lib.ptr(out), N, _lib.ptr(sums), K, M, N, 1.0,
            _lib.ptr(ws), ws.numel(), _lib.stream_ptr()), "rgbx_gemm_tn_rows_f32")
    return (out, sums) if colsum else out


class _Linear(torch.autograd.Function):

    @staticmethod
    def forward(ctx, x, weight, bias):
        ctx.save_for_backward(x, weight)
        ctx.has_bias = bias is not None
        if _EVENT_SINK is None or not x.is_cuda:
            return torch.nn.functional.linear(x, weight, bias)
        with _Timed("linear_fwd", f"{weight.size(1)}->{weight.size(0)}"):
            return torch.nn.functional.linear(x, weight, bias)

    @staticmethod
    def backward(ctx, gy):
        x, weight = ctx.saved_tensors
        gy = gy.contiguous()
        gx = gy @ weight if ctx.needs_input_grad[0] else None
        gw = gb = None
        want_b = ctx.has_bias and ctx.needs_input_grad[2]
        if ctx.needs_input_grad[1] and gy.is_cuda and want_b:
            gw, gb = gemm_tn(gy, x, colsum=True)
        else:
            if ctx.needs_input_grad[1]:
                gw = gemm_tn(gy, x) if gy.is_cuda else gy.t() @ x
            gb = gy.sum(0) if want_b else None
        return gx, gw, gb


def linear(x, weight, bias=None):
    sp = getattr(x, "_rgbx_sparse", None)
    if sp is not None and not x.requires_grad:
        return _SparseRowsLinear.apply(sp, weight, bias)
    return _Linear.apply(x, weight, bias)


SHORT_ROWS_TABLE_BYTES = 2 << 20
SHORT_ROWS_MEAN_SLOTS = 64


def short_rows_ok(csr, table):
    d = table.size(1)
    return (table.is_cuda and d % 4 == 0 and 4 <= d <= 64 and table.numel() * 4 <= SHORT_ROWS_TABLE_BYTES
            and csr.nnz <= SHORT_ROWS_MEAN_SLOTS * max(csr.N, 1))


def spmm_short_rows_raw(csr, w, x, bias=None, kind="spmm"):
    _lib.require_device(x, w, bias)
    px, ldx = _lib.mat(x, "x")
    N, d = csr.N, x.size(1)
    out = torch.empty((N, d), dtype=torch.float32, device=x.device)
    with _Timed(kind, f"shortrows+d{d}" if _EVENT_SINK is not None else None):
# ... 237 lines not shown
```

Baseline: 17.24 billion.

## Store CE logit gradients compactly for selected rows and remap backward gathers

Result: no change. 17.69 billion (median of 2 runs) (+2.6%).

```diff
diff --git a/include/rgbx_hip.h b/include/rgbx_hip.h
--- a/include/rgbx_hip.h
+++ b/include/rgbx_hip.h
@@ -153,6 +153,7 @@
   const int32_t* rows;
   int64_t n_rows;
   int32_t skip_unselected;
+  int32_t compact;
 } rgbx_ce_epilogue_t;
 
 int rgbx_spmm_linear_supported(int64_t K, int64_t Nout, int has_root);
@@ -198,6 +199,7 @@
   const float* w_pos;
   float* z_pos_out;
   const uint8_t* col_sel;
+  const int32_t* slot_src;
 } rgbx_fused_layer_t;
 
 int rgbx_fused_layer_f32(const rgbx_fused_layer_t* layer, rgbx_stream_t stream);
@@ -409,6 +411,13 @@
                           int64_t n_rows, float* C, int64_t ldc, float* a_colsum, int64_t K, int64_t M, int64_t N,
                           float alpha, void* workspace, size_t workspace_bytes, rgbx_stream_t stream);
 
+int rgbx_gemm_tn_rows_compact_f32(const float* A, int64_t lda, const float* B, int64_t ldb, const int32_t* rows,
+                                  int64_t n_rows, float* C, int64_t ldc, float* a_colsum, int64_t K, int64_t M,
+                                  int64_t N, float alpha, void* workspace, size_t workspace_bytes, rgbx_stream_t stream);
+
+int rgbx_slot_src_i32(const int32_t* col, int64_t nnz, const int32_t* pos, int64_t n_cols, int32_t* slot_src,
+                      rgbx_stream_t stream);
+
 
 int rgbx_bn_scratch_doubles(int64_t N, int64_t d, int64_t* count);
 
diff --git a/rgb_experiment_amd/_lib.py b/rgb_experiment_amd/_lib.py
--- a/rgb_experiment_amd/_lib.py
+++ b/rgb_experiment_amd/_lib.py
@@ -31,7 +31,8 @@
 class CeEpilogue(ctypes.Structure):
     _fields_ = [("y", ctypes.c_void_p), ("mask", ctypes.c_void_p), ("grad_scale", ctypes.c_void_p),
                 ("stats", ctypes.c_void_p), ("scratch", ctypes.c_void_p), ("mask_groups", ctypes.c_int32),
-                ("rows", ctypes.c_void_p), ("n_rows", ctypes.c_int64), ("skip_unselected", ctypes.c_int32)]
+                ("rows", ctypes.c_void_p), ("n_rows", ctypes.c_int64), ("skip_unselected", ctypes.c_int32),
+                ("compact", ctypes.c_int32)]
 
 
 class SpmmEpilogue(ctypes.Structure):
@@ -46,7 +47,7 @@
                 ("ldo", _I64), ("out_blk", _P), ("ob_cols", _I64), ("ob_stride", _I64), ("z_out", _P), ("ldz", _I64),
                 ("pre_scale", _P), ("pre_shift", _P), ("pre_rowsum", _P), ("out_colsums", _P), ("stats_ws", _P),
                 ("stats_ws_bytes", ctypes.c_size_t), ("ce", _P), ("N", _I64), ("K", _I64), ("Nout", _I64),
-                ("split", _P), ("w_pos", _P), ("z_pos_out", _P), ("col_sel", _P)]
+                ("split", _P), ("w_pos", _P), ("z_pos_out", _P), ("col_sel", _P), ("slot_src", _P)]
 
 
 SIGNATURES = {
@@ -142,6 +143,9 @@
     "rgbx_gemm_tn_bn_bwd_f32": [_P, _I64, _P, _I64, _P, _P, _P, _P, _P, _P, _I64, _P, _I64, _P, _I64, _I64, _I64, _F, _P,
                                 ctypes.c_size_t, _P],
     "rgbx_gemm_tn_rows_f32": [_P, _I64, _P, _I64, _P, _I64, _P, _I64, _P, _I64, _I64, _I64, _F, _P, ctypes.c_size_t, _P],
+    "rgbx_gemm_tn_rows_compact_f32": [_P, _I64, _P, _I64, _P, _I64, _P, _I64, _P, _I64, _I64, _I64, _F, _P, ctypes.c_size_t,
+                                      _P],
+    "rgbx_slot_src_i32": [_P, _I64, _P, _I64, _P, _P],
     "rgbx_bn_scratch_doubles": [_I64, _I64, ctypes.POINTER(ctypes.c_int64)],
     "rgbx_bn_stats_f32": [_P, _I64, _I64, _I64, _P, _P, _I64, _P],
     "rgbx_bn_finalize_f32": [_P, _P, _P, _F, _F, _P, _P, _P, _P, _P, _P, _I64, _P],
diff --git a/rgb_experiment_amd/csrc/gemm.hip b/rgb_experiment_amd/csrc/gemm.hip
--- a/rgb_experiment_amd/csrc/gemm.hip
+++ b/rgb_experiment_amd/csrc/gemm.hip
@@ -4,7 +4,7 @@
 namespace {
 
 constexpr int BM = 128, BN = 128, KT = 32;
-enum { A_PLAIN = 0, A_BN = 1, A_ROWS = 2 };
+enum { A_PLAIN = 0, A_BN = 1, A_ROWS = 2, A_ROWS_LIST = 3 };
 
 struct TnExtra {
   const float* X;
@@ -199,6 +199,23 @@
       }
       consume();
     }
+  } else if constexpr (MODE == A_ROWS_LIST) {
+    const int64_t j_begin = lower_bound_rows(ex.rows, ex.n_rows, k_begin);
+    const int64_t j_end = lower_bound_rows(ex.rows, ex.n_rows, k_end);
+    float4 ra[KT * (MT / 4) / 256], rb[KT * 32 / 256];
+    fetch_tile<MT>(ra, A, lda, j_begin, j_end, m0, M);
+    fetch_tile<128>(rb, B, ldb, j_begin, j_end, n0, N);
+    for (int64_t j0 = j_begin; j0 < j_end; j0 += KT) {
+      __syncthreads();
+      put_tile<MT>(la, ra);
+      put_tile<128>(lb, rb);
+      __syncthreads();
+      if (j0 + KT < j_end) {
+        fetch_tile<MT>(ra, A, lda, j0 + KT, j_end, m0, M);
+        fetch_tile<128>(rb, B, ldb, j0 + KT, j_end, n0, N);
+      }
+      consume();
+    }
   } else if constexpr (VEC4) {
     float4 ra[KT * (MT / 4) / 256], rb[KT * 32 / 256];
     fetch_tile<MT>(ra, A, lda, k_begin, k_end, m0, M);
@@ -301,7 +318,7 @@
     if (ex.ldx < M) return fail(RGBX_E_ARG, "%s: leading dimension too small", name);
     v4 = v4 && aligned16(ex.X) && ex.ldx % 4 == 0;
   }
-  if (mode == A_ROWS) {
+  if (mode == A_ROWS || mode == A_ROWS_LIST) {
     if (ex.n_rows < 0 || ex.n_rows > K || (ex.n_rows > 0 && !ex.rows)) return fail(RGBX_E_ARG, "%s: bad row list", name);
     if (K >= INT32_MAX) return fail(RGBX_E_RANGE, "%s: K exceeds int32", name);
   }
@@ -322,6 +339,7 @@
   gemm_tn_partial_kernel<V4, MT, MODE><<<grid, 256, 0, s>>>(A, lda, B, ldb, part, colpart, K, (int)M, (int)N, slab, ex)
   if (mode == A_BN) { if (mt == 64) RGBX_GEMM_TN(true, 64, A_BN); else RGBX_GEMM_TN(true, 128, A_BN); }
   else if (mode == A_ROWS) { if (mt == 64) RGBX_GEMM_TN(true, 64, A_ROWS); else RGBX_GEMM_TN(true, 128, A_ROWS); }
+  else if (mode == A_ROWS_LIST) { if (mt == 64) RGBX_GEMM_TN(true, 64, A_ROWS_LIST); else RGBX_GEMM_TN(true, 128, A_ROWS_LIST); }
   else if (v4) { if (mt == 64) RGBX_GEMM_TN(true, 64, A_PLAIN); else RGBX_GEMM_TN(true, 128, A_PLAIN); }
   else { if (mt == 64) RGBX_GEMM_TN(false, 64, A_PLAIN); else RGBX_GEMM_TN(false, 128, A_PLAIN); }
 #undef RGBX_GEMM_TN
@@ -368,3 +386,13 @@
   return run_gemm_tn("gemm_tn_rows", A_ROWS, A, lda, B, ldb, C, ldc, a_colsum, K, M, N, alpha, workspace,
                      workspace_bytes, stream, ex);
 }
+
+extern "C" int rgbx_gemm_tn_rows_compact_f32(const float* A, int64_t lda, const float* B, int64_t ldb, const int32_t* rows,
+                                             int64_t n_rows, float* C, int64_t ldc, float* a_colsum, int64_t K, int64_t M,
+                                             int64_t N, float alpha, void* workspace, size_t workspace_bytes,
+                                             rgbx_stream_t stream) {
+  TnExtra ex{};
+  ex.rows = rows, ex.n_rows = n_rows;
+  return run_gemm_tn("gemm_tn_rows_compact", A_ROWS_LIST, A, lda, B, ldb, C, ldc, a_colsum, K, M, N, alpha, workspace,
+                     workspace_bytes, stream, ex);
+}
diff --git a/rgb_experiment_amd/csrc/graph_prep.hip b/rgb_experiment_amd/csrc/graph_prep.hip
--- a/rgb_experiment_amd/csrc/graph_prep.hip
+++ b/rgb_experiment_amd/csrc/graph_prep.hip
@@ -109,6 +109,15 @@
   for (int64_t p = (int64_t)blockIdx.x * blockDim.x + threadIdx.x; p < nnz; p += (int64_t)gridDim.x * blockDim.x) {
     const int id = perm[p];
     ew_slot[p] = id < E ? ew[id] : loop_w[id - E];
+  }
+}
+
+__global__ void __launch_bounds__(256)
+slot_src_kernel(const int* __restrict__ col, int64_t nnz, const int* __restrict__ pos, int n_cols,
+                int* __restrict__ slot_src) {
+  for (int64_t p = (int64_t)blockIdx.x * blockDim.x + threadIdx.x; p < nnz; p += (int64_t)gridDim.x * blockDim.x) {
+    const int c = col[p];
+    slot_src[p] = (unsigned)c < (unsigned)n_cols ? pos[c] : -1;
   }
 }
 
@@ -356,3 +365,14 @@
   RGBX_CHECK_LAUNCH("gcn_norm_bwd_edge_kernel");
   return RGBX_OK;
 }
+
+extern "C" int rgbx_slot_src_i32(const int32_t* col, int64_t nnz, const int32_t* pos, int64_t n_cols, int32_t* slot_src,
+                                 rgbx_stream_t stream) {
+  if (nnz < 0 || n_cols < 0 || (nnz > 0 && (!col || !slot_src || (n_cols > 0 && !pos))))
+    return fail(RGBX_E_ARG, "slot_src: null pointer or negative size");
+  if (n_cols >= INT32_MAX) return fail(RGBX_E_RANGE, "slot_src: n_cols exceeds int32");
+  if (nnz == 0) return RGBX_OK;
+  slot_src_kernel<<<grid_for(nnz), 256, 0, (hipStream_t)stream>>>(col, nnz, pos, (int)n_cols, slot_src);
+  RGBX_CHECK_LAUNCH("slot_src_kernel");
+  return RGBX_OK;
+}
diff --git a/rgb_experiment_amd/csrc/spmm.hip b/rgb_experiment_amd/csrc/spmm.hip
--- a/rgb_experiment_amd/csrc/spmm.hip
+++ b/rgb_experiment_amd/csrc/spmm.hip
@@ -17,9 +17,10 @@
   int N, d;
   float a, b;
   int skip_longer;
+  const int* slot_src;
 };
 
-template <int G, int VEC, bool HAS_W>
+template <int G, int VEC, bool HAS_W, bool SLOT = false>
 __device__ __forceinline__ void accumulate_slots(const SpmmArgs& A, int start, int end, const float* xc,
                                                  bool active, int lane, int g, float (&acc)[VEC]) {
   constexpr int NG = kWave / G;
@@ -29,7 +30,7 @@
     int mycol = 0;
     float myw = 0.f;
     if (lane < n) {
-      mycol = A.col[base + lane];
+      mycol = SLOT ? A.slot_src[base + lane] : A.col[base + lane];
       if constexpr (HAS_W) myw = A.w[base + lane];
     }
     for (int k = 0; k < n; k += NG * U) {
@@ -40,7 +41,7 @@
         const int idx = k + u * NG + g;
         const int src = __shfl(mycol, idx & 63);
         if constexpr (HAS_W) ww[u] = __shfl(myw, idx & 63);
-        const bool ok = active && idx < n;
+        const bool ok = active && idx < n && (!SLOT || src >= 0);
 #pragma unroll
         for (int i = 0; i < VEC; ++i) v[u][i] = 0.f;
         if (ok) load_vec<VEC>(v[u], xc + (int64_t)src * A.ldx);
@@ -115,7 +116,7 @@
   }
 }
 
-template <int G, int VEC, bool HAS_W>
+template <int G, int VEC, bool HAS_W, bool SLOT = false>
 __global__ void __launch_bounds__(256)
 spmm_chunk_kernel(const SpmmArgs A, int n_chunks, const int* __restrict__ chunk_begin,
                   const int* __restrict__ chunk_end, float* __restrict__ partial) {
@@ -132,7 +133,7 @@
       float acc[VEC];
 #pragma unroll
       for (int i = 0; i < VEC; ++i) acc[i] = 0.f;
-      accumulate_slots<G, VEC, HAS_W>(A, start, end, A.x + c, active, lane, g, acc);
+      accumulate_slots<G, VEC, HAS_W, SLOT>(A, start, end, A.x + c, active, lane, g, acc);
       if (g == 0 && active) store_vec<VEC>(partial + (int64_t)ch * A.d + c, acc);
     }
   }
@@ -193,7 +194,11 @@
 int launch_long_compact(const SpmmArgs& A, const rgbx_row_split_t* sp, float* zlong, hipStream_t s) {
   int64_t cb = cdiv(sp->n_chunks, 4);
   if (cb > kMaxGrid) cb = kMaxGrid;
-  if (A.w)
+  if (A.slot_src && A.w)
+    spmm_chunk_kernel<G, 4, true, true><<<(int)cb, 256, 0, s>>>(A, sp->n_chunks, sp->chunk_begin, sp->chunk_end, sp->partial);
+  else if (A.slot_src)
+    spmm_chunk_kernel<G, 4, false, true><<<(int)cb, 256, 0, s>>>(A, sp->n_chunks, sp->chunk_begin, sp->chunk_end, sp->partial);
+  else if (A.w)
     spmm_chunk_kernel<G, 4, true><<<(int)cb, 256, 0, s>>>(A, sp->n_chunks, sp->chunk_begin, sp->chunk_end, sp->partial);
   else
     spmm_chunk_kernel<G, 4, false><<<(int)cb, 256, 0, s>>>(A, sp->n_chunks, sp->chunk_begin, sp->chunk_end, sp->partial);
@@ -485,13 +490,14 @@
 }
 
 int spmm_long_rows_compact(const int* rowptr, const int* col, const float* w, const float* rs, const float* x,
-                           int64_t ldx, int d, const rgbx_row_split_t* split, float* zlong, hipStream_t s) {
+                           int64_t ldx, int d, const rgbx_row_split_t* split, float* zlong, hipStream_t s,
+                           const int* slot_src) {
   if (!split || split->n_long <= 0 || split->n_chunks <= 0 || !split->chunk_begin || !split->chunk_end ||
       !split->long_row || !split->long_chunk_ptr || !split->partial || !zlong)
     return fail(RGBX_E_ARG, "spmm_long_rows: incomplete row-split plan");
   if (d % 4 || !aligned16(x) || ldx % 4 || !aligned16(split->partial) || !aligned16(zlong))
     return fail(RGBX_E_ALIGN, "spmm_long_rows: needs d %% 4 == 0 and 16-byte aligned x / partial / zlong");
-  SpmmArgs A{rowptr, col, w, rs, x, nullptr, nullptr, zlong, ldx, 0, d, 0, d, 1.0f, 0.0f, 0};
+  SpmmArgs A{rowptr, col, w, rs, x, nullptr, nullptr, zlong, ldx, 0, d, 0, d, 1.0f, 0.0f, 0, slot_src};
   const int lanes = d / 4;
   if (lanes <= 1) return launch_long_compact<1>(A, split, zlong, s);
   if (lanes <= 2) return launch_long_compact<2>(A, split, zlong, s);
diff --git a/rgb_experiment_amd/csrc/spmm_internal.h b/rgb_experiment_amd/csrc/spmm_internal.h
--- a/rgb_experiment_amd/csrc/spmm_internal.h
+++ b/rgb_experiment_amd/csrc/spmm_internal.h
@@ -4,7 +4,8 @@
 namespace rgbx {
 
 int spmm_long_rows_compact(const int* rowptr, const int* col, const float* w, const float* rs, const float* x,
-                           int64_t ldx, int d, const rgbx_row_split_t* split, float* zlong, hipStream_t s);
+                           int64_t ldx, int d, const rgbx_row_split_t* split, float* zlong, hipStream_t s,
+                           const int* slot_src = nullptr);
 
 constexpr int kTileRows = 32;
 constexpr int kCeGather = 64;
diff --git a/rgb_experiment_amd/csrc/spmm_linear.hip b/rgb_experiment_amd/csrc/spmm_linear.hip
--- a/rgb_experiment_amd/csrc/spmm_linear.hip
+++ b/rgb_experiment_amd/csrc/spmm_linear.hip
@@ -51,6 +51,8 @@
   float* ce_term;
   uint8_t* ce_hit;
   const uint8_t* col_sel;
+  int ce_compact;
+  const int* slot_src;
 };
 
 __device__ __forceinline__ const float* blocked_at(const float* base, int64_t bc, int64_t bs, int64_t ld, int row,
@@ -240,6 +242,7 @@
   }
 }
 
+template <bool LST = false>
 __device__ __forceinline__ void ce_epilogue(const FusedArgs& A, const f32x16& acc, float* __restrict__ ot, int row_base,
                                             int wave, int lane, int tile = -1) {
   if (tile < 0) tile = blockIdx.x;
@@ -261,7 +264,13 @@
   for (int rr = 0; rr < TM / 4; ++rr) {
     const int rl = wave * (TM / 4) + rr;
     const int row = tile_row<true>(A, row_base, rl);
-    if (row >= A.N) break;
+    if (row >= A.N) {
+      if (!LST || row_base + rl >= A.ce_n_rows) break;
+      float* orow = A.out + (int64_t)(row_base + rl) * A.ldo;
+      if (c0) nt_store1(&orow[lane], 0.f);
+      if (c1) nt_store1(&orow[lane + 64], 0.f);
+      continue;
+    }
     int t;
     const int bits = ce_select(A, row, &t);
     if (t < 0 && !A.ce_scale) continue;
@@ -300,7 +309,7 @@
       }
     }
     if (A.ce_scale) {
-      float* orow = A.out + (int64_t)row * A.ldo;
+      float* orow = A.out + (int64_t)(LST ? row_base + rl : row) * A.ldo;
       if (c0) nt_store1(&orow[lane], t >= 0 ? sc * (expf(v0 - lse) - (lane == t ? 1.f : 0.f)) : 0.f);
       if (c1) nt_store1(&orow[lane + 64], t >= 0 ? sc * (expf(v1 - lse) - (lane + 64 == t ? 1.f : 0.f)) : 0.f);
     }
@@ -385,7 +394,7 @@
 }
 
 template <int G, bool HAS_W, int KC, int NT, bool CE = false, bool DENSE = false, bool BLK = false, bool POS = false,
-          bool SEL = false>
+          int SEL = 0, bool LST = false>
 __global__ void __launch_bounds__(256, POS ? 7 : (NT == 2 ? 5 : 8)) spmm_linear_kernel(const FusedArgs A) {
   constexpr int NG = kWave / G;
   constexpr int U = 4;
@@ -429,7 +438,7 @@
     if (lr >= TM) break;
     const int row = tile_row<CE>(A, row_base, lr);
     if constexpr (CE && !POS && !DENSE) {
-      if (A.ce_term) ce_fill_gaps(A, row_base + lr, row, lane);
+      if (!LST && A.ce_term) ce_fill_gaps(A, row_base + lr, row, lane);
     }
     float acc[4] = {0.f, 0.f, 0.f, 0.f};
     float accp[4] = {0.f, 0.f, 0.f, 0.f};
@@ -461,10 +470,11 @@
           int mycol = 0;
           float myw = 0.f, mywp = 0.f;
           if (lane < n) {
-            mycol = A.col[base + lane];
+            if constexpr (SEL != 2) mycol = A.col[base + lane];
             if constexpr (HAS_W) myw = A.w[base + lane];
             if constexpr (POS) mywp = A.w2[base + lane];
-            if constexpr (SEL) { if (!A.col_sel[mycol]) mycol = -1; }
+            if constexpr (SEL == 1) { if (!A.col_sel[mycol]) mycol = -1; }
+            if constexpr (SEL == 2) mycol = A.slot_src[base + lane];
           }
           for (int k = 0; k < n; k += NG * U) {
             float v[U][4];
@@ -520,7 +530,11 @@
         for (int i = 0; i < 4; ++i) acc[i] = fmaf(acc[i], ps[i], pt[i] * rsum);
       }
       store_vec<4>(&zt[lr * ldz + c], acc);
-      if (A.z_out && row < A.N) nt_store4(A.z_out + (int64_t)row * A.ldz + c, acc);
+      if constexpr (LST) {
+        if (A.z_out && row_base + lr < A.ce_n_rows) nt_store4(A.z_out + (int64_t)(row_base + lr) * A.ldz + c, acc);
+      } else {
+        if (A.z_out && row < A.N) nt_store4(A.z_out + (int64_t)row * A.ldz + c, acc);
+      }
       if constexpr (POS) {
         if (row < A.N) store_vec<4>(A.zpos_out + (int64_t)row * A.ldz + c, accp);
       }
@@ -582,7 +596,7 @@
   }
   if (!A.xr) {
     if constexpr (CE) {
-      ce_epilogue(A, acc[0], zt, row_base, wave, lane);
+      ce_epilogue<LST>(A, acc[0], zt, row_base, wave, lane);
       return;
     }
     if (wave >= 4) return;
@@ -624,7 +638,7 @@
   __syncthreads();
   if constexpr (CE) {
     if (wave * 32 < A.Nout) tile_times_wt<KC>(acc[0], zt, ldz, A.wtr, K, A.Nout, wave * 32, kr, cc);
-    ce_epilogue(A, acc[0], zt, row_base, wave, lane);
+    ce_epilogue<LST>(A, acc[0], zt, row_base, wave, lane);
     return;
   }
   if (wave >= 4) return;
@@ -878,11 +892,28 @@
   }
   if constexpr (!DENSE && KC > 0) {
     if (A.col_sel && !blk && nt == 1) {
-      if (A.w) spmm_linear_kernel<G, true, KC, 1, false, false, false, false, true><<<(int)blocks, 256, lds, s>>>(A);
-      else spmm_linear_kernel<G, false, KC, 1, false, false, false, false, true><<<(int)blocks, 256, lds, s>>>(A);
+      if (A.w) spmm_linear_kernel<G, true, KC, 1, false, false, false, false, 1><<<(int)blocks, 256, lds, s>>>(A);
+      else spmm_linear_kernel<G, false, KC, 1, false, false, false, false, 1><<<(int)blocks, 256, lds, s>>>(A);
       RGBX_CHECK_LAUNCH("spmm_linear_kernel (column selection)");
       return RGBX_OK;
     }
+    if (A.slot_src && !blk && nt == 1) {
+      if (A.w) spmm_linear_kernel<G, true, KC, 1, false, false, false, false, 2><<<(int)blocks, 256, lds, s>>>(A);
+      else spmm_linear_kernel<G, false, KC, 1, false, false, false, false, 2><<<(int)blocks, 256, lds, s>>>(A);
+      RGBX_CHECK_LAUNCH("spmm_linear_kernel (slot sources)");
+      return RGBX_OK;
+    }
+  }
+  if (A.slot_src)
+    return fail(RGBX_E_ARG, "fused_layer: slot_src has no instantiation for this launch");
+  if (A.ce_compact) {
+    if constexpr (!DENSE && KC > 0) {
+      if (A.w) spmm_linear_kernel<G, true, KC, 1, true, false, false, false, 0, true><<<(int)blocks, 256, lds, s>>>(A);
+      else spmm_linear_kernel<G, false, KC, 1, true, false, false, false, 0, true><<<(int)blocks, 256, lds, s>>>(A);
+      RGBX_CHECK_LAUNCH("spmm_linear_kernel (cross-entropy epilogue, list order)");
+      return RGBX_OK;
+    }
+    return fail(RGBX_E_ARG, "spmm_linear: compact has no instantiation for this launch");
   }
   if (A.ce_part) {
     if (A.w && !DENSE) spmm_linear_kernel<G, !DENSE, KC, 1, true, DENSE, DENSE><<<(int)blocks, 256, lds, s>>>(A);
@@ -985,6 +1016,20 @@
         return fail(RGBX_E_ALIGN, "spmm_linear: a row list with the loss gradient needs `out` 16-byte aligned with "
                                   "ldo %% 4 == 0");
     }
+  }
+  if (ce && ce->compact) {
+    if (!ce->rows || ce->n_rows <= 0 || !ce->grad_scale || L.w_pos || (L.x_root && L.xr_blk_cols > 0))
+      return fail(RGBX_E_ARG, "spmm_linear: compact needs a non-empty row list with the loss gradient, without w_pos or "
+                              "blocked layouts");
+    if (K != 64 && K != 128 && K != 256)
+      return fail(RGBX_E_ARG, "spmm_linear: compact needs K in {64, 128, 256} (got K=%lld)", (long long)K);
+  }
+  if (L.slot_src) {
+    if (dense || ce || L.w_pos || L.out_blk || L.col_sel || (L.x_root && L.xr_blk_cols > 0))
+      return fail(RGBX_E_ARG, "fused_layer: slot_src needs an aggregating launch without ce, w_pos, col_sel or blocked layouts");
+    if ((K != 64 && K != 128 && K != 256) || Nout > 128)
+      return fail(RGBX_E_ARG, "fused_layer: slot_src needs K in {64, 128, 256} and Nout <= 128 (got K=%lld, Nout=%lld)",
+                  (long long)K, (long long)Nout);
   }
   if (L.col_sel && (dense || ce || L.w_pos || L.out_blk || (L.x_root && L.xr_blk_cols > 0)))
     return fail(RGBX_E_ARG, "fused_layer: col_sel needs an aggregating launch without ce, w_pos or blocked layouts");
@@ -1042,7 +1087,7 @@
   const rgbx_row_split_t* split = dense ? nullptr : L.split;
   if (split && split->threshold > 0 && split->n_chunks > 0) {
     float* zl = split->partial ? split->partial + (size_t)split->n_chunks * K : nullptr;
-    if (int rc = spmm_long_rows_compact(L.rowptr, L.col, L.w, L.rs, L.x, L.ldx, (int)K, split, zl, s)) return rc;
+    if (int rc = spmm_long_rows_compact(L.rowptr, L.col, L.w, L.rs, L.x, L.ldx, (int)K, split, zl, s, L.slot_src)) return rc;
     if (L.w_pos) {
       float* zlp = zl ? zl + (size_t)split->n_long * K : nullptr;
       if (int rc = spmm_long_rows_compact(L.rowptr, L.col, L.w_pos, L.rs, L.x, L.ldx, (int)K, split, zlp, s)) return rc;
@@ -1061,6 +1106,7 @@
               x_blk ? L.x_blk_cols : 0, L.x_blk_stride, xr_blk ? L.xr_blk_cols : 0, L.xr_blk_stride,
               L.out_blk, L.ob_cols, L.ob_stride, L.w_pos, L.z_pos_out, zlong_pos};
   A.col_sel = L.col_sel;
+  A.slot_src = L.slot_src;
   if (ce) {
     A.ce_rows = ce->rows;
     A.ce_n_rows = (int)ce->n_rows;
@@ -1074,6 +1120,7 @@
         A.ce_term = reinterpret_cast<float*>(behind);
         A.ce_hit = reinterpret_cast<uint8_t*>(behind + cdiv(N, 2));
         A.ce_skip = 0;
+        A.ce_compact = ce->compact ? 1 : 0;
       }
     }
   }
diff --git a/rgb_experiment_amd/ops.py b/rgb_experiment_amd/ops.py
--- a/rgb_experiment_amd/ops.py
+++ b/rgb_experiment_amd/ops.py
@@ -726,8 +726,8 @@
 
 def fused_layer(x, wt, csr=None, w=None, rs=None, bias=None, x_root=None, wt_root=None, pre=None, want_out=True,
                 out_blocked=None, want_z=False, want_colsums=False, ce=None, kind="linear", out=None, z=None, w_pos=None,
-                select_rows=False, col_sel=None):
-    _lib.require_device(x, wt, bias, x_root, wt_root, out_blocked, col_sel)
+                select_rows=False, col_sel=None, compact=False, slot_src=None):
+    _lib.require_device(x, wt, bias, x_root, wt_root, out_blocked, col_sel, slot_src)
     lib = _lib.load()
     L = _lib.FusedLayer()
     dense = csr is None
@@ -756,6 +756,12 @@
             col_sel = col_sel.contiguous()
             keep.append(col_sel)
             L.col_sel = col_sel.data_ptr()
+        if slot_src is not None:
+            if slot_src.dtype != torch.int32 or slot_src.numel() < csr.nnz or not slot_src.is_contiguous():
+                raise RuntimeError(f"fused_layer: slot_src must be a contiguous int32 vector with an entry per slot, got "
+                                   f"{slot_src.dtype} {tuple(slot_src.shape)} for {csr.nnz} slots")
+            keep.append(slot_src)
+            L.slot_src = slot_src.data_ptr()
         split, _scratch = csr.split_arg(K, x.device, hub_rows=2 if w_pos is not None else 1)
         keep.append(_scratch)
         if split is not None:
@@ -781,6 +787,7 @@
         L.pre_scale, L.pre_shift, L.pre_rowsum = ps.data_ptr(), pt.data_ptr(), pr.data_ptr()
     ce_stats = None
     groups = 1
+    compact = bool(compact and select_rows)
     if ce is not None:
         y, mask, grad_scale = ce
         if isinstance(mask, (tuple, list)):
@@ -817,16 +824,27 @@
             keep.append(rows)
         elif select_rows and not dense and w_pos is None and grad_scale is not None:
             ce_arg.skip_unselected = 1
+        if compact:
+            if rows is None or grad_scale is None or out is not None or z is not None:
+                raise RuntimeError("fused_layer: compact needs the loss gradient over an existing, non-empty row list and "
+                                   "no caller-owned out / z")
+            ce_arg.compact = 1
+            out = torch.empty((rows.numel(), n_out), dtype=torch.float32, device=x.device)
+            if want_z:
+                z = torch.empty((rows.numel(), K), dtype=torch.float32, device=x.device)
         keep += [y, mask, ce_scratch, ce_arg]
         L.ce = ctypes.addressof(ce_arg)
         want_out = grad_scale is not None
+    elif compact:
+        raise RuntimeError("fused_layer: compact needs the loss epilogue (ce)")
+    n_store = out.size(0) if compact else N
     if out is not None:
-        if tuple(out.shape) != (N, n_out) or out.stride(1) != 1 or out.dtype != torch.float32:
+        if tuple(out.shape) != (n_store, n_out) or out.stride(1) != 1 or out.dtype != torch.float32:
             raise RuntimeError(f"fused_layer: out is {tuple(out.shape)}, expected a float32 [{N}, {n_out}] with contiguous rows")
     elif want_out:
         out = torch.empty((N, n_out), dtype=torch.float32, device=x.device)
     if out is not None:
-        L.out, L.ldo = out.data_ptr(), out.stride(0) if N > 1 else n_out
+        L.out, L.ldo = out.data_ptr(), out.stride(0) if n_store > 1 else n_out
     else:
         L.ldo = n_out
     if out_blocked is not None:
@@ -834,13 +852,13 @@
         if out_blocked.size(1) != N or out_blocked.size(0) * out_blocked.size(2) != n_out:
             raise RuntimeError(f"fused_layer: out_blocked is {tuple(out_blocked.shape)} for a [{N}, {n_out}] output")
     if z is not None:
-        if tuple(z.shape) != (N, K) or z.stride(1) != 1 or z.dtype != torch.float32:
+        if tuple(z.shape) != (n_store, K) or z.stride(1) != 1 or z.dtype != torch.float32:
             raise RuntimeError(f"fused_layer: z is {tuple(z.shape)}, expected a float32 [{N}, {K}] with contiguous rows")
     elif want_z or w_pos is not None:
         z = torch.empty((N, K), dtype=torch.float32, device=x.device)
     L.ldz = K
     if z is not None:
-        L.z_out, L.ldz = z.data_ptr(), z.stride(0) if N > 1 else K
+        L.z_out, L.ldz = z.data_ptr(), z.stride(0) if n_store > 1 else K
     z_pos = None
     if w_pos is not None:
         _lib.require_device(w_pos)
@@ -885,10 +903,10 @@
 
 
 def spmm_linear_raw(csr, w, rs, x, wt, bias=None, want_z=False, x_root=None, wt_root=None, kind="linear", pre=None,
-                    want_colsums=False, ce=None, select_rows=False):
+                    want_colsums=False, ce=None, select_rows=False, compact=False):
     out, z, extra = fused_layer(x, wt, csr=csr, w=w, rs=rs, bias=bias, x_root=x_root if wt_root is not None else None,
                                 wt_root=wt_root, pre=pre, want_z=want_z, want_colsums=want_colsums, ce=ce, kind=kind,
-                                select_rows=select_rows)
+                                select_rows=select_rows, compact=compact)
     if ce is not None or want_colsums:
         return out, z, extra
     return out, z
@@ -963,6 +981,7 @@
 
 FUSE_DENSE_BACKWARD = True
 CE_GRAD_ROW_LIST = True
+CE_COMPACT = True
 
 BN_HANDOVER = "_rgbx_bn_handover"
 
@@ -1041,11 +1060,15 @@
         return gx, None, None, gw, gb, None, gwr, None, None, g_bnw, g_bnb, None
 
 
-def _propagate_linear_input_grad(g, kind, gy, weight, root_weight, ce_sel=None):
+def _propagate_linear_input_grad(g, kind, gy, weight, root_weight, ce_sel=None, slot_src=None):
     csr = g.bwd
     wt = {"gcn": lambda: g.w_t, "mean": lambda: g.w_mean_t, "sum": lambda: None}[kind]()
     prefix = getattr(g, "event_prefix", "")
     n_out, n_in = weight.shape
+    if slot_src is not None:
+        gx, _, _ = fused_layer(gy, weight.detach().contiguous(), csr=csr, w=wt, slot_src=slot_src,
+                               kind=f"{prefix}{kind}_linear_bwd")
+        return gx
     if n_out <= n_in and _lib.load().rgbx_spmm_linear_supported(n_out, n_in, int(root_weight is not None)):
         gx, _, _ = fused_layer(gy, weight.detach().contiguous(), csr=csr, w=wt,
                                x_root=gy if root_weight is not None else None,
@@ -1184,6 +1207,56 @@
 
 
 
+def slot_positions(sel):
+    sel = sel.bool()
+    rank = torch.cumsum(sel, 0, dtype=torch.int32) - 1
+    return torch.where(sel, rank, torch.full_like(rank, -1))
+
+
+_SLOT_SRC = {}
+
+
+def slot_sources(csr, y, mask, C):
+    key = (csr.col.data_ptr(), csr.col._version, csr.nnz) + _sel_key(y, mask, C)
+    hit = _SLOT_SRC.get(key)
+    if hit is None:
+        if torch.cuda.is_current_stream_capturing():
+            return None
+        pos = slot_positions(ce_selection(y, mask, C)).contiguous()
+        src = torch.empty(max(csr.nnz, 1), dtype=torch.int32, device=pos.device)
+        _lib.check(_lib.load().rgbx_slot_src_i32(_lib.ptr(csr.col), csr.nnz, _lib.ptr(pos), pos.numel(), _lib.ptr(src),
+                                                 _lib.stream_ptr()), "rgbx_slot_src_i32")
+        hit = (_MadeOn(src), csr.col, y, mask)
+        _SLOT_SRC[key] = hit
+        while len(_SLOT_SRC) > 2:
+            _SLOT_SRC.pop(next(iter(_SLOT_SRC)))
+    return hit[0].get()
+
+
+def ce_compact_decision(*, switch, row_list, dense_backward, want_grad, weight_grad, has_mask, has_root, distributed,
+                        n_in, n_out, bwd_fused, n_rows, have_slot_src):
+    return bool(switch and row_list and dense_backward and want_grad and weight_grad and has_mask and not has_root
+                and not distributed and n_out <= n_in and bwd_fused and n_out in (64, 128, 256) and n_in in (64, 128)
+                and n_rows is not None and n_rows > 0 and have_slot_src)
+
+
+def _ce_compact_plan(graph, kind, weight, root_weight, y, mask, want_grad):
+    n_out, n_in = weight.shape
+    if (not (CE_COMPACT and CE_GRAD_ROW_LIST and FUSE_DENSE_BACKWARD and want_grad and mask is not None)
+            or root_weight is not None or _is_dist(graph)):
+        return None
+    rows = selected_rows(y, mask, n_out)
+    bwd_fused = bool(_lib.load().rgbx_spmm_linear_supported(n_out, n_in, 0))
+    n_rows = None if rows is None else rows.numel()
+    if not ce_compact_decision(switch=True, row_list=True, dense_backward=True, want_grad=True,
+                               weight_grad=weight.requires_grad, has_mask=True, has_root=False, distributed=False,
+                               n_in=n_in, n_out=n_out, bwd_fused=bwd_fused, n_rows=n_rows, have_slot_src=True):
+        return None
+    csr = getattr(graph, "_bwd", None) if torch.cuda.is_current_stream_capturing() else graph.bwd
+    src = None if csr is None else slot_sources(csr, y, mask, n_out)
+    return None if src is None else (rows, src)
+
+
 def ce_from_logits(logits, y, mask):
     if isinstance(mask, (tuple, list)):
         return None, torch.stack([masked_ce_accuracy(logits, y, m) for m in mask])
@@ -1214,11 +1287,15 @@
         ctx.handed_over = bn_weight is not None and bn_args[4] is not None
         w, rs = (graph.w, None) if kind == "gcn" else (None, graph.inv_deg)
         grad_scale = mask_scale(y, mask, weight.size(0)) if want_grad else None
+        plan = _ce_compact_plan(graph, kind, weight, root_weight, y, mask, want_grad)
+        ctx.compact = plan
         dlogits, z, stats = spmm_linear_raw(
             graph.fwd, w, rs, x, weight_t(weight), None if bias is None else bias.detach(),
             want_grad and weight.requires_grad, x if root_weight is not None else None,
             None if root_weight is None else weight_t(root_weight), kind=f"{kind}_linear_fwd", pre=pre,
-            ce=(y, mask, grad_scale), select_rows=True)
+            ce=(y, mask, grad_scale), select_rows=True, compact=plan is not None)
+        if plan is not None and dlogits.size(0) != plan[0].numel():
+            ctx.compact = None
         ctx.graph, ctx.kind, ctx.has_bias, ctx.has_bn = graph, kind, bias is not None, bn_weight is not None
         ctx.ce_sel = (y, mask, weight.size(0)) if want_grad else None
         if want_grad:
@@ -1245,8 +1322,11 @@
         gw = gb = gwr = gx = g_bnw = g_bnb = None
         gcol = None
         if ctx.needs_input_grad[3]:
-            rows = selected_rows(*ctx.ce_sel) if FUSE_DENSE_BACKWARD else None
-            gw, gcol = gemm_tn_rows(gy, z, rows, colsum=True)
+            if ctx.compact is not None:
+                gw, gcol = gemm_tn_rows(gy, z, ctx.compact[0], colsum=True, n_full=graph.fwd.N)
+            else:
+                rows = selected_rows(*ctx.ce_sel) if FUSE_DENSE_BACKWARD else None
+                gw, gcol = gemm_tn_rows(gy, z, rows, colsum=True)
         if ctx.has_bias and ctx.needs_input_grad[4]:
             gb = gcol if gcol is not None else gy.sum(0)
         if root_weight is not None and ctx.needs_input_grad[5]:
@@ -1264,7 +1344,8 @@
         sc = dict(zip((k for k, _ in items), torch._foreach_mul([t for _, t in items], g))) if items else {}
         gw, gb, gwr = sc.get("gw"), sc.get("gb"), sc.get("gwr")
         if need_h:
-            g_h = _propagate_linear_input_grad(graph, kind, gy, sc["w"], sc.get("wr"), ce_sel=ctx.ce_sel)
+            g_h = _propagate_linear_input_grad(graph, kind, gy, sc["w"], sc.get("wr"), ce_sel=ctx.ce_sel,
+                                               slot_src=None if ctx.compact is None else ctx.compact[1])
             if ctx.has_bn and not ctx.handed_over:
                 gx, g_bnw, g_bnb = B.train_backward(g_h, x, bn_weight, mean, rstd, n, ctx.reduce)
             else:
@@ -2698,8 +2779,10 @@
     return out, sums
 
 
-def gemm_tn_rows(a, b, rows, colsum=False):
+def gemm_tn_rows(a, b, rows, colsum=False, n_full=None):
     _lib.require_device(a, b)
+    if n_full is not None:
+        return gemm_tn_rows_compact(a, b, rows, n_full, colsum=colsum)
     if rows is None or not _gemm_tn_v4(a, b) or a.size(0) != b.size(0) or a.size(0) >= 2**31:
         return gemm_tn(a, b, colsum=colsum)
     K, M, N = a.size(0), a.size(1), b.size(1)
@@ -2709,6 +2792,20 @@
         _lib.check(_lib.load().rgbx_gemm_tn_rows_f32(
             pa, lda, pb, ldb, _lib.ptr(rows), rows.numel(), _lib.ptr(out), N, _lib.ptr(sums), K, M, N, 1.0,
             _lib.ptr(ws), ws.numel(), _lib.stream_ptr()), "rgbx_gemm_tn_rows_f32")
+    return (out, sums) if colsum else out
+
+
+def gemm_tn_rows_compact(a, b, rows, n_full, colsum=False):
+    _lib.require_device(a, b, rows)
+    if a.size(0) != rows.numel() or b.size(0) != rows.numel() or n_full >= 2**31:
+        raise RuntimeError(f"gemm_tn_rows_compact: operands of {a.size(0)} / {b.size(0)} rows for a list of {rows.numel()}")
+    K, M, N = int(n_full), a.size(1), b.size(1)
+    ws, out, sums = _gemm_tn_buffers(K, M, N, a.device, colsum)
+    (pa, lda), (pb, ldb) = _lib.mat(a, "a"), _lib.mat(b, "b")
+    with _Timed("gemm_tn", f"{M}x{N}+rows" if _EVENT_SINK is not None else None):
+        _lib.check(_lib.load().rgbx_gemm_tn_rows_compact_f32(
+            pa, lda, pb, ldb, _lib.ptr(rows), rows.numel(), _lib.ptr(out), N, _lib.ptr(sums), K, M, N, 1.0,
+            _lib.ptr(ws), ws.numel(), _lib.stream_ptr()), "rgbx_gemm_tn_rows_compact_f32")
     return (out, sums) if colsum else out
 
 
```
